# taconite/arah-release

Hardware: AMD Instinct MI355X
Metric: rendered rays/sec (higher is better)
Workload: dtype f32 (operands as hi+lo f16 pairs on the f16 MFMA pipe, fp32 accumulate)

## Files before the change

arah_release_amd/csrc/arah_hip.hip:

```cpp
#include <hip/hip_runtime.h>
#include <stdint.h>
#include <stdlib.h>
#include <string.h>

#include <atomic>
#include <mutex>
#include <type_traits>

#include "../../include/arah_hip.h"
#include "pointwise.hpp"
#include "mlp.hpp"

using namespace arah;

namespace {

constexpr float kRootThresh = 1e-5f;
constexpr int kSphereIters = 50;
constexpr float kSurfaceRange = 0.05f;
constexpr float kClampDist = 0.1f;
constexpr int kBroydenSteps = 50;
constexpr float kDvg = 1.0f;
constexpr int kMaxVerts = 6912;
constexpr int kKnnThreads = 1024;
// ... 187 lines not shown
                            const unsigned* amax, float* fw, float* pw, float* fws) {
    const int i = blockIdx.x * blockDim.x + threadIdx.x;
    if (i >= 6 * 256) return;
    const int k = i >> 8;
    const double c = kFilmScale;
    const double f = freq[i];
    fw[i] = (float)(f * c);
    pw[i] = (float)((f * (double)bias[i] + (double)phase[i]) * c);
    const float inv = k == 0 ? 1.0f : 1.0f / (split_weight_scale(amax[k - 1]) * kActScale);
    fws[i] = (float)(f * c) * inv;
    if ((i & 255) == 0) fws[6 * 256 + k] = inv;
}

struct SkinRaw {
    const float* w[4];
    const float* b[4];
};
__global__ __launch_bounds__(128) void k_skin_probe(SkinRaw net, unsigned* amax) {
    __shared__ float h[2][128];
    const int pt = blockIdx.x, c = threadIdx.x;
    const float x = -1.5f + 3.0f * (float)(pt % 9) / 8.0f, y = -1.5f + 3.0f * (float)((pt / 9) % 9) / 8.0f,
                z = -1.5f + 3.0f * (float)(pt / 81) / 8.0f;
    float v = softplus100(net.w[0][c * 3] * x + net.w[0][c * 3 + 1] * y + net.w[0][c * 3 + 2] * z + net.b[0][c]);
    h[0][c] = v;
    float m = v;
#pragma unroll
    for (int o = 32; o > 0; o >>= 1) m = fmaxf(m, __shfl_xor(m, o));
    if ((c & 63) == 0) atomicMax(amax + 0, __float_as_uint(m));
    __syncthreads();
    for (int k = 1; k < 4; ++k) {
        const float* hin = h[(k - 1) & 1];
        float s = net.b[k][c];
        for (int i = 0; i < 128; ++i) s += net.w[k][c * 128 + i] * hin[i];
        v = softplus100(s);
        h[k & 1][c] = v;
        m = v == v ? v : 0.f;
#pragma unroll
        for (int o = 32; o > 0; o >>= 1) m = fmaxf(m, __shfl_xor(m, o));
        if ((c & 63) == 0) atomicMax(amax + k, __float_as_uint(m));
        __syncthreads();
    }
}

__global__ void k_skin_scales(const unsigned* amax, float* scales) {
    const int k = threadIdx.x;
    if (k >= 4) return;
    const float a = __uint_as_float(amax[k]);
    float S = 1.0f;
    if (a > 0.f && a < 3.0e38f) {
        int e;
        frexpf(a, &e);
        S = ldexpf(1.0f, 11 - e);
    }
    scales[k] = S;
    scales[4 + k] = 1.0f / (split_weight_scale(amax[4 + k]) * S);
}

__global__ void k_skin_wave_consts(SkinRaw net, const float* __restrict__ w4, const float* __restrict__ w4b, const unsigned* amax,
                                   float* __restrict__ c) {
    const int i = threadIdx.x;
    auto act_scale = [&](int k) {
        const float a = __uint_as_float(amax[k]) * kZUnit;
        if (!(a > 0.f) || a > 3.0e38f) return 1.0f;
        int e;
        frexpf(a, &e);
        return e > 11 ? ldexpf(1.0f, 11 - e) : 1.0f;
    };
    const double M = (double)kCwShift;
    if (i < 128) {
        unsigned* ct = reinterpret_cast<unsigned*>(c + kCwW0T) + i * 8;
        unsigned short h[3], l[3];
#pragma unroll
        for (int k = 0; k < 3; ++k) {
            const float w = net.w[0][i * 3 + k] * kZUnit;
            const _Float16 hh = (_Float16)w, ll = (_Float16)(w - (float)hh);
            h[k] = __builtin_bit_cast(unsigned short, hh);
            l[k] = __builtin_bit_cast(unsigned short, ll);
        }
        ct[0] = ct[2] = (unsigned)h[0] | ((unsigned)h[1] << 16);
        ct[1] = ct[3] = (unsigned)h[2];
        ct[4] = ct[6] = (unsigned)l[0] | ((unsigned)l[1] << 16);
        ct[5] = ct[7] = (unsigned)l[2];
        c[kCwBinit + i] = (float)((double)net.b[0][i] * (double)kZUnit - M);
#pragma unroll 1
        for (int k = 1; k < 4; ++k) {
            double rs = 0.0;
            for (int col = 0; col < 128; ++col) rs += (double)net.w[k][i * 128 + col];
            c[kCwBinit + k * 128 + i] = (float)(((double)net.b[k][i] * (double)kZUnit + M * rs - M) * (double)act_scale(k - 1));
        }
    }
    if (i < 32) {
        double v = 0.0;
        if (i < 25) {
            double rs = 0.0;
            for (int col = 0; col < 128; ++col) rs += (double)w4[i * 128 + col];
            v = ((double)w4b[i] * (100.0 / 0.6931471805599453) + M * rs) * (double)act_scale(3);
        }
        c[kCwBinit + 512 + i] = (float)v;
    }
    if (i < 4) {
        c[kCwActS + i] = act_scale(i);
        if (i == 0) c[kCwScaled] = (act_scale(0) != 1.0f || act_scale(1) != 1.0f || act_scale(2) != 1.0f || act_scale(3) != 1.0f) ? 1.0f : 0.0f;
        c[kCwInv + i] = i < 3 ? 1.0f / act_scale(i) : 0.2f / act_scale(3);
    }
}

__global__ void k_gather_scalars(float* __restrict__ dst, const float* trans, const float* center, const float* cmin,
                                 const float* cmax, const float* beta) {
    const int i = threadIdx.x;
    if (i < 3) dst[i] = trans[i];
    else if (i < 6) dst[i] = center[i - 3];
    else if (i == 6) dst[i] = cmin[0];
    else if (i == 7) dst[i] = cmax[0];
    else if (i == 8) dst[i] = beta ? beta[0] : 1e-3f;
}

__global__ __launch_bounds__(64) void k_vertex_transforms(const float* __restrict__ weights, const float* __restrict__ bones,
                                                          int n_verts, float* __restrict__ vert_T) {
    __shared__ __attribute__((aligned(16))) float sb[24 * 16];
    for (int i = threadIdx.x; i < 24 * 16; i += 64) sb[i] = bones[i];
    __syncthreads();
    const int v = blockIdx.x * 64 + threadIdx.x;
    if (v >= n_verts) return;
    float T[16];
    blend(weights + (size_t)v * 24, sb, T);
#pragma unroll
    for (int c = 0; c < 4; ++c)
        reinterpret_cast<f32x4*>(vert_T + (size_t)v * 16)[c] = f32x4{T[c * 4], T[c * 4 + 1], T[c * 4 + 2], T[c * 4 + 3]};
}

__global__ void k_pad_rows4(float* __restrict__ dst, const float* __restrict__ src, int rows, int rows_pad, int ncol,
                            float fill) {
    const int r = blockIdx.x * blockDim.x + threadIdx.x;
    if (r >= rows_pad) return;
    f32x4 v = {fill, fill, fill, 0.f};
    if (r < rows) {
        for (int c = 0; c < 4; ++c) v[c] = c < ncol ? src[(size_t)r * ncol + c] : 0.f;
    }
    reinterpret_cast<f32x4*>(dst)[r] = v;
}

__global__ void k_copy(float* __restrict__ dst, const float* __restrict__ src, int n, int n_pad) {
    const int i = blockIdx.x * blockDim.x + threadIdx.x;
    if (i < n_pad) dst[i] = i < n ? src[i] : 0.f;
}

__global__ void k_fold_bias(float* __restrict__ dst, const float* __restrict__ b, const float* __restrict__ W, int ld,
                            int col0, const float* __restrict__ vec, int n_vec, int rows) {
    const int r = blockIdx.x * blockDim.x + threadIdx.x;
    if (r >= rows) return;
    float s = b[r];
    for (int c = 0; c < n_vec; ++c) s += W[(size_t)r * ld + col0 + c] * vec[c];
    dst[r] = s;
}

enum { SRC_POINTS = 0, SRC_RAYS = 1, SRC_SAMPLES = 2 };

constexpr int kClusterSize = 28;
constexpr int kClusterLds = 29;
constexpr int kMaxClusters = 256;
constexpr int kMaxCells = 65536;
constexpr int kCellBytes = 64;
constexpr float kGridMargin = 0.08f;

struct GridInfo {
    float origin[3];
    float h, inv_h;
    int dims[3];
    int n_cells;
    int n_clusters;
    int pad[2];
};

struct RaySet {
    const float* cam_loc;
    const float* dirs;
    int rays_per_cam;
};

__device__ __forceinline__ V3 ray_point(const RaySet& rs, int ray, float t) {
    const int cam = ray / rs.rays_per_cam;
    V3 p;
    p.x = rs.dirs[ray * 3 + 0] * t + rs.cam_loc[cam * 3 + 0];
    p.y = rs.dirs[ray * 3 + 1] * t + rs.cam_loc[cam * 3 + 1];
    p.z = rs.dirs[ray * 3 + 2] * t + rs.cam_loc[cam * 3 + 2];
    return p;
}

__device__ __forceinline__ void bitonic_cas(unsigned* keys, unsigned short* idxs, int i, int j, int k) {
    const int l = i | j;
    const bool up = (i & k) == 0;
    const unsigned ka = keys[i], kb = keys[l];
    const unsigned short ia = idxs[i], ib = idxs[l];
    const bool gt = ka > kb || (ka == kb && ia > ib);
    if (gt == up) {
        keys[i] = kb;
        keys[l] = ka;
        idxs[i] = ib;
        idxs[l] = ia;
    }
}
__device__ __forceinline__ void bitonic_sort_8192(unsigned* keys, unsigned short* idxs, int tid) {
    const int wave = tid >> 6, lane = tid & 63;
    for (int k = 2; k <= 8192; k <<= 1) {
        int j = k >> 1;
        for (; j >= 512; j >>= 1) {
            for (int t = tid; t < 4096; t += 1024) bitonic_cas(keys, idxs, ((t & ~(j - 1)) << 1) | (t & (j - 1)), j, k);
            __syncthreads();
        }
        for (; j > 0; j >>= 1) {
#pragma unroll
            for (int u = 0; u < 4; ++u) {
                const int t = lane + 64 * u;
                bitonic_cas(keys, idxs, wave * 512 + (((t & ~(j - 1)) << 1) | (t & (j - 1))), j, k);
            }
            __builtin_amdgcn_fence(__ATOMIC_RELEASE, "wavefront");
            __builtin_amdgcn_wave_barrier();
            __builtin_amdgcn_fence(__ATOMIC_ACQUIRE, "wavefront");
        }
        __syncthreads();
    }
}

__device__ __forceinline__ void wave_lds_handover() {
    __builtin_amdgcn_fence(__ATOMIC_RELEASE, "wavefront");
    __builtin_amdgcn_wave_barrier();
    __builtin_amdgcn_fence(__ATOMIC_ACQUIRE, "wavefront");
}

__device__ __forceinline__ int float_ordered(float f) {
    const int b = __float_as_int(f);
    return b >= 0 ? b : b ^ 0x7fffffff;
}
__device__ __forceinline__ float ordered_float(int o) { return __int_as_float(o >= 0 ? o : o ^ 0x7fffffff); }

__global__ __launch_bounds__(1024) void k_sort_verts(const float* __restrict__ verts, int n, float* __restrict__ sorted4,
                                                      GridInfo* __restrict__ grid) {
    __shared__ unsigned keys[8192];
    __shared__ unsigned short idxs[8192];
    __shared__ unsigned char segid[8192];
    int (*sbox)[6] = reinterpret_cast<int(*)[6]>(keys);
    __shared__ int sstart[2][257];
    __shared__ unsigned char saxis[256];
    __shared__ float bb[6];
    const int tid = threadIdx.x;
    for (int i = tid; i < 8192; i += 1024) {
        idxs[i] = (unsigned short)i;
        segid[i] = 0;
    }
    if (tid == 0) {
        sstart[0][0] = 0;
        sstart[0][1] = n;
    }
    __syncthreads();
    int cur = 0;
    for (int level = 0; level < 8; ++level) {
        const int nseg = 1 << level;
        for (int i = tid; i < nseg * 6; i += 1024) sbox[i / 6][i % 6] = (i % 6) < 3 ? 0x7fffffff : (int)0x80000000;
        __syncthreads();
        for (int i = tid; i < n; i += 1024) {
            const int o = idxs[i], sg = segid[i];
            for (int c = 0; c < 3; ++c) {
                const int v = float_ordered(verts[o * 3 + c]);
                atomicMin(&sbox[sg][c], v);
                atomicMax(&sbox[sg][3 + c], v);
            }
        }
        __syncthreads();
        if (level == 0 && tid < 6) bb[tid] = ordered_float(sbox[0][tid]);
        if (tid < nseg) {
            float e[3];
            for (int c = 0; c < 3; ++c) e[c] = ordered_float(sbox[tid][3 + c]) - ordered_float(sbox[tid][c]);
            saxis[tid] = (unsigned char)(e[0] >= e[1] ? (e[0] >= e[2] ? 0 : 2) : (e[1] >= e[2] ? 1 : 2));
        }
        __syncthreads();
        for (int i = tid; i < 8192; i += 1024) {
            unsigned key = 0xffffffffu;
            if (i < n) {
                const int o = idxs[i], sg = segid[i], a = saxis[sg];
                const float lo = bb[a], ext = fmaxf(bb[3 + a] - bb[a], 1e-9f);
                const unsigned q = (unsigned)fminf(fmaxf((verts[o * 3 + a] - lo) / ext * 65535.0f, 0.f), 65535.f);
                key = ((unsigned)sg << 16) | q;
            }
            keys[i] = key;
        }
        __syncthreads();
        bitonic_sort_8192(keys, idxs, tid);
        if (tid < nseg) {
            const int a = sstart[cur][tid], b = sstart[cur][tid + 1];
            sstart[cur ^ 1][2 * tid] = a;
            sstart[cur ^ 1][2 * tid + 1] = a + (b - a + 1) / 2;
            if (tid == nseg - 1) sstart[cur ^ 1][2 * nseg] = b;
        }
        __syncthreads();
        for (int i = tid; i < n; i += 1024) {
            const int sg = segid[i];
            segid[i] = (unsigned char)(2 * sg + (i >= sstart[cur ^ 1][2 * sg + 1] ? 1 : 0));
        }
        cur ^= 1;
        __syncthreads();
    }
    if (tid == 0) {
        GridInfo g;
        float ext[3];
        for (int c = 0; c < 3; ++c) {
            g.origin[c] = bb[c] - kGridMargin;
// ... 2712 lines not shown
    unsigned char* cells = nullptr;
};
constexpr size_t kBodyOffSpheres = (size_t)kMaxClusters * kClusterSize * 16;
constexpr size_t kBodyOffGrid = kBodyOffSpheres + (size_t)kMaxClusters * 16;
constexpr size_t kBodyOffCells = kBodyOffGrid + ((sizeof(GridInfo) + 255) / 256) * 256;
constexpr size_t kBodyBytes = kBodyOffCells + (size_t)kMaxCells * kCellBytes;
static_assert(kBodyOffSpheres == ARAH_BODY_OFF_SPHERES && kBodyOffGrid == ARAH_BODY_OFF_GRID && kBodyOffCells == ARAH_BODY_OFF_CELLS,
              "the body buffer's layout is part of the test ABI (arah_cell_clusters_debug)");

BodyTables body_tables(void* buf) {
    char* b = reinterpret_cast<char*>(buf);
    BodyTables t;
    t.verts4 = reinterpret_cast<float*>(b);
    t.spheres = reinterpret_cast<float*>(b + kBodyOffSpheres);
    t.grid = reinterpret_cast<GridInfo*>(b + kBodyOffGrid);
    t.cells = reinterpret_cast<unsigned char*>(b + kBodyOffCells);
    return t;
}

void launch_cell_clusters(int variant, const GridInfo* grid, const float* spheres, unsigned char* cells, hipStream_t s) {
    if (variant == 0)
        hipLaunchKernelGGL(k_cell_clusters, dim3(kMaxCells / kCellThreads), dim3(kCellThreads), 0, s, grid, spheres, cells);
    else
        hipLaunchKernelGGL(k_cell_clusters_wave, dim3(2048), dim3(kCellWaves * 64), 0, s, grid, spheres, cells);
}

void launch_body_tables(const float* verts, int n_verts, const BodyTables& t, hipStream_t s) {
    hipLaunchKernelGGL(k_sort_verts, dim3(1), dim3(1024), 0, s, verts, n_verts, t.verts4, t.grid);
    hipLaunchKernelGGL(k_cluster_spheres, dim3(1), dim3(256), 0, s, (const float*)t.verts4, t.spheres);
    launch_cell_clusters(1, t.grid, t.spheres, t.cells, s);
}

}

static B3Nets b3_of(const ArahFrame& f) {
    B3Nets b;
    for (int i = 0; i < 5; ++i) {
        b.sdf_wp[i] = reinterpret_cast<const bf16x8*>(f.b3[i]);
        b.sdf_wpT[i] = reinterpret_cast<const bf16x8*>(f.b3[5 + i]);
    }
    for (int i = 0; i < 6; ++i) {
        b.col[i] = reinterpret_cast<const bf16x8*>(f.b3[10 + i]);
        b.colT[i] = reinterpret_cast<const bf16x8*>(f.b3[16 + i]);
    }
    return b;
}

static bool shade_b3(int32_t shade_engine) { return shade_engine != ARAH_SHADE_ENGINE_FP32; }

extern "C" {

size_t arah_body_bytes(void) { return kBodyBytes; }

int arah_prepare_body(const float* verts, int32_t n_verts, void* body_buf, size_t body_bytes, void* stream) {
    if (!verts || !body_buf || (reinterpret_cast<uintptr_t>(body_buf) & 255) != 0) return ARAH_E_BADARG;
    if (n_verts <= 0 || n_verts > kMaxVerts) return ARAH_E_SHAPE;
    if (body_bytes < kBodyBytes) return ARAH_E_WORKSPACE;
    if (int arc = setup_attributes()) return arc;
    launch_body_tables(verts, n_verts, body_tables(body_buf), reinterpret_cast<hipStream_t>(stream));
    return check_launch();
}

int arah_cell_clusters_debug(int32_t variant, const void* grid, const float* spheres, uint8_t* cells, void* stream) {
    if ((variant != 0 && variant != 1) || !grid || !spheres || !cells) return ARAH_E_BADARG;
    launch_cell_clusters(variant, reinterpret_cast<const GridInfo*>(grid), spheres, cells, reinterpret_cast<hipStream_t>(stream));
    return check_launch();
}

const char* arah_dominant_kernel(void) { return "k_canon_wave"; }

size_t arah_frame_bytes(const ArahNets* h_nets, const ArahBody* h_body) {
    if (!h_nets || !h_body) return 0;
    return frame_layout(h_nets->col_mode).bytes;
}

int arah_prepare_frame(const ArahNets* nets, const ArahBody* body, void* frame_buf, size_t frame_bytes,
                       ArahFrame* out, void* stream) {
    if (!nets || !body || !frame_buf || !out) return ARAH_E_BADARG;
    if (nets->col_mode != ARAH_COLOR_IDR && nets->col_mode != ARAH_COLOR_NO_VIEW_DIR) return ARAH_E_SHAPE;
    if (body->n_verts <= 0 || body->n_verts > kMaxVerts || nets->n_pose < 0) return ARAH_E_SHAPE;
    if (nets->precision != ARAH_PRECISION_SPLIT_F16 && nets->precision != ARAH_PRECISION_FP32) return ARAH_E_BADARG;
    const FrameLayout L = frame_layout(nets->col_mode);
    if (frame_bytes < L.bytes) return ARAH_E_WORKSPACE;
    if (int arc = setup_attributes()) return arc;
    hipStream_t s = reinterpret_cast<hipStream_t>(stream);
    char* base = reinterpret_cast<char*>(frame_buf);
    auto P = [&](size_t off) { return reinterpret_cast<float*>(base + off); };
    const bool idr = nets->col_mode == ARAH_COLOR_IDR;
    const int kin_pad = idr ? ColDims<true>::kInPad : ColDims<false>::kInPad;
    const int kc0 = kin_pad / 16;
    const int n_view = idr ? 27 : 0;
    const int in_dim = 3 + n_view + 3 + 256 + nets->n_pose;
    PrepJobs jobs;
    unsigned* amax_sdf = reinterpret_cast<unsigned*>(base + L.sdf_amax);
    unsigned* amax_skin = reinterpret_cast<unsigned*>(base + L.skin_amax);
    hipLaunchKernelGGL(k_zero_words, dim3(1), dim3(64), 0, s, amax_sdf, 64, amax_skin, 64);
    jobs.add_rows4(P(L.sdf_w0), nets->sdf_w[0], 256, 256, 3);
    for (int i = 0; i < 5; ++i) {
        jobs.add_pack(P(L.sdf_wp[i]), nets->sdf_w[i + 1], 256, 256, 16, 16, one_seg(256), 0);
        jobs.add_pack(P(L.sdf_wpT[i]), nets->sdf_w[i + 1], 256, 256, 16, 16, one_seg(256), 1);
    }
    jobs.add_copy(P(L.sdf_w6), nets->sdf_w[6], 256, 256);
    for (int i = 0; i < 6; ++i) jobs.add_copy(P(L.sdf_bias) + i * 256, nets->sdf_b[i], 256, 256);
    jobs.add_copy(P(L.sdf_freq), nets->film_freq, 6 * 256, 6 * 256);
    jobs.add_copy(P(L.sdf_phase), nets->film_phase, 6 * 256, 6 * 256);
    jobs.add_copy(P(L.sdf_b6), nets->sdf_b[6], 1, 64);
    for (int i = 0; i < 5; ++i) {
        jobs.add_absmax(nets->sdf_w[i + 1], 256 * 256, amax_sdf + i, 16);
        jobs.add_split(reinterpret_cast<f16x8*>(base + L.sdf_wps[i]), nets->sdf_w[i + 1], 256, 256, 16, 8, amax_sdf + i, 0);
    }
    jobs.add_rows4(P(L.skin_w0), nets->skin_w[0], 128, 128, 3);
    for (int i = 0; i < 3; ++i) jobs.add_pack(P(L.skin_wp[i]), nets->skin_w[i + 1], 128, 128, 8, 8, one_seg(128), 0);
    jobs.add_pack(P(L.skin_w4p), nets->skin_w[4], 25, 128, 2, 8, one_seg(128), 0);
    for (int i = 0; i < 4; ++i) jobs.add_copy(P(L.skin_bias) + i * 128, nets->skin_b[i], 128, 128);
    jobs.add_copy(P(L.skin_bias) + 512, nets->skin_b[4], 25, 32);
    SkinRaw raw;
    for (int i = 0; i < 4; ++i) {
        raw.w[i] = nets->skin_w[i];
        raw.b[i] = nets->skin_b[i];
    }
    hipLaunchKernelGGL(k_skin_probe, dim3(9 * 9 * 9), dim3(128), 0, s, raw, amax_skin);
    for (int i = 0; i < 4; ++i) {
        const int M = i < 3 ? 128 : 25, mt = i < 3 ? 8 : 2;
        jobs.add_absmax(nets->skin_w[i + 1], M * 128, amax_skin + 4 + i, 8);
        jobs.add_split(reinterpret_cast<f16x8*>(base + L.skin_wps[i]), nets->skin_w[i + 1], M, 128, mt, 4, amax_skin + 4 + i, 0);
        jobs.add_split(reinterpret_cast<f16x8*>(base + L.skin_wpr + (size_t)i * kCwLayerBytes), nets->skin_w[i + 1], M, 128, mt, 4,
                       amax_skin + 4 + i, 1);
    }
    {
        ColSegs sg;
        memset(&sg, 0, sizeof(sg));
        const int feat0 = 3 + n_view + 3;
        sg.n = idr ? 4 : 3;
        sg.dst0[0] = 0; sg.src0[0] = feat0; sg.len[0] = 256;
        sg.dst0[1] = 256; sg.src0[1] = 0; sg.len[1] = 3;
        sg.dst0[2] = 259; sg.src0[2] = 3 + n_view; sg.len[2] = 3;
        if (idr) { sg.dst0[3] = 262; sg.src0[3] = 3; sg.len[3] = 27; }
        jobs.add_pack(P(L.col_w0p), nets->col_w[0], 256, in_dim, 16, kc0, sg, 0);
        jobs.add_pack(P(L.col_w3ap), nets->col_w[3], 256, in_dim + 128, 16, kc0, sg, 0);
        ColSegs sb = one_seg(128);
        sb.src0[0] = in_dim;
        jobs.add_pack(P(L.col_w3bp), nets->col_w[3], 256, in_dim + 128, 16, 8, sb, 0);
        jobs.add_pack(P(L.col_w1p), nets->col_w[1], 256, 256, 16, 16, one_seg(256), 0);
        jobs.add_pack(P(L.col_w2p), nets->col_w[2], 128, 256, 8, 16, one_seg(256), 0);
        jobs.add_pack(P(L.col_w4p), nets->col_w[4], 256, 256, 16, 16, one_seg(256), 0);
        jobs.add_pack(P(L.col_w0pT), nets->col_w[0], kin_pad, in_dim, kc0, 16, sg, 2, 256);
        jobs.add_pack(P(L.col_w3apT), nets->col_w[3], kin_pad, in_dim + 128, kc0, 16, sg, 2, 256);
        jobs.add_pack(P(L.col_w3bpT), nets->col_w[3], 128, in_dim + 128, 8, 16, sb, 2, 256);
        jobs.add_pack(P(L.col_w1pT), nets->col_w[1], 256, 256, 16, 16, one_seg(256), 1);
        jobs.add_pack(P(L.col_w2pT), nets->col_w[2], 256, 256, 16, 8, one_seg(128), 1);
        jobs.add_pack(P(L.col_w4pT), nets->col_w[4], 256, 256, 16, 16, one_seg(256), 1);
        jobs.add_copy(P(L.col_w5), nets->col_w[5], 3 * 256, 3 * 256);
        float* cb = P(L.col_bias);
        hipLaunchKernelGGL(k_fold_bias, dim3(1), dim3(256), 0, s, cb, nets->col_b[0], nets->col_w[0], in_dim,
                           feat0 + 256, nets->pose_vec, nets->pose_vec ? nets->n_pose : 0, 256);
        jobs.add_copy(cb + 256, nets->col_b[1], 256, 256);
        jobs.add_copy(cb + 512, nets->col_b[2], 128, 128);
        hipLaunchKernelGGL(k_fold_bias, dim3(1), dim3(256), 0, s, cb + 640, nets->col_b[3], nets->col_w[3],
                           in_dim + 128, feat0 + 256, nets->pose_vec, nets->pose_vec ? nets->n_pose : 0, 256);
        jobs.add_copy(cb + 896, nets->col_b[4], 256, 256);
        jobs.add_copy(cb + 1152, nets->col_b[5], 3, 4);
    }
    if (nets->precision == ARAH_PRECISION_SPLIT_F16) {
        const size_t src[kB3Count] = {L.sdf_wp[0], L.sdf_wp[1], L.sdf_wp[2], L.sdf_wp[3], L.sdf_wp[4],
                                      L.sdf_wpT[0], L.sdf_wpT[1], L.sdf_wpT[2], L.sdf_wpT[3], L.sdf_wpT[4],
                                      L.col_w0p, L.col_w1p, L.col_w2p, L.col_w3ap, L.col_w3bp, L.col_w4p,
                                      L.col_w0pT, L.col_w1pT, L.col_w2pT, L.col_w3apT, L.col_w3bpT, L.col_w4pT};
        for (int i = 5; i < 16; ++i) {
            const B3Src e = b3_source(i, kc0);
            jobs.add_b3(reinterpret_cast<bf16x8*>(base + L.b3[i]), (const float*)P(src[i]), e.m_tiles, e.kc16);
        }
    }
    if (!jobs.ok) return ARAH_E_LAUNCH;
    jobs.flush_a(s);
    jobs.flush_b(s);
    hipLaunchKernelGGL(k_fold_film, dim3(6), dim3(256), 0, s, (const float*)P(L.sdf_freq), (const float*)P(L.sdf_phase),
                       (const float*)P(L.sdf_bias), (const unsigned*)amax_sdf, P(L.sdf_fw), P(L.sdf_pw), P(L.sdf_fws));
    hipLaunchKernelGGL(k_skin_scales, dim3(1), dim3(64), 0, s, (const unsigned*)amax_skin, P(L.skin_scales));
    hipLaunchKernelGGL(k_skin_wave_consts, dim3(1), dim3(128), 0, s, raw, nets->skin_w[4], nets->skin_b[4],
                       (const unsigned*)amax_skin, P(L.skin_wconsts));
    if (!body->trans || !body->center || !body->coord_min || !body->coord_max || !body->verts || !body->vert_weights ||
        !body->bones)
        return ARAH_E_BADARG;
    hipLaunchKernelGGL(k_gather_scalars, dim3(1), dim3(64), 0, s, P(L.scalars), body->trans, body->center, body->coord_min,
                       body->coord_max, nets->beta);
    BodyTables bt;
    if (body->prepared) {
        bt = body_tables(const_cast<void*>(body->prepared));
    } else {
        bt.verts4 = P(L.verts4);
        bt.spheres = P(L.knn_spheres);
        bt.grid = reinterpret_cast<GridInfo*>(base + L.knn_grid);
        bt.cells = reinterpret_cast<unsigned char*>(base + L.knn_cells);
        launch_body_tables(body->verts, body->n_verts, bt, s);
    }
    hipLaunchKernelGGL(k_vertex_transforms, dim3((body->n_verts + 63) / 64), dim3(64), 0, s, body->vert_weights, body->bones,
                       body->n_verts, P(L.vert_T));
    memset(out, 0, sizeof(*out));
    out->sdf_w0 = P(L.sdf_w0);
    for (int i = 0; i < 5; ++i) {
        out->sdf_wp[i] = P(L.sdf_wp[i]);
        out->sdf_wpT[i] = P(L.sdf_wpT[i]);
    }
    out->sdf_w6 = P(L.sdf_w6);
    out->sdf_bias = P(L.sdf_bias);
    out->sdf_freq = P(L.sdf_freq);
    out->sdf_phase = P(L.sdf_phase);
    for (int i = 0; i < 5; ++i) out->sdf_wps[i] = base + L.sdf_wps[i];
    out->sdf_fw = P(L.sdf_fw);
    out->sdf_pw = P(L.sdf_pw);
    out->sdf_fws = P(L.sdf_fws);
    out->precision = nets->precision;
    out->skin_w0 = P(L.skin_w0);
    for (int i = 0; i < 3; ++i) out->skin_wp[i] = P(L.skin_wp[i]);
    out->skin_w4p = P(L.skin_w4p);
    out->skin_bias = P(L.skin_bias);
    for (int i = 0; i < 4; ++i) out->skin_wps[i] = base + L.skin_wps[i];
    out->skin_scales = P(L.skin_scales);
    out->skin_wpr = base + L.skin_wpr;
    out->skin_wconsts = P(L.skin_wconsts);
    out->col_w0p = P(L.col_w0p);
    out->col_w1p = P(L.col_w1p);
    out->col_w2p = P(L.col_w2p);
    out->col_w3ap = P(L.col_w3ap);
    out->col_w3bp = P(L.col_w3bp);
    out->col_w4p = P(L.col_w4p);
    out->col_w5 = P(L.col_w5);
    out->col_bias = P(L.col_bias);
    out->col_w0pT = P(L.col_w0pT);
    out->col_w1pT = P(L.col_w1pT);
    out->col_w2pT = P(L.col_w2pT);
    out->col_w3apT = P(L.col_w3apT);
    out->col_w3bpT = P(L.col_w3bpT);
    out->col_w4pT = P(L.col_w4pT);
    for (int i = 0; i < kB3Count; ++i) out->b3[i] = base + L.b3[i];
    out->verts4 = bt.verts4;
    out->knn_spheres = bt.spheres;
    out->knn_grid = bt.grid;
    out->knn_cells = bt.cells;
    out->verts = body->verts;
    out->vert_T = P(L.vert_T);
    out->bones = body->bones;
    out->sdf_b6 = P(L.sdf_b6);
    out->scalars = P(L.scalars);
    out->n_verts = body->n_verts;
    out->col_mode = nets->col_mode;
    return check_launch();
}

size_t arah_workspace_bytes(int32_t n_rays, int32_t n_steps) {
    if (n_rays < 0 || n_steps < 0) return 0;
    return carve(nullptr, n_rays, n_steps).bytes;
}

int arah_counters_reset(void* workspace, void* stream) {
    if (!workspace) return ARAH_E_BADARG;
    Workspace w = carve(workspace, 1, 1);
    return hipMemsetAsync(w.ctr, 0, sizeof(Counters), reinterpret_cast<hipStream_t>(stream)) == hipSuccess ? ARAH_OK
                                                                                                           : ARAH_E_LAUNCH;
}

#ifdef ARAH_CLOCKS
int arah_debug_clocks(const void* workspace, unsigned long long* h_out, void* stream) {
    if (!workspace || !h_out) return ARAH_E_BADARG;
    Workspace w = carve(const_cast<void*>(workspace), 1, 1);
    hipStream_t s = reinterpret_cast<hipStream_t>(stream);
    if (hipMemcpyAsync(h_out, w.ctr->clk, sizeof(w.ctr->clk) + sizeof(w.ctr->clk_shade), hipMemcpyDeviceToHost, s) != hipSuccess) return ARAH_E_LAUNCH;
    return hipStreamSynchronize(s) == hipSuccess ? ARAH_OK : ARAH_E_LAUNCH;
}
#endif

int arah_counters_read(const void* workspace, ArahCounters* h_out, void* stream) {
    if (!workspace || !h_out) return ARAH_E_BADARG;
    Workspace w = carve(const_cast<void*>(workspace), 1, 1);
    hipStream_t s = reinterpret_cast<hipStream_t>(stream);
    if (hipMemcpyAsync(h_out, w.ctr, sizeof(ArahCounters), hipMemcpyDeviceToHost, s) != hipSuccess) return ARAH_E_LAUNCH;
    return hipStreamSynchronize(s) == hipSuccess ? ARAH_OK : ARAH_E_LAUNCH;
}

int arah_sdf_eval(const ArahFrame* f, const float* x_norm, int32_t n, float* sdf, float* feat, float* grad,
                  void* workspace, size_t wbytes, void* stream) {
    if (!f || n < 0 || !workspace) return ARAH_E_BADARG;
    if (n == 0) return ARAH_OK;
    if (!x_norm || !sdf) return ARAH_E_BADARG;
    Workspace w = carve(workspace, 1, 1);
    if (wbytes < w.bytes) return ARAH_E_WORKSPACE;
    if (int arc = setup_attributes()) return arc;
    hipStream_t s = reinterpret_cast<hipStream_t>(stream);
    const FrameDev fd = to_dev(*f);
    const int g = grid_for(n, kTile);
    if (grad)
        LAUNCH_ENGINE(fd.split, (k_sdf_eval<true, true>), (k_sdf_eval<true, false>), dim3(g), dim3(kThreads), kLdsSdfGrad,
                      s, fd, x_norm, (const int*)nullptr, (const int*)nullptr, n, sdf, feat, grad, w.spill,
                      &w.ctr->n_sdf_fwd, &w.ctr->n_sdf_grad, 0);
    else
        LAUNCH_ENGINE(fd.split, (k_sdf_eval<false, true>), (k_sdf_eval<false, false>), dim3(g), dim3(kThreads),
                      kLdsSdfFwd, s, fd, x_norm, (const int*)nullptr, (const int*)nullptr, n, sdf, feat, (float*)nullptr,
                      (f32x4*)nullptr, &w.ctr->n_sdf_fwd, (unsigned long long*)nullptr, 0);
    return check_launch();
}

int arah_sdf_grid(const ArahFrame* f, int32_t n_side, float* sdf, void* workspace, size_t wbytes, void* stream) {
    if (!f || !sdf || !workspace || n_side < 2 || n_side > 1024) return ARAH_E_BADARG;
    Workspace w = carve(workspace, 1, 1);
    if (wbytes < w.bytes) return ARAH_E_WORKSPACE;
    if (int arc = setup_attributes()) return arc;
    hipStream_t s = reinterpret_cast<hipStream_t>(stream);
    const FrameDev fd = to_dev(*f);
    const long long n = (long long)n_side * n_side * n_side;
    if (n > 0x7fffffffLL) return ARAH_E_BADARG;
    if (fd.split && n >= 128ll * 1024)
        hipLaunchKernelGGL(k_sdf_lattice, dim3(min(num_cus(), grid_for(n, 128))), dim3(kThreads), kLdsDensityWide, s, fd, (int)n_side,
// ... 783 lines not shown
    const int64_t n_pix = (int64_t)H * W;
    unsigned long long* k = reinterpret_cast<unsigned long long*>(keys);
    int* med_list = pix_to_face;
    int* huge_list = reinterpret_cast<int*>(depth);
    unsigned* counters = reinterpret_cast<unsigned*>(bary);
    hipLaunchKernelGGL(k_mr_init, dim3(mesh_grid(n_pix, kMrMaxGrid)), dim3(kImeshThreads), 0, s, k, (long long)n_pix, counters);
    if (F > 0 && V > 0) {
        hipLaunchKernelGGL(k_mr_scatter, dim3(mesh_grid(F, kMrMaxGrid)), dim3(kImeshThreads), 0, s, verts, V, (const int*)faces, F, (int)H, (int)W, z_near,
                           (int)cull, (int)small_area, (int)wave_area, (int)huge_area, k, med_list, huge_list, (unsigned)n_pix, counters);
        hipLaunchKernelGGL(k_mr_lists, dim3(kMrListGrid), dim3(kImeshThreads), 0, s, verts, V, (const int*)faces, F, (int)H, (int)W, z_near,
                           (int)cull, k, (const int*)med_list, (const int*)huge_list, (unsigned)n_pix, (const unsigned*)counters);
    }
    hipLaunchKernelGGL(k_mr_resolve, dim3(mesh_grid(n_pix, kMrMaxGrid)), dim3(kImeshThreads), 0, s, verts, V, (const int*)faces, F, (int)H, (int)W,
                       (const unsigned long long*)k, (int*)pix_to_face, depth, bary);
    return check_launch();
}

int arah_mesh_rasterize(const float* verts, int64_t n_verts, const int32_t* faces, int64_t n_faces, int32_t H, int32_t W, float z_near,
                        int32_t cull, uint64_t* keys, int32_t* pix_to_face, float* depth, float* bary, void* stream) {
    return mr_rasterize(verts, n_verts, faces, n_faces, H, W, z_near, cull, kMrSmallArea, kMrWaveArea, kMrHugeArea, keys, pix_to_face,
                        depth, bary, stream);
}

int arah_mesh_rasterize_debug(const float* verts, int64_t n_verts, const int32_t* faces, int64_t n_faces, int32_t H, int32_t W,
                              float z_near, int32_t cull, int32_t small_area, int32_t wave_area, int32_t huge_area, uint64_t* keys,
                              int32_t* pix_to_face, float* depth, float* bary, void* stream) {
    return mr_rasterize(verts, n_verts, faces, n_faces, H, W, z_near, cull, small_area, wave_area, huge_area, keys, pix_to_face, depth,
                        bary, stream);
}

int arah_mesh_interpolate(const int32_t* pix_to_face, const float* bary, int32_t H, int32_t W, const int32_t* faces, int64_t n_faces,
                          const float* attr, int64_t n_verts, int32_t n_channels, float background, float* out, void* stream) {
    if (n_verts < 0 || n_faces < 0 || n_verts > (int64_t)INT32_MAX || n_faces > (int64_t)INT32_MAX) return ARAH_E_BADARG;
    if (H <= 0 || W <= 0 || (int64_t)H * W > (int64_t)INT32_MAX || n_channels < 1 || n_channels > 32) return ARAH_E_BADARG;
    if (!pix_to_face || !bary || !out || (n_verts > 0 && !attr) || (n_faces > 0 && !faces)) return ARAH_E_BADARG;
    const int64_t n_pix = (int64_t)H * W;
    hipLaunchKernelGGL(k_mr_interpolate, dim3(mesh_grid(n_pix * n_channels, kMrMaxGrid)), dim3(kImeshThreads), 0, reinterpret_cast<hipStream_t>(stream),
                       (const int*)pix_to_face, bary, (long long)n_pix, (const int*)faces, (int)n_faces, attr, (int)n_verts,
                       (int)n_channels, background, out);
    return check_launch();
}

int arah_skin_jacobian(const ArahFrame* f, const float* x_hat, int32_t n, float* jac, void* workspace, size_t wbytes,
                       void* stream) {
    if (!f || n < 0 || !workspace) return ARAH_E_BADARG;
    if (n == 0) return ARAH_OK;
    if (!x_hat || !jac) return ARAH_E_BADARG;
    Workspace w = carve(workspace, 1, 1);
    if (wbytes < w.bytes) return ARAH_E_WORKSPACE;
    if (int arc = setup_attributes()) return arc;
    hipLaunchKernelGGL(k_skin_jac, dim3(grid_for(n, 16)), dim3(kThreads), kLdsSkin,
                       reinterpret_cast<hipStream_t>(stream), to_dev(*f), x_hat, (const int*)nullptr,
                       (const int*)nullptr, n, jac, &w.ctr->n_skin_jac);
    return check_launch();
}

int arah_color_eval(const ArahFrame* f, const float* x_norm, const float* normal, const float* view,
                    const float* feat, int32_t n, float* rgb, void* workspace, size_t wbytes, void* stream) {
    if (!f || n < 0 || !workspace) return ARAH_E_BADARG;
    if (n == 0) return ARAH_OK;
    if (!x_norm || !normal || !feat || !rgb) return ARAH_E_BADARG;
    if (f->col_mode == ARAH_COLOR_IDR && !view) return ARAH_E_BADARG;
    Workspace w = carve(workspace, 1, 1);
    if (wbytes < w.bytes) return ARAH_E_WORKSPACE;
    if (int arc = setup_attributes()) return arc;
    hipStream_t s = reinterpret_cast<hipStream_t>(stream);
    const FrameDev fd = to_dev(*f);
    if (f->col_mode == ARAH_COLOR_IDR)
        hipLaunchKernelGGL(k_color_eval<true>, dim3(grid_for(n, kTile)), dim3(kThreads), lds_color<true>(), s, fd,
                           x_norm, normal, view, feat, n, rgb, &w.ctr->n_col);
    else
        hipLaunchKernelGGL(k_color_eval<false>, dim3(grid_for(n, kTile)), dim3(kThreads), lds_color<false>(), s, fd,
                           x_norm, normal, view, feat, n, rgb, &w.ctr->n_col);
    return check_launch();
}

int arah_nearest_inverse_lbs(const ArahFrame* f, const float* pts, int32_t n, int32_t* idx, float* x_hat0, float* T0,
                             void* workspace, size_t wbytes, void* stream) {
    if (!f || !pts || !x_hat0 || !T0 || n < 0 || !workspace) return ARAH_E_BADARG;
    if (n == 0) return ARAH_OK;
    Workspace w = carve(workspace, 1, 1);
    if (wbytes < w.bytes) return ARAH_E_WORKSPACE;
    if (int arc = setup_attributes()) return arc;
    RaySet rs = make_rays(nullptr, nullptr, 1);
    launch_nearest<SRC_POINTS>(reinterpret_cast<hipStream_t>(stream), to_dev(*f), n, pts, rs, (const float*)nullptr, 1,
                               (const int*)nullptr, (const int*)nullptr, n, idx, x_hat0, T0, 0,
                               &w.ctr->n_knn);
    return check_launch();
}

static int run_broyden3(const FrameDev& fd, Workspace& w, const float* tgt, CanonOut outp, long long max_pts,
                        hipStream_t s, int mode_arg = ARAH_CANON_KERNEL_WAVE, void* const* ev = nullptr,
                        const int* list_arg = nullptr, int* cnt_arg = nullptr) {
    int* cnt = cnt_arg ? cnt_arg : w.counts;
    const int* const list = list_arg ? list_arg : w.listA;
    if (tgt)
        hipLaunchKernelGGL(k_canon_seed, dim3(grid_for(max_pts, 256)), dim3(256), 0, s, list,
                           (const int*)&cnt[0], tgt, outp.T);
    const int mode = mode_arg == ARAH_CANON_KERNEL_TILE ? 0 : (mode_arg == ARAH_CANON_KERNEL_WAVE_L2 ? 2 : 1);
    hipEvent_t ev0 = ev ? reinterpret_cast<hipEvent_t>(ev[0]) : nullptr, ev1 = ev ? reinterpret_cast<hipEvent_t>(ev[1]) : nullptr;
    if (ev0 && ev1) hipEventRecord(ev0, s);
    unsigned long long* const clk_arg = w.ctr->clk;
    if (fd.split && mode != 0) {
        long long gw = (max_pts + kCwWaves * kCwSlots - 1) / (kCwWaves * kCwSlots);
        int cus = num_cus();
        if (list_arg && knobs().canon_tier_wgs > 0) cus = min(cus, knobs().canon_tier_wgs);
        if (gw > cus) gw = cus;
        if (gw < 1) gw = 1;
        if (mode == 1) {
            hipLaunchKernelGGL((k_canon_wave<true, false>), dim3((int)gw), dim3(kCwThreads), kLdsCanonWave, s, fd, list,
                               (const int*)&cnt[0], &cnt[1], outp, &w.ctr->n_skin_fwd, &w.ctr->n_canon,
                               &w.ctr->n_split_nonfinite, clk_arg);
            hipLaunchKernelGGL((k_canon_wave<true, true>), dim3((int)gw), dim3(kCwThreads), kLdsCanonWave, s, fd, list,
                               (const int*)&cnt[0], &cnt[1], outp, &w.ctr->n_skin_fwd, &w.ctr->n_canon,
                               &w.ctr->n_split_nonfinite, clk_arg);
        } else {
            const size_t lds_l2 = kLdsCanonWave - kCwHiBytes;
            hipLaunchKernelGGL((k_canon_wave<false, false>), dim3((int)gw), dim3(kCwThreads), lds_l2, s, fd,
                               list, (const int*)&cnt[0], &cnt[1], outp, &w.ctr->n_skin_fwd,
                               &w.ctr->n_canon, &w.ctr->n_split_nonfinite, clk_arg);
            hipLaunchKernelGGL((k_canon_wave<false, true>), dim3((int)gw), dim3(kCwThreads), lds_l2, s, fd,
                               list, (const int*)&cnt[0], &cnt[1], outp, &w.ctr->n_skin_fwd,
                               &w.ctr->n_canon, &w.ctr->n_split_nonfinite, clk_arg);
        }
    } else {
        LAUNCH_ENGINE(fd.split, k_canon_solve<true>, k_canon_solve<false>, dim3(grid_for(max_pts, kTile)), dim3(kThreads),
                      kLdsCanonSolve, s, fd, list, (const int*)&cnt[0], &cnt[1], outp,
                      &w.ctr->n_skin_fwd, &w.ctr->n_canon, w.ctr->clk);
    }
    if (ev0 && ev1) hipEventRecord(ev1, s);
    return check_launch();
}

int arah_broyden3_lbs(const ArahFrame* f, const float* tgt, const float* x0, const float* T0, int32_t n, float* x,
                      float* T, float* err, uint8_t* conv, int32_t canon_kernel, void* workspace, size_t wbytes, void* stream) {
    if (!f || n < 0 || !workspace) return ARAH_E_BADARG;
    if (n == 0) return ARAH_OK;
    if (!tgt || !x0 || !T0 || !x || !T || !conv) return ARAH_E_BADARG;
    Workspace w = carve(workspace, n, 1);
    if (wbytes < w.bytes) return ARAH_E_WORKSPACE;
    if (int arc = setup_attributes()) return arc;
    hipStream_t s = reinterpret_cast<hipStream_t>(stream);
    const FrameDev fd = to_dev(*f);
    hipMemcpyAsync(x, x0, (size_t)n * 3 * 4, hipMemcpyDeviceToDevice, s);
    hipMemcpyAsync(T, T0, (size_t)n * 16 * 4, hipMemcpyDeviceToDevice, s);
    hipMemsetAsync(w.counts, 0, sizeof(int) * 3 * kNumCounts, s);
    hipLaunchKernelGGL(k_iota, dim3((n + 255) / 256), dim3(256), 0, s, n, w.listA, &w.counts[0]);
    int rc = run_broyden3(fd, w, tgt, CanonOut{x, T, w.q_err}, n, s, canon_kernel);
    if (rc) return rc;
    hipLaunchKernelGGL(k_broyden3_finalize, dim3((n + 255) / 256), dim3(256), 0, s, n, (const float*)w.q_err, err, conv);
    return check_launch();
}

static void joint_impl(const FrameDev& fd, Workspace& w, const RaySet& rs, int n, float* T, hipStream_t s) {
    int* cntB = w.counts + kNumCounts;
    const int gm = grid_for(n, kTile);
    hipLaunchKernelGGL(k_skin_jac, dim3(grid_for(n, 16)), dim3(kThreads), kLdsSkin, s, fd, (const float*)w.x0raw,
                       (const int*)w.listA, (const int*)&cntB[0], 0, w.jac_lbs, &w.ctr->n_skin_jac);
    LAUNCH_ENGINE(fd.split, (k_sdf_eval<true, true>), (k_sdf_eval<true, false>), dim3(gm), dim3(kThreads), kLdsSdfGrad, s,
                  fd, (const float*)w.xcur, (const int*)w.listA, (const int*)&cntB[0], 0, w.u_gx ,
                  (float*)nullptr, w.grad_sdf, w.spill, &w.ctr->n_sdf_fwd, &w.ctr->n_sdf_grad, 0);
    Broyden4State st{w.u_eval, w.u_step, w.u_gx, w.u_Jinv, w.err_best_ray, w.xbest_ray, w.zbest_ray, T};
    hipLaunchKernelGGL(k_joint_init, dim3(grid_for(n, 256)), dim3(256), 0, s, fd, st, rs, (const int*)w.listA,
                       (const int*)&cntB[0], (const float*)w.grad_sdf, (const float*)w.jac_lbs, (const float*)w.xcur,
                       (const float*)w.t, w.x0raw);
    const int bulk = knobs().joint_bulk;
    for (int it = 0; it < bulk; ++it) {
        int* lin = (it & 1) ? w.listB : w.listA;
        int* lout = (it & 1) ? w.listA : w.listB;
        if (it == 0)
            LAUNCH_ENGINE(fd.split, (k_joint_iter<true, true>), (k_joint_iter<true, false>), dim3(gm), dim3(kThreads),
                          kLdsJoint, s, fd, st, rs, (const int*)lin, (const int*)&cntB[it], lout, &cntB[it + 1],
                          &w.ctr->n_skin_fwd, &w.ctr->n_sdf_fwd);
        else
            LAUNCH_ENGINE(fd.split, (k_joint_iter<false, true>), (k_joint_iter<false, false>), dim3(gm), dim3(kThreads),
                          kLdsJoint, s, fd, st, rs, (const int*)lin, (const int*)&cntB[it], lout, &cntB[it + 1],
                          &w.ctr->n_skin_fwd, &w.ctr->n_sdf_fwd);
    }
    if (bulk <= kBroydenSteps) {
        const int* lin = (bulk & 1) ? w.listB : w.listA;
        const int gf = min(4 * num_cus(), max(1, (n + kFinTile - 1) / kFinTile));
        LAUNCH_ENGINE(fd.split, k_joint_finish<true>, k_joint_finish<false>, dim3(gf), dim3(kThreads), kLdsJointFinish, s, fd,
                      st, rs, lin, (const int*)&cntB[bulk], kBroydenSteps + 1 - bulk, &w.ctr->n_skin_fwd, &w.ctr->n_sdf_fwd);
    }
}

static int trace_impl(const ArahFrame* f, Workspace& w, const float* cam_loc, int32_t rays_per_cam,
                      const float* dirs, const float* near_far, int32_t n, int root_find_all, float* points_hat_norm,
                      float* T, uint8_t* conv, float* start, float* end, hipStream_t s, const uint8_t* skip = nullptr) {
    const FrameDev fd = to_dev(*f);
    const RaySet rs = make_rays(cam_loc, dirs, rays_per_cam);
    const int gb = (n + 255) / 256;
    int* cntA = w.counts;
    int* cntB = w.counts + kNumCounts;
    hipMemsetAsync(w.counts, 0, sizeof(int) * 3 * kNumCounts, s);
    hipMemsetAsync(w.nn_idx, 0xff, sizeof(int) * (size_t)n, s);
    hipLaunchKernelGGL(k_trace_begin, dim3(gb), dim3(256), 0, s, near_far, n, w.t, w.far, w.diverged, w.xcur, w.Tcur,
                       w.listA, &cntA[0], skip);
    TraceState ts{w.t, w.far, w.xcur, w.diverged};
    const int gm = grid_for(n, kTile);
    const int bulk = n <= knobs().trace_small ? 0 : knobs().trace_bulk;
    for (int it = 0; it < bulk; ++it) {
        int* lin = (it & 1) ? w.listB : w.listA;
        int* lout = (it & 1) ? w.listA : w.listB;
        launch_nearest<SRC_RAYS>(s, fd, n, (const float*)nullptr, rs, (const float*)w.t, 1, (const int*)lin,
                                 (const int*)&cntA[it], 0, w.nn_idx, w.xcur, w.Tcur, 0, &w.ctr->n_knn);
        LAUNCH_ENGINE(fd.split, k_sdf_march<true>, k_sdf_march<false>, dim3(gm), dim3(kThreads), kLdsSdfFwd, s, fd, ts,
                      (const int*)lin, (const int*)&cntA[it], lout, &cntA[it + 1], &w.ctr->n_sdf_fwd);
    }
    if (bulk < kSphereIters) {
        const int* lin = (bulk & 1) ? w.listB : w.listA;
        const int gf = min(4 * num_cus(), max(1, (n + kFinTile - 1) / kFinTile));
        LAUNCH_ENGINE(fd.split, k_trace_finish<true>, k_trace_finish<false>, dim3(gf), dim3(kThreads), kLdsTraceFinish, s, fd,
                      knn_of(fd), rs, ts, w.Tcur, w.nn_idx, lin, (const int*)&cntA[bulk], kSphereIters - bulk, &w.ctr->n_knn,
                      &w.ctr->n_sdf_fwd);
    }
    hipLaunchKernelGGL(k_joint_select, dim3(gb), dim3(256), 0, s, fd, n, (const float*)w.xcur, (const float*)w.Tcur,
                       (const float*)w.t, (const uint8_t*)w.diverged, root_find_all, w.x0raw, w.xbest_ray, w.zbest_ray, T,
                       w.err_best_ray, w.listA, &cntB[0]);
    joint_impl(fd, w, rs, n, T, s);
    hipLaunchKernelGGL(k_trace_finalize, dim3(gb), dim3(256), 0, s, fd, n, near_far, (const float*)w.xbest_ray,
                       (const float*)w.zbest_ray, (const float*)w.err_best_ray, points_hat_norm, conv, start, end);
    return check_launch();
}

int arah_trace(const ArahFrame* f, const float* cam_loc, int32_t rays_per_cam, const float* dirs,
               const float* near_far, int32_t n, int32_t root_find_all, float* points_hat_norm, float* T,
               uint8_t* conv, float* start, float* end, void* workspace, size_t wbytes, void* stream) {
    if (!f || n < 0 || !workspace) return ARAH_E_BADARG;
    if (n == 0) return ARAH_OK;
    if (!cam_loc || !dirs || !near_far || !points_hat_norm || !T || !conv || !start || !end) return ARAH_E_BADARG;
    Workspace w = carve(workspace, n, 1);
    if (wbytes < w.bytes) return ARAH_E_WORKSPACE;
    if (int arc = setup_attributes()) return arc;
    return trace_impl(f, w, cam_loc, rays_per_cam, dirs, near_far, n, root_find_all, points_hat_norm, T, conv, start,
                      end, reinterpret_cast<hipStream_t>(stream));
}

int arah_joint_root_find(const ArahFrame* f, const float* cam_loc, int32_t rays_per_cam, const float* dirs,
                         const uint8_t* valid, const float* x0, const float* z0, const float* T0, int32_t n, float* x,
                         float* z, float* T, uint8_t* conv, void* workspace, size_t wbytes, void* stream) {
    if (!f || n < 0 || !workspace) return ARAH_E_BADARG;
    if (n == 0) return ARAH_OK;
    if (!cam_loc || !dirs || !valid || !x0 || !z0 || !T0 || !x || !z || !T || !conv) return ARAH_E_BADARG;
    Workspace w = carve(workspace, n, 1);
    if (wbytes < w.bytes) return ARAH_E_WORKSPACE;
    if (int arc = setup_attributes()) return arc;
    hipStream_t s = reinterpret_cast<hipStream_t>(stream);
    const FrameDev fd = to_dev(*f);
    const RaySet rs = make_rays(cam_loc, dirs, rays_per_cam);
    const int gb = (n + 255) / 256;
    hipMemsetAsync(w.counts, 0, sizeof(int) * 3 * kNumCounts, s);
    hipLaunchKernelGGL(k_joint_seed, dim3(gb), dim3(256), 0, s, fd, n, x0, z0, T0, valid, w.x0raw, w.xcur, w.t, w.xbest_ray,
                       w.zbest_ray, T, w.err_best_ray, w.listA, &w.counts[kNumCounts]);
    joint_impl(fd, w, rs, n, T, s);
    hipLaunchKernelGGL(k_joint_seam_out, dim3(gb), dim3(256), 0, s, n, (const float*)w.xbest_ray, (const float*)w.zbest_ray,
                       (const float*)w.err_best_ray, valid, x, z, conv);
    return check_launch();
}

static DepthArgs depth_args(const ArahSampling* cfg, const float* near_far, const float* start, const float* end) {
    return DepthArgs{cfg->n_near, cfg->n_far, near_far, start, end, cfg->lin_steps, cfg->lin_near, cfg->lin_far};
}

static void launch_sample_depths(int variant, int n, const ArahSampling* cfg, const float* near_far, const uint8_t* conv,
                                 const float* start, const float* end, const float* rand_s, const float* rand_near,
                                 const float* rand_far, float* z, uint8_t* mask, hipStream_t s) {
    if (variant == 0)
        hipLaunchKernelGGL(k_sample_depths, dim3((n + 127) / 128), dim3(128), 0, s, n, cfg->n_steps, cfg->n_near, cfg->n_far, near_far,
                           conv, start, end, cfg->lin_steps, cfg->lin_near, cfg->lin_far, rand_s, rand_near, rand_far, z, mask);
    else
        hipLaunchKernelGGL(k_sample_depths_wave, dim3(min(2048, (n + kTierWaves - 1) / kTierWaves)), dim3(kTierWaves * 64), 0, s, n,
                           cfg->n_steps, depth_args(cfg, near_far, start, end), conv, z, mask);
}

static int sample_impl(const ArahFrame* f, const ArahSampling* cfg, Workspace& w, const float* cam_loc,
                       int32_t rays_per_cam, const float* dirs, const float* near_far, const uint8_t* conv,
                       const float* start, const float* end, int32_t n, const float* rand_s, const float* rand_near,
                       const float* rand_far, float* z, float* pts, float* T, uint8_t* mask, hipStream_t s) {
    const int S = cfg->n_steps;
    const FrameDev fd = to_dev(*f);
    const RaySet rs = make_rays(cam_loc, dirs, rays_per_cam);
    const long long Q = (long long)n * S;
    hipMemsetAsync(w.counts, 0, sizeof(int) * 3 * kNumCounts, s);
    launch_sample_depths(rand_s || rand_near || rand_far ? 0 : 1, n, cfg, near_far, conv, start, end, rand_s, rand_near, rand_far, z,
                         w.q_smask, s);
    const int gq = (int)((Q + 255) / 256);
    hipLaunchKernelGGL(k_build_list, dim3((int)((Q + 4095) / 4096)), dim3(1024), 0, s, (const uint8_t*)w.q_smask, (int)Q, w.listA, &w.counts[0]);
    launch_nearest<SRC_SAMPLES>(s, fd, Q, (const float*)nullptr, rs, (const float*)z, S, (const int*)w.listA,
                                (const int*)&w.counts[0], 0, (int*)nullptr, pts, T, 1, &w.ctr->n_knn);
    int rc = run_broyden3(fd, w, nullptr, CanonOut{pts, T, w.q_err}, Q, s, cfg->canon_kernel, cfg->ev_canon);
    if (rc) return rc;
    hipLaunchKernelGGL(k_canon_finalize, dim3(gq), dim3(256), 0, s, fd, (int)Q, (const uint8_t*)w.q_smask,
                       (const float*)w.q_err, pts, T, mask);
    return check_launch();
}

static int check_sampling(const ArahSampling* cfg) {
    const int S = cfg->n_steps;
    if (S <= 0 || S > ARAH_MAX_STEPS || cfg->n_near < 0 || cfg->n_far < 0 || S < cfg->n_near + cfg->n_far + 1)
        return ARAH_E_SAMPLING;
    if (!cfg->lin_steps || !cfg->lin_near || (cfg->n_far > 0 && !cfg->lin_far)) return ARAH_E_BADARG;
    return ARAH_OK;
}

int arah_sample_canonicalize(const ArahFrame* f, const ArahSampling* cfg, const float* cam_loc, int32_t rays_per_cam,
                             const float* dirs, const float* near_far, const uint8_t* conv, const float* start,
                             const float* end, int32_t n, const float* rand_steps, const float* rand_near,
                             const float* rand_far, float* z, float* pts, float* T, uint8_t* mask, void* workspace,
                             size_t wbytes, void* stream) {
    if (!f || !cfg || n < 0 || !workspace) return ARAH_E_BADARG;
    int rc = check_sampling(cfg);
    if (rc) return rc;
    if (n == 0) return ARAH_OK;
    if (!cam_loc || !dirs || !near_far || !conv || !start || !end || !z || !pts || !T || !mask) return ARAH_E_BADARG;
    Workspace w = carve(workspace, n, cfg->n_steps);
    if (wbytes < w.bytes) return ARAH_E_WORKSPACE;
    if (int arc = setup_attributes()) return arc;
    if ((rand_steps || rand_near || rand_far) && (!rand_steps || !rand_near || (cfg->n_far > 0 && !rand_far)))
        return ARAH_E_BADARG;
    return sample_impl(f, cfg, w, cam_loc, rays_per_cam, dirs, near_far, conv, start, end, n, rand_steps, rand_near,
                       rand_far, z, pts, T, mask, reinterpret_cast<hipStream_t>(stream));
}

int arah_sample_depths_debug(int32_t variant, int32_t n, int32_t n_steps, int32_t n_near, int32_t n_far,
                             const float* near_far, const uint8_t* conv, const float* start, const float* end,
                             const float* lin_steps, const float* lin_near, const float* lin_far, float* z, uint8_t* mask,
                             void* stream) {
    if ((variant != 0 && variant != 1) || n < 0) return ARAH_E_BADARG;
    ArahSampling cfg;
    memset(&cfg, 0, sizeof(cfg));
    cfg.n_steps = n_steps;
    cfg.n_near = n_near;
    cfg.n_far = n_far;
    cfg.lin_steps = lin_steps;
    cfg.lin_near = lin_near;
    cfg.lin_far = lin_far;
    if (int rc = check_sampling(&cfg)) return rc;
    if (n == 0) return ARAH_OK;
    if (!near_far || !conv || !start || !end || !z || !mask) return ARAH_E_BADARG;
    launch_sample_depths(variant, n, &cfg, near_far, conv, start, end, nullptr, nullptr, nullptr, z, mask,
                         reinterpret_cast<hipStream_t>(stream));
    return check_launch();
}

static void launch_density(const FrameDev& fd, Workspace& w, const float* pts, long long Q, const int* list, const int* count,
                           int* next_list, int* next_count, hipStream_t s) {
    const int g = grid_for(Q, kTile);
    if (fd.split && Q >= 128ll * 1024)
        hipLaunchKernelGGL((k_density<true, 8>), dim3(min(num_cus(), grid_for(Q, 128))), dim3(kThreads), kLdsDensityWide, s, fd,
                           pts, list, count, w.shaded, next_list, next_count, &w.ctr->n_sdf_fwd, &w.ctr->n_density);
    else
        LAUNCH_ENGINE(fd.split, k_density<true>, k_density<false>, dim3(g), dim3(kThreads), kLdsSdfFwd, s, fd, pts, list, count,
                      w.shaded, next_list, next_count, &w.ctr->n_sdf_fwd, &w.ctr->n_density);
}

struct MapsOut {
    f32x4* nrm;
    float* normal;
    float* depth;
};

static int shade_tail(const ArahFrame* f, const ArahSampling* cfg, Workspace& w, const FrameDev& fd, const float* dirs,
                      const float* z, const float* pts, const float* T, const uint8_t* mask, int32_t n, const int* slist,
                      const int* scount, float* rgb, float* acc, uint8_t* vol_mask, const MapsOut* maps, hipStream_t s);

static int shade_impl(const ArahFrame* f, const ArahSampling* cfg, Workspace& w, const float* dirs, const float* z,
                      const float* pts, const float* T, const uint8_t* mask, int32_t n, float* rgb, float* acc,
                      uint8_t* vol_mask, const MapsOut* maps, hipStream_t s) {
    const int S = cfg->n_steps;
    const FrameDev fd = to_dev(*f);
    const long long Q = (long long)n * S;
    hipMemsetAsync(w.counts, 0, sizeof(int) * 3 * kNumCounts, s);
    hipLaunchKernelGGL(k_build_list, dim3((int)((Q + 4095) / 4096)), dim3(1024), 0, s, mask, (int)Q, w.listA, &w.counts[0]);
    const int g = grid_for(Q, kTile);
    const int* slist = w.listA;
    const int* scount = &w.counts[0];
    if (!cfg->full_shading) {
        if (cfg->ev_density[0] && cfg->ev_density[1]) hipEventRecord(reinterpret_cast<hipEvent_t>(cfg->ev_density[0]), s);
        launch_density(fd, w, pts, Q, (const int*)w.listA, (const int*)&w.counts[0], w.listB, &w.counts[1], s);
        if (cfg->ev_density[0] && cfg->ev_density[1]) hipEventRecord(reinterpret_cast<hipEvent_t>(cfg->ev_density[1]), s);
        slist = w.listB;
        scount = &w.counts[1];
    }
    return shade_tail(f, cfg, w, fd, dirs, z, pts, T, mask, n, slist, scount, rgb, acc, vol_mask, maps, s);
}

extern "C++" template <bool MAPS>
static void launch_shade(const ArahFrame* f, const ArahSampling* cfg, Workspace& w, const FrameDev& fd, const float* dirs,
                         const float* pts, const float* T, const int* slist, const int* scount, int g, f32x4* nrm,
                         hipStream_t s) {
    const int S = cfg->n_steps;
    const B3Nets b3 = b3_of(*f);
    if (fd.split && shade_b3(cfg->shade_engine)) {
        if (f->col_mode == ARAH_COLOR_IDR)
            hipLaunchKernelGGL((k_shade<true, true, true, MAPS>), dim3(g), dim3(kThreads), lds_shade_b3<true>(), s, fd,
                               S, cfg->cano_view_dirs, dirs, pts, T, slist, scount, 0, w.shaded, w.spill, &w.ctr->n_sdf_fwd,
                               &w.ctr->n_sdf_grad, &w.ctr->n_col, b3, nrm);
        else
            hipLaunchKernelGGL((k_shade<false, true, true, MAPS>), dim3(g), dim3(kThreads), lds_shade_b3<false>(), s, fd,
                               S, cfg->cano_view_dirs, dirs, pts, T, slist, scount, 0, w.shaded, w.spill, &w.ctr->n_sdf_fwd,
                               &w.ctr->n_sdf_grad, &w.ctr->n_col, b3, nrm);
    } else if (f->col_mode == ARAH_COLOR_IDR)
        LAUNCH_ENGINE(fd.split, (k_shade<true, true, false, MAPS>), (k_shade<true, false, false, MAPS>), dim3(g), dim3(kThreads),
                      lds_shade<true>(), s, fd, S, cfg->cano_view_dirs, dirs, pts, T, slist, scount, 0, w.shaded, w.spill,
                      &w.ctr->n_sdf_fwd, &w.ctr->n_sdf_grad, &w.ctr->n_col, b3, nrm);
    else
        LAUNCH_ENGINE(fd.split, (k_shade<false, true, false, MAPS>), (k_shade<false, false, false, MAPS>), dim3(g), dim3(kThreads),
                      lds_shade<false>(), s, fd, S, cfg->cano_view_dirs, dirs, pts, T, slist, scount, 0, w.shaded, w.spill,
                      &w.ctr->n_sdf_fwd, &w.ctr->n_sdf_grad, &w.ctr->n_col, b3, nrm);
}

static int shade_tail(const ArahFrame* f, const ArahSampling* cfg, Workspace& w, const FrameDev& fd, const float* dirs,
                      const float* z, const float* pts, const float* T, const uint8_t* mask, int32_t n, const int* slist,
                      const int* scount, float* rgb, float* acc, uint8_t* vol_mask, const MapsOut* maps, hipStream_t s) {
    const int S = cfg->n_steps;
    const long long Q = (long long)n * S;
    const int g = grid_for(Q, kTile);
    if (cfg->ev_shade[0] && cfg->ev_shade[1]) hipEventRecord(reinterpret_cast<hipEvent_t>(cfg->ev_shade[0]), s);
    if (maps) launch_shade<true>(f, cfg, w, fd, dirs, pts, T, slist, scount, g, maps->nrm, s);
    else launch_shade<false>(f, cfg, w, fd, dirs, pts, T, slist, scount, g, nullptr, s);
    if (cfg->ev_shade[0] && cfg->ev_shade[1]) hipEventRecord(reinterpret_cast<hipEvent_t>(cfg->ev_shade[1]), s);
    const bool chunk = S % 8 == 0 && (reinterpret_cast<uintptr_t>(z) & 15) == 0 && (reinterpret_cast<uintptr_t>(mask) & 7) == 0;
    const dim3 gc((n + 127) / 128), bc(128);
    if (maps) {
        if (chunk) hipLaunchKernelGGL(k_composite_maps<true>, gc, bc, 0, s, n, S, cfg->render_last_pt, z, mask, (const f32x4*)w.shaded,
                                      rgb, acc, vol_mask, (const f32x4*)maps->nrm, maps->normal, maps->depth);
        else hipLaunchKernelGGL(k_composite_maps<false>, gc, bc, 0, s, n, S, cfg->render_last_pt, z, mask, (const f32x4*)w.shaded,
                                rgb, acc, vol_mask, (const f32x4*)maps->nrm, maps->normal, maps->depth);
    } else if (chunk) hipLaunchKernelGGL(k_composite<true>, gc, bc, 0, s, n, S, cfg->render_last_pt, z, mask, (const f32x4*)w.shaded,
                                         rgb, acc, vol_mask);
    else hipLaunchKernelGGL(k_composite<false>, gc, bc, 0, s, n, S, cfg->render_last_pt, z, mask, (const f32x4*)w.shaded,
                            rgb, acc, vol_mask);
    return check_launch();
}

int arah_shade_points(const ArahFrame* f, const float* x_norm, const float* T, const float* dirs, int32_t n,
                      int32_t cano_view_dirs, int32_t shade_engine, float* rgbs, float* sdfn, void* workspace, size_t wbytes,
                      void* stream) {
    if (!f || n < 0 || !workspace) return ARAH_E_BADARG;
    if (n == 0) return ARAH_OK;
    if (!x_norm || !T || !dirs || !rgbs || !sdfn) return ARAH_E_BADARG;
    Workspace w = carve(workspace, n, 1);
    if (wbytes < w.bytes) return ARAH_E_WORKSPACE;
    if (int arc = setup_attributes()) return arc;
    hipStream_t s = reinterpret_cast<hipStream_t>(stream);
    const FrameDev fd = to_dev(*f);
    const B3Nets b3 = b3_of(*f);
    const int g = grid_for(n, kTile);
    f32x4* out = reinterpret_cast<f32x4*>(rgbs);
    f32x4* dbg = reinterpret_cast<f32x4*>(sdfn);
    if (fd.split && shade_b3(shade_engine)) {
        if (f->col_mode == ARAH_COLOR_IDR)
            hipLaunchKernelGGL((k_shade<true, true, true>), dim3(g), dim3(kThreads), lds_shade_b3<true>(), s, fd, 1,
                               cano_view_dirs, dirs, x_norm, T, (const int*)nullptr, (const int*)nullptr, n, out, w.spill,
                               &w.ctr->n_sdf_fwd, &w.ctr->n_sdf_grad, &w.ctr->n_col, b3, dbg);
        else
            hipLaunchKernelGGL((k_shade<false, true, true>), dim3(g), dim3(kThreads), lds_shade_b3<false>(), s, fd, 1,
                               cano_view_dirs, dirs, x_norm, T, (const int*)nullptr, (const int*)nullptr, n, out, w.spill,
                               &w.ctr->n_sdf_fwd, &w.ctr->n_sdf_grad, &w.ctr->n_col, b3, dbg);
    } else if (f->col_mode == ARAH_COLOR_IDR)
        LAUNCH_ENGINE(fd.split, (k_shade<true, true>), (k_shade<true, false>), dim3(g), dim3(kThreads), lds_shade<true>(),
                      s, fd, 1, cano_view_dirs, dirs, x_norm, T, (const int*)nullptr, (const int*)nullptr, n, out, w.spill,
                      &w.ctr->n_sdf_fwd, &w.ctr->n_sdf_grad, &w.ctr->n_col, b3, dbg);
    else
        LAUNCH_ENGINE(fd.split, (k_shade<false, true>), (k_shade<false, false>), dim3(g), dim3(kThreads),
                      lds_shade<false>(), s, fd, 1, cano_view_dirs, dirs, x_norm, T, (const int*)nullptr, (const int*)nullptr, n,
                      out, w.spill, &w.ctr->n_sdf_fwd, &w.ctr->n_sdf_grad, &w.ctr->n_col, b3, dbg);
    return check_launch();
}

int arah_shade_composite(const ArahFrame* f, const ArahSampling* cfg, const float* dirs, const float* z,
                         const float* pts, const float* T, const uint8_t* mask, int32_t n, float* rgb, float* acc,
                         uint8_t* vol_mask, void* workspace, size_t wbytes, void* stream) {
    if (!f || !cfg || n < 0 || !workspace) return ARAH_E_BADARG;
    if (cfg->n_steps <= 0 || cfg->n_steps > ARAH_MAX_STEPS) return ARAH_E_SAMPLING;
    if (n == 0) return ARAH_OK;
    if (!dirs || !z || !pts || !T || !mask || !rgb || !vol_mask) return ARAH_E_BADARG;
    Workspace w = carve(workspace, n, cfg->n_steps);
    if (wbytes < w.bytes) return ARAH_E_WORKSPACE;
    if (int arc = setup_attributes()) return arc;
    return shade_impl(f, cfg, w, dirs, z, pts, T, mask, n, rgb, acc, vol_mask, nullptr, reinterpret_cast<hipStream_t>(stream));
}

static ColNetT colT_of(const ArahFrame& f) {
    return ColNetT{f.col_w0pT, f.col_w1pT, f.col_w2pT, f.col_w3apT, f.col_w3bpT, f.col_w4pT};
}

static bool train_b3(const ArahFrame& f) {
    return knobs().train_b3 && f.precision == ARAH_PRECISION_SPLIT_F16;
}

size_t arah_shade_train_slab_bytes(void) { return (size_t)kMaxGrid / 2 * kTrainSlabPerWg * sizeof(f32x4); }

int arah_shade_train_forward(const ArahFrame* f, const ArahTrainIn* in, float* sdf, float* rgb4, void* workspace,
// ... 1704 lines not shown
```

arah_release_amd/csrc/finish.hpp:

```cpp
#pragma once

constexpr int kFinTile = 16;
constexpr size_t kLdsTraceFinish = (kFinTile * 4 * 2 + kFinTile * 16 + kFinTile * 8) * 4 + (size_t)kFinTile * kSdfLd * 4;
constexpr size_t kLdsJointFinish = (kFinTile * 4 * 3 + 24 * 16 + kFinTile * 2 + kFinTile * kLogitLd + 32) * 4 + (size_t)kFinTile * kSdfLd * 4;

template <bool SPLIT>
__global__ __launch_bounds__(kThreads, 4) void k_trace_finish(FrameDev fr, KnnData kd, RaySet rs, TraceState st, float* Tcur,
                                                            int* nn_idx, const int* list, const int* count, int steps_left,
                                                            unsigned long long* ctr_knn, unsigned long long* ctr_fwd) {
    const BodyConst bc = load_bc(fr);
    extern __shared__ __attribute__((aligned(16))) float smem[];
    float* xin = smem;
    float* outv = xin + kFinTile * 4;
    float* Tl = outv + kFinTile * 4;
    int* ids = reinterpret_cast<int*>(Tl + kFinTile * 16);
    float* tl = reinterpret_cast<float*>(ids + kFinTile);
    float* farl = tl + kFinTile;
    int* nnl = reinterpret_cast<int*>(farl + kFinTile);
    int* divl = nnl + kFinTile;
    int* s_live = divl + kFinTile;
    float* actA = reinterpret_cast<float*>(s_live + 3 * kFinTile);
    const int tid = threadIdx.x, wave = __builtin_amdgcn_readfirstlane(tid >> 6), lane = tid & 63;
    const int n = *count;
    const GridInfo g = *kd.grid;
    const float scale = sdf_scale(bc);
    int n_done = 0;
    for (int tile = blockIdx.x; tile * kFinTile < n; tile += gridDim.x) {
        __syncthreads();
        if (tid < kFinTile) {
            const int i = tile * kFinTile + tid;
            const int id = i < n ? list[i] : -1;
            ids[tid] = id;
            tl[tid] = id >= 0 ? st.t[id] : 0.f;
            farl[tid] = id >= 0 ? st.far[id] : 0.f;
            nnl[tid] = id >= 0 ? nn_idx[id] : -1;
            divl[tid] = 0;
        }
        for (int step = 0; step < steps_left; ++step) {
            __syncthreads();
            if (wave == 0) {
                const unsigned long long live = __ballot(lane < kFinTile && ids[lane] >= 0);
                n_done += __popcll(live);
                if (lane == 0) *s_live = live != 0ull;
            }
            __syncthreads();
            if (!*s_live) break;
            if (wave < 4) {
                const int s = wave * 4 + (lane >> 4);
                const int id = ids[s];
                if (id >= 0) {
                    const V3 p = ray_point(rs, id, tl[s]);
                    float best = 3.4e38f;
                    int bi = 0x7fffffff;
                    const int seed = nnl[s];
                    if (seed >= 0) {
                        const float dx = fr.verts_raw[seed * 3] - p.x, dy = fr.verts_raw[seed * 3 + 1] - p.y,
                                    dz = fr.verts_raw[seed * 3 + 2] - p.z;
                        best = dx * dx + dy * dy + dz * dz;
                        bi = seed;
                    }
                    bi = nearest_vertex_group16<kClusterSize>(kd, kd.sorted4, kd.spheres, g, p, best, bi, lane);
                    if ((lane & 15) == 0) {
                        float T[16];
                        vertex_transform(fr, bi, T);
                        const V3 y = V3{p.x - bc.trans[0], p.y - bc.trans[1], p.z - bc.trans[2]};
                        const V3 xh = normalize_pt(bc, inverse_affine_apply(T, y));
                        store_T(Tl + s * 16, T);
                        nnl[s] = bi;
                        reinterpret_cast<f32x4*>(xin)[s] = f32x4{xh.x, xh.y, xh.z, 0.f};
                    }
                } else if ((lane & 15) == 0) {
                    reinterpret_cast<f32x4*>(xin)[s] = f32x4{0.f, 0.f, 0.f, 0.f};
                }
            }
            __syncthreads();
            f32x4 dlast[kSdfMT][1];
            sdf_trunk<false, 1, SPLIT>(fr.sdf, xin, actA, kSdfLd, nullptr, dlast, wave, lane);
            sdf_head<SPLIT>(fr.sdf, actA, kSdfLd, outv, 4, tid, kFinTile);
            __syncthreads();
            if (tid < kFinTile) {
                const int id = ids[tid];
                if (id >= 0) {
                    const float sdf = outv[tid * 4] * scale;
                    const float march = fminf(fmaxf(sdf, -kClampDist), kClampDist);
                    bool div = false;
                    if (fabsf(march) > kRootThresh) {
                        const float t = tl[tid] + march;
                        tl[tid] = t;
                        div = t >= farl[tid];
                        divl[tid] = div ? 1 : 0;
                    }
                    const bool keep = !((fabsf(sdf) <= kRootThresh) || div);
                    if (!keep || step + 1 == steps_left) {
                        st.t[id] = tl[tid];
                        st.diverged[id] = divl[tid] ? 1 : 0;
                        const f32x4 xn = reinterpret_cast<const f32x4*>(xin)[tid];
                        st.xcur[(size_t)id * 3] = xn[0];
                        st.xcur[(size_t)id * 3 + 1] = xn[1];
                        st.xcur[(size_t)id * 3 + 2] = xn[2];
#pragma unroll
                        for (int c = 0; c < 4; ++c)
                            reinterpret_cast<f32x4*>(Tcur + (size_t)id * 16)[c] = reinterpret_cast<const f32x4*>(Tl + tid * 16)[c];
                        nn_idx[id] = nnl[tid];
                        ids[tid] = -1;
                    }
                }
            }
        }
    }
    if (tid == 0) {
        count_add(ctr_knn, n_done);
        count_add(ctr_fwd, n_done);
    }
}

template <bool SPLIT>
__global__ __launch_bounds__(kThreads, 4) void k_joint_finish(FrameDev fr, Broyden4State st, RaySet rs, const int* list,
                                                            const int* count, int iters_left, unsigned long long* ctr_skin,
                                                            unsigned long long* ctr_sdf) {
    const BodyConst bc = load_bc(fr);
    extern __shared__ __attribute__((aligned(16))) float smem[];
    constexpr int TW = kFinTile;
    float* xin = smem;
    float* xraw = xin + TW * 4;
    float* outv = xraw + TW * 4;
    float* sbones = outv + TW * 4;
    int* ids = reinterpret_cast<int*>(sbones + 24 * 16);
    int* s_live = ids + TW;
    float* logits = reinterpret_cast<float*>(s_live + TW);
    float* act = logits + TW * kLogitLd;
    const int tid = threadIdx.x, wave = __builtin_amdgcn_readfirstlane(tid >> 6), lane = tid & 63;
    const int n = *count;
    const float scale = sdf_scale(bc);
    int n_done = 0;
    for (int i = tid; i < 24 * 16; i += kThreads) sbones[i] = fr.bones[i];
    for (int tile = blockIdx.x; tile * TW < n; tile += gridDim.x) {
        __syncthreads();
        if (tid < TW) {
            const int i = tile * TW + tid;
            ids[tid] = i < n ? list[i] : -1;
        }
        for (int it = 0; it < iters_left; ++it) {
            __syncthreads();
            if (wave == 0) {
                const unsigned long long live = __ballot(lane < TW && ids[lane] >= 0);
                n_done += __popcll(live);
                if (lane == 0) *s_live = live != 0ull;
            }
            if (tid < TW) {
                const int id = ids[tid];
                f32x4 u = {0.f, 0.f, 0.f, 0.f};
                if (id >= 0) u = reinterpret_cast<const f32x4*>(st.ueval)[id];
                const V3 q = normalize_pt(bc, V3{u[0], u[1], u[2]});
                reinterpret_cast<f32x4*>(xin)[tid] = f32x4{q.x, q.y, q.z, 0.f};
                reinterpret_cast<f32x4*>(xraw)[tid] = u;
            }
            __syncthreads();
            if (!*s_live) break;
            skin_mlp<1>(fr.skin, xin, act, logits, wave, lane);
            f32x4 dlast[kSdfMT][1];
            sdf_trunk<false, 1, SPLIT>(fr.sdf, xin, act, kSdfLd, nullptr, dlast, wave, lane);
            sdf_head<SPLIT>(fr.sdf, act, kSdfLd, outv, 4, tid, TW);
            __syncthreads();
            if (tid < TW) {
                const int id = ids[tid];
                if (id >= 0) {
                    float T[16];
                    V3 xb;
                    const f32x4 u = reinterpret_cast<const f32x4*>(xraw)[tid];
                    skin_tail(logits + tid * kLogitLd, sbones, V3{u[0], u[1], u[2]}, T, xb);
                    const V3 p = ray_point(rs, id, u[3]);
                    float gnew[4] = {outv[tid * 4] * scale, xb.x - (p.x - bc.trans[0]), xb.y - (p.y - bc.trans[1]),
                                     xb.z - (p.z - bc.trans[2])};
                    float J[16], stp[4], gx[4], dg[4], dx[4];
#pragma unroll
                    for (int e = 0; e < 16; ++e) J[e] = st.Jinv[(size_t)id * 16 + e];
#pragma unroll
                    for (int r = 0; r < 4; ++r) {
                        dx[r] = st.step[(size_t)id * 4 + r];
                        const float gold = st.gx[(size_t)id * 4 + r];
                        dg[r] = gnew[r] - gold;
                        gx[r] = gold + dg[r];
                    }
                    const float err = sqrtf(gx[0] * gx[0] + gx[1] * gx[1] + gx[2] * gx[2] + gx[3] * gx[3]);
                    float eb = st.err_best[id];
                    if (err < eb) {
                        eb = err;
                        st.err_best[id] = err;
                        st.xbest[(size_t)id * 3] = u[0];
                        st.xbest[(size_t)id * 3 + 1] = u[1];
                        st.xbest[(size_t)id * 3 + 2] = u[2];
                        st.zbest[id] = u[3];
                        store_T(st.Tbest + (size_t)id * 16, T);
                    }
                    const bool keep = (eb > kRootThresh) && (err < kDvg);
                    if (keep) {
                        broyden_update<4>(J, dx, dg, gx, stp);
#pragma unroll
                        for (int r = 0; r < 4; ++r) st.gx[(size_t)id * 4 + r] = gx[r];
#pragma unroll
                        for (int e = 0; e < 16; ++e) st.Jinv[(size_t)id * 16 + e] = J[e];
                        reinterpret_cast<f32x4*>(st.step)[id] = f32x4{stp[0], stp[1], stp[2], stp[3]};
                        reinterpret_cast<f32x4*>(st.ueval)[id] = f32x4{u[0] + stp[0], u[1] + stp[1], u[2] + stp[2], u[3] + stp[3]};
                    } else {
                        ids[tid] = -1;
                    }
                }
            }
        }
    }
    if (tid == 0) {
        count_add(ctr_skin, n_done);
        count_add(ctr_sdf, n_done);
    }
}
```

arah_release_amd/csrc/mlp.hpp:

```cpp
#pragma once
#include <hip/hip_runtime.h>

#include "pointwise.hpp"

namespace arah {

typedef float f32x4 __attribute__((ext_vector_type(4)));

constexpr int kThreads = 512;
constexpr int kWaves = 8;
constexpr int kTile = 64;
constexpr int kNT = 4;

__device__ __forceinline__ void zero_acc(f32x4& a) { a = f32x4{0.f, 0.f, 0.f, 0.f}; }

__device__ __forceinline__ void no_pack(f32x4& v) { asm volatile("" : "+v"(v[0]), "+v"(v[1]), "+v"(v[2]), "+v"(v[3])); }

template <typename Tp>
__device__ __forceinline__ Tp ld_frag(const void* __restrict__ base, unsigned lane_off, int const_off) {
    typedef unsigned u32x4_t __attribute__((ext_vector_type(4)));
    static_assert(sizeof(Tp) == 16, "fragments are 16 bytes per lane");
    const __amdgpu_buffer_rsrc_t rsrc = __builtin_amdgcn_make_buffer_rsrc(const_cast<void*>(base), 0, 0x7fffffff, 0x00020000);
    const u32x4_t v = __builtin_amdgcn_raw_buffer_load_b128(rsrc, (int)lane_off + (const_off & 4095), const_off & ~4095, 0);
    return __builtin_bit_cast(Tp, v);
// ... 137 lines not shown
                    bl[x][n] = *reinterpret_cast<const f16x8*>(bptr + n * 16 * ld * 4 + lo_off + (kc + 1) * 64);
                }
            }
#pragma unroll
            for (int m = 0; m < MT; ++m)
#pragma unroll
                for (int n = 0; n < NT; ++n)
                    acc[m][n] = __builtin_amdgcn_mfma_f32_16x16x32_f16(al[c][m], bh[c][n], acc[m][n], 0, 0, 0);
#pragma unroll
            for (int m = 0; m < MT; ++m)
#pragma unroll
                for (int n = 0; n < NT; ++n)
                    acc[m][n] = __builtin_amdgcn_mfma_f32_16x16x32_f16(ah[c][m], bl[c][n], acc[m][n], 0, 0, 0);
#pragma unroll
            for (int m = 0; m < MT; ++m)
#pragma unroll
                for (int n = 0; n < NT; ++n)
                    acc[m][n] = __builtin_amdgcn_mfma_f32_16x16x32_f16(ah[c][m], bh[c][n], acc[m][n], 0, 0, 0);
            __builtin_amdgcn_sched_barrier(0);
        }
    } else {
        f16x8 ah[MT], al[MT], ahn[MT], aln[MT];
#pragma unroll
        for (int m = 0; m < MT; ++m) {
            ah[m] = lda(((m * KC32) * 2 + 0));
            al[m] = lda(((m * KC32) * 2 + 1));
        }
#pragma unroll 1
        for (int kc = 0; kc < KC32; ++kc) {
            const int kn = kc + 1 < KC32 ? kc + 1 : kc;
#pragma unroll
            for (int m = 0; m < MT; ++m) {
                ahn[m] = lda(((m * KC32 + kn) * 2 + 0));
                aln[m] = lda(((m * KC32 + kn) * 2 + 1));
            }
            f16x8 bh[NT], bl[NT];
#pragma unroll
            for (int n = 0; n < NT; ++n) {
                bh[n] = *reinterpret_cast<const f16x8*>(bptr + n * 16 * ld * 4 + kc * 64);
                bl[n] = *reinterpret_cast<const f16x8*>(bptr + n * 16 * ld * 4 + lo_off + kc * 64);
            }
#pragma unroll
            for (int m = 0; m < MT; ++m)
#pragma unroll
                for (int n = 0; n < NT; ++n)
                    acc[m][n] = __builtin_amdgcn_mfma_f32_16x16x32_f16(al[m], bh[n], acc[m][n], 0, 0, 0);
#pragma unroll
            for (int m = 0; m < MT; ++m)
#pragma unroll
                for (int n = 0; n < NT; ++n)
                    acc[m][n] = __builtin_amdgcn_mfma_f32_16x16x32_f16(ah[m], bl[n], acc[m][n], 0, 0, 0);
#pragma unroll
            for (int m = 0; m < MT; ++m)
#pragma unroll
                for (int n = 0; n < NT; ++n)
                    acc[m][n] = __builtin_amdgcn_mfma_f32_16x16x32_f16(ah[m], bh[n], acc[m][n], 0, 0, 0);
#pragma unroll
            for (int m = 0; m < MT; ++m) {
                ah[m] = ahn[m];
                al[m] = aln[m];
            }
        }
    }
}

template <int I>
struct IC {
    static constexpr int value = I;
};
template <int I, int N, typename F>
__device__ __forceinline__ void static_for(F&& f) {
    if constexpr (I < N) {
        f(IC<I>{});
        static_for<I + 1, N>(f);
    }
}

typedef __bf16 bf16x8 __attribute__((ext_vector_type(8)));
__device__ __forceinline__ f32x4 mfma_frag(const f16x8 a, const f16x8 b, const f32x4 c) {
    return __builtin_amdgcn_mfma_f32_16x16x32_f16(a, b, c, 0, 0, 0);
}
__device__ __forceinline__ f32x4 mfma_frag(const bf16x8 a, const bf16x8 b, const f32x4 c) {
    return __builtin_amdgcn_mfma_f32_16x16x32_bf16(a, b, c, 0, 0, 0);
}
template <int KC32, int MT, int NT, int H, typename FR = f16x8>
__device__ __forceinline__ void gemm_acc_split_pipe(const FR* __restrict__ wp, int mt0, const float* act, int ld,
                                                    int lo_off, f32x4 (&acc)[MT][NT], int lane) {
    constexpr int NH = NT / H, S = KC32 * H;
    const int j = lane & 15, g = lane >> 4;
    const char* bptr = reinterpret_cast<const char*>(act) + j * ld * 4 + split_slot(j, g) * 16;
    const unsigned aoff = (unsigned)(mt0 * KC32 * 2 * 64 + lane) * 16u;
    auto lda = [&](int idx) { return ld_frag<FR>(wp, aoff, idx * 1024); };
    FR ah[2][MT], al[2][MT], bh[2][NH], bl[2][NH];
#pragma unroll
    for (int m = 0; m < MT; ++m) {
        ah[0][m] = lda((m * KC32) * 2 + 0);
        al[0][m] = lda((m * KC32) * 2 + 1);
    }
#pragma unroll
    for (int n = 0; n < NH; ++n) {
        bh[0][n] = *reinterpret_cast<const FR*>(bptr + n * 16 * ld * 4);
        bl[0][n] = *reinterpret_cast<const FR*>(bptr + n * 16 * ld * 4 + lo_off);
    }
    __builtin_amdgcn_sched_barrier(0);
    static_for<0, S>([&](auto Sc) {
        constexpr int s = decltype(Sc)::value, kc = s / H, h = s % H, cb = s & 1, ca = kc & 1;
        constexpr bool more_b = s + 1 < S, more_a = h == 0 && kc + 1 < KC32;
        if constexpr (more_a) {
#pragma unroll
            for (int m = 0; m < MT; ++m) {
                ah[ca ^ 1][m] = lda((m * KC32 + kc + 1) * 2 + 0);
                al[ca ^ 1][m] = lda((m * KC32 + kc + 1) * 2 + 1);
            }
        }
        if constexpr (more_b) {
            constexpr int k1 = (s + 1) / H, h1 = (s + 1) % H;
#pragma unroll
            for (int n = 0; n < NH; ++n) {
                bh[cb ^ 1][n] = *reinterpret_cast<const FR*>(bptr + (h1 * NH + n) * 16 * ld * 4 + k1 * 64);
                bl[cb ^ 1][n] = *reinterpret_cast<const FR*>(bptr + (h1 * NH + n) * 16 * ld * 4 + lo_off + k1 * 64);
            }
        }
#pragma unroll
        for (int m = 0; m < MT; ++m)
#pragma unroll
            for (int n = 0; n < NH; ++n)
                acc[m][h * NH + n] = mfma_frag(al[ca][m], bh[cb][n], acc[m][h * NH + n]);
#pragma unroll
        for (int m = 0; m < MT; ++m)
#pragma unroll
            for (int n = 0; n < NH; ++n)
                acc[m][h * NH + n] = mfma_frag(ah[ca][m], bl[cb][n], acc[m][h * NH + n]);
#pragma unroll
        for (int m = 0; m < MT; ++m)
#pragma unroll
            for (int n = 0; n < NH; ++n)
                acc[m][h * NH + n] = mfma_frag(ah[ca][m], bh[cb][n], acc[m][h * NH + n]);
        constexpr int n_vm = more_a ? 2 * MT : 0, n_ds = more_b ? 2 * NH : 0, n_mf = 3 * MT * NH;
        constexpr int per = (n_vm + n_ds) > 0 ? (n_mf - 2) / (n_vm + n_ds) : n_mf;
        constexpr int lead = per >= 2 ? 2 : 1;
        static_for<0, n_vm>([&](auto) {
            __builtin_amdgcn_sched_group_barrier(0x008, lead > per ? per : (per >= 1 ? per : 1), 0);
            __builtin_amdgcn_sched_group_barrier(0x020, 1, 0);
        });
        static_for<0, n_ds>([&](auto) {
            __builtin_amdgcn_sched_group_barrier(0x008, per >= 1 ? per : 1, 0);
            __builtin_amdgcn_sched_group_barrier(0x100, 1, 0);
        });
        __builtin_amdgcn_sched_group_barrier(0x008, n_mf, 0);
        __builtin_amdgcn_sched_barrier(0);
    });
}


struct B3Nets {
    const bf16x8* sdf_wp[5];
    const bf16x8* sdf_wpT[5];
    const bf16x8* col[6];
    const bf16x8* colT[6];
};

__device__ __forceinline__ void bsplit8(const f32x4 a, const f32x4 b, bf16x8& hi, bf16x8& lo) {
    typedef __bf16 bf16x2 __attribute__((ext_vector_type(2)));
    typedef float f32x2 __attribute__((ext_vector_type(2)));
#pragma unroll
    for (int i = 0; i < 4; ++i) {
        const float x0 = i < 2 ? a[2 * i] : b[2 * i - 4], x1 = i < 2 ? a[2 * i + 1] : b[2 * i - 3];
        const bf16x2 h = __builtin_convertvector(f32x2{x0, x1}, bf16x2);
        const bf16x2 l = __builtin_convertvector(f32x2{x0 - (float)h[0], x1 - (float)h[1]}, bf16x2);
        hi[2 * i] = h[0];
        hi[2 * i + 1] = h[1];
        lo[2 * i] = l[0];
        lo[2 * i + 1] = l[1];
    }
}

template <int KC16, int MT, int NT = kNT>
__device__ __forceinline__ void gemm_acc_b3(const bf16x8* __restrict__ wp, int mt0, const float* act, int ld,
                                            f32x4 (&acc)[MT][NT], int lane) {
    constexpr int KC32 = (KC16 + 1) / 2;
    const int j = lane & 15, g = lane >> 4;
    const unsigned aoff = (unsigned)(mt0 * KC32 * 2 * 64 + lane) * 16u;
    auto lda = [&](int idx) { return ld_frag<bf16x8>(wp, aoff, idx * 1024); };
    const bool tail_ok = (KC16 & 1) == 0 || g < 2;
    const float* brow = act + j * ld;
    bf16x8 ah[MT], al[MT], ahn[MT], aln[MT];
#pragma unroll
    for (int m = 0; m < MT; ++m) {
        ah[m] = lda((m * KC32) * 2 + 0);
        al[m] = lda((m * KC32) * 2 + 1);
    }
#pragma unroll 2
    for (int kc = 0; kc < KC32; ++kc) {
        const int kn = kc + 1 < KC32 ? kc + 1 : kc;
#pragma unroll
        for (int m = 0; m < MT; ++m) {
            ahn[m] = lda((m * KC32 + kn) * 2 + 0);
            aln[m] = lda((m * KC32 + kn) * 2 + 1);
        }
        const bool ok = kc + 1 < KC32 || tail_ok;
        const float* bp = brow + (ok ? kc * 32 + 8 * g : 0);
#pragma unroll
        for (int n = 0; n < NT; ++n) {
            f32x4 x0 = *reinterpret_cast<const f32x4*>(bp + n * 16 * ld);
            f32x4 x1 = *reinterpret_cast<const f32x4*>(bp + n * 16 * ld + 4);
            if (!ok) x0 = x1 = f32x4{0.f, 0.f, 0.f, 0.f};
            bf16x8 bh, bl;
            bsplit8(x0, x1, bh, bl);
#pragma unroll
            for (int m = 0; m < MT; ++m) {
                acc[m][n] = __builtin_amdgcn_mfma_f32_16x16x32_bf16(al[m], bh, acc[m][n], 0, 0, 0);
                acc[m][n] = __builtin_amdgcn_mfma_f32_16x16x32_bf16(ah[m], bl, acc[m][n], 0, 0, 0);
                acc[m][n] = __builtin_amdgcn_mfma_f32_16x16x32_bf16(ah[m], bh, acc[m][n], 0, 0, 0);
            }
        }
#pragma unroll
        for (int m = 0; m < MT; ++m) {
            ah[m] = ahn[m];
            al[m] = aln[m];
        }
    }
}

template <bool B3, int KC16, int MT, int NT = kNT>
__device__ __forceinline__ void gemm_any(const float* __restrict__ wp, const bf16x8* __restrict__ wpb, int mt0, const float* act,
                                         int ld, f32x4 (&acc)[MT][NT], int lane) {
    if constexpr (B3) gemm_acc_b3<KC16, MT, NT>(wpb, mt0, act, ld, acc, lane);
    else gemm_acc<KC16, MT, NT>(wp, mt0, act, ld, acc, lane);
}

__device__ __forceinline__ void store_bsplit4(float* act, int ld, int lo_off, int pt, int ch0, const f32x4 v) {
    typedef __bf16 bf16x2 __attribute__((ext_vector_type(2)));
    typedef float f32x2 __attribute__((ext_vector_type(2)));
    typedef unsigned u32x2 __attribute__((ext_vector_type(2)));
    u32x2 hi, lo;
#pragma unroll
    for (int p = 0; p < 2; ++p) {
        const bf16x2 h = __builtin_convertvector(f32x2{v[2 * p], v[2 * p + 1]}, bf16x2);
        const bf16x2 l = __builtin_convertvector(f32x2{v[2 * p] - (float)h[0], v[2 * p + 1] - (float)h[1]}, bf16x2);
        hi[p] = __builtin_bit_cast(unsigned, h);
        lo[p] = __builtin_bit_cast(unsigned, l);
    }
    char* row = reinterpret_cast<char*>(act) + pt * ld * 4 + split_byte(pt, ch0);
    *reinterpret_cast<u32x2*>(row) = hi;
    *reinterpret_cast<u32x2*>(row + lo_off) = lo;
}
__device__ __forceinline__ void store_bsplit1(float* act, int ld, int lo_off, int pt, int ch, float v) {
    const __bf16 h = (__bf16)v;
    char* row = reinterpret_cast<char*>(act) + pt * ld * 4 + split_byte(pt, ch);
    *reinterpret_cast<__bf16*>(row) = h;
    *reinterpret_cast<__bf16*>(row + lo_off) = (__bf16)(v - (float)h);
}
__device__ __forceinline__ float load_bsplit(const float* act, int ld, int lo_off, int pt, int ch) {
    const char* row = reinterpret_cast<const char*>(act) + pt * ld * 4 + split_byte(pt, ch);
    return (float)*reinterpret_cast<const __bf16*>(row) + (float)*reinterpret_cast<const __bf16*>(row + lo_off);
}

template <int KC32, int MT, int NT = kNT>
__device__ __forceinline__ void gemm_acc_bsplit(const bf16x8* __restrict__ wp, int mt0, const float* act, int ld, int lo_off,
                                                f32x4 (&acc)[MT][NT], int lane) {
    gemm_acc_split_pipe<KC32, MT, NT, NT % 2 == 0 ? 2 : 1, bf16x8>(wp, mt0, act, ld, lo_off, acc, lane);
}

__device__ __forceinline__ float opaque_one() {
    float one;
    asm("s_mov_b32 %0, 1.0" : "=s"(one));
    return one;
}
__device__ __forceinline__ unsigned split_residual2(float a, float b, unsigned hi_pk) {
    typedef _Float16 f16x2 __attribute__((ext_vector_type(2)));
    const float one = opaque_one();
    const f16x2 h = __builtin_bit_cast(f16x2, hi_pk);
    f16x2 l;
    l[0] = (_Float16)__builtin_fmaf(a, one, -(float)h[0]);
    l[1] = (_Float16)__builtin_fmaf(b, one, -(float)h[1]);
    return __builtin_bit_cast(unsigned, l);
}
__device__ __forceinline__ void store_split4(float* act, int ld, int lo_off, int pt, int ch0, const f32x4 hs) {
    typedef _Float16 f16x2 __attribute__((ext_vector_type(2)));
    typedef float f32x2 __attribute__((ext_vector_type(2)));
    typedef unsigned u32x2 __attribute__((ext_vector_type(2)));
    u32x2 hi, lo;
#pragma unroll
    for (int p = 0; p < 2; ++p) {
        const f16x2 h2 = __builtin_convertvector(f32x2{hs[2 * p], hs[2 * p + 1]}, f16x2);
        hi[p] = __builtin_bit_cast(unsigned, h2);
        lo[p] = split_residual2(hs[2 * p], hs[2 * p + 1], hi[p]);
    }
    char* row = reinterpret_cast<char*>(act) + pt * ld * 4 + split_byte(pt, ch0);
    *reinterpret_cast<u32x2*>(row) = hi;
    *reinterpret_cast<u32x2*>(row + lo_off) = lo;
}

__device__ __forceinline__ void split4(const float (&v)[4], unsigned& h0, unsigned& h1, unsigned& l0, unsigned& l1) {
    typedef _Float16 f16x2 __attribute__((ext_vector_type(2)));
    typedef float f32x2 __attribute__((ext_vector_type(2)));
    h0 = __builtin_bit_cast(unsigned, __builtin_convertvector(f32x2{v[0], v[1]}, f16x2));
    h1 = __builtin_bit_cast(unsigned, __builtin_convertvector(f32x2{v[2], v[3]}, f16x2));
    l0 = split_residual2(v[0], v[1], h0);
    l1 = split_residual2(v[2], v[3], h1);
}

__device__ __forceinline__ float load_split(const float* act, int ld, int lo_off, int pt, int ch) {
    const char* row = reinterpret_cast<const char*>(act) + pt * ld * 4 + split_byte(pt, ch);
    return ((float)*reinterpret_cast<const _Float16*>(row) + (float)*reinterpret_cast<const _Float16*>(row + lo_off)) * kInvActScale;
}
// ... 287 lines not shown
        const float u = bwd[pt * ld + ch];
        const f32x4 w = *reinterpret_cast<const f32x4*>(net.w0 + ch * 4);
        gx += w[0] * u;
        gy += w[1] * u;
        gz += w[2] * u;
    }
#pragma unroll
    for (int o = 1; o < 8; o <<= 1) {
        gx += __shfl_xor(gx, o);
        gy += __shfl_xor(gy, o);
        gz += __shfl_xor(gz, o);
    }
    if (part == 0) {
        out[pt * ostride + 1] = gx;
        out[pt * ostride + 2] = gy;
        out[pt * ostride + 3] = gz;
    }
}

struct SkinNet {
    const float* w0;
    const float* wp[3];
    const float* w4p;
    const float* bias;
    const f16x8* wps[4];
    const float* scales;
};

constexpr int kSkinLd = 136;
constexpr int kLogitLd = 33;

struct SkinWave {
    const f16x8* wpr;
    const float* consts;
};
constexpr int kCwLayerBytes = 128 * 128 * 4;
constexpr int kCwWeightBytes = 3 * kCwLayerBytes + 32 * 128 * 4;
enum {
    kCwW0T = 0,
    kCwBinit = 1024,
    kCwInv = 1568,
    kCwActS = 1572,
    kCwScaled = 1576,
    kCwSize = 1580
};
constexpr float kZUnit = 144.269504088896341f;
constexpr float kCwShift = 24.0f;

__device__ __forceinline__ float softplus_shift(float zs, float inf) {
    const float e = __builtin_amdgcn_fmed3f(__builtin_amdgcn_exp2f(zs), 0.f, 1.f);
    return __builtin_amdgcn_fmed3f(zs, __builtin_amdgcn_logf(e + 0x1p-24f), inf);
}

__device__ __forceinline__ float softplus100_scaled(float xs, float c1, float c2) {
    const float e = __builtin_amdgcn_exp2f(-fabsf(xs) * c1);
    return fmaf(__builtin_amdgcn_logf(1.0f + e), c2, fmaxf(xs, 0.f));
}
__device__ __forceinline__ float softplus100(float x) {
    return softplus100_scaled(x, 144.269504088896341f, 6.93147180559945e-3f);
}

template <int NT = kNT, bool SPLIT = false, typename CLK = NoClk>
__device__ __forceinline__ void skin_mlp(const SkinNet& net, const float* xin, float* act, float* logits, int wave,
                                         int lane, CLK&& clk = NoClk()) {
    const int j = lane & 15, g = lane >> 4;
    const int ld = kSkinLd;
    constexpr float kSat = 65504.0f;
    {
        const int ch0 = wave * 16 + 4 * g;
        f32x4 w[4];
#pragma unroll
        for (int r = 0; r < 4; ++r) w[r] = *reinterpret_cast<const f32x4*>(net.w0 + (ch0 + r) * 4);
        const f32x4 b = *reinterpret_cast<const f32x4*>(net.bias + ch0);
        const float S = SPLIT ? net.scales[0] : 1.0f;
        const float c1 = 144.269504088896341f / S, c2 = 6.93147180559945e-3f * S;
#pragma unroll
        for (int n = 0; n < NT; ++n) {
            const f32x4 x = *reinterpret_cast<const f32x4*>(xin + (n * 16 + j) * 4);
            f32x4 h;
#pragma unroll
            for (int r = 0; r < 4; ++r)
                h[r] = fmaf(w[r][2], x[2], fmaf(w[r][1], x[1], fmaf(w[r][0], x[0], b[r])));
            no_pack(h);
            if (SPLIT) {
#pragma unroll
                for (int r = 0; r < 4; ++r) h[r] = fminf(softplus100_scaled(h[r] * S, c1, c2), kSat);
                store_split4(act, ld, 256, n * 16 + j, ch0, h);
            } else {
#pragma unroll
                for (int r = 0; r < 4; ++r) h[r] = softplus100(h[r]);
                *reinterpret_cast<f32x4*>(act + (n * 16 + j) * ld + ch0) = h;
            }
        }
    }
    __syncthreads();
    clk.mark(2);
    SplitA<4> a_out;
#pragma unroll 1
    for (int k = 1; k < 4; ++k) {
        f32x4 acc[1][NT];
#pragma unroll
        for (int n = 0; n < NT; ++n) zero_acc(acc[0][n]);
        if (SPLIT) gemm_acc_split<4, 1, NT>(net.wps[k - 1], wave, act, ld, 256, acc, lane);
        else gemm_acc<8, 1, NT>(net.wp[k - 1], wave, act, ld, acc, lane);
        clk.mark(1 + 2 * k);
        const int ch0 = wave * 16 + 4 * g;
        f32x4 b = *reinterpret_cast<const f32x4*>(net.bias + k * 128 + ch0);
        const float S = SPLIT ? net.scales[k] : 1.0f;
        const float inv = SPLIT ? net.scales[4 + k - 1] * S : 1.0f;
        __syncthreads();
        const float c1 = 144.269504088896341f / S, c2 = 6.93147180559945e-3f * S;
        if (SPLIT) b = b * S;
#pragma unroll
        for (int n = 0; n < NT; ++n) {
            f32x4 h;
            if (SPLIT) {
#pragma unroll
                for (int r = 0; r < 4; ++r)
                    h[r] = fminf(softplus100_scaled(fmaf(acc[0][n][r], inv, b[r]), c1, c2), kSat);
                store_split4(act, ld, 256, n * 16 + j, ch0, h);
            } else {
#pragma unroll
                for (int r = 0; r < 4; ++r) h[r] = softplus100(acc[0][n][r] + b[r]);
                *reinterpret_cast<f32x4*>(act + (n * 16 + j) * ld + ch0) = h;
            }
        }
        if (k < 3) {
            __syncthreads();
            clk.mark(2 + 2 * k);
        }
    }
    if (SPLIT && (wave >> 1) < NT) a_out = load_split_a<4>(net.wps[3], wave & 1, lane);
    __syncthreads();
    clk.mark(8);
    {
        const int mt = wave & 1, nt = wave >> 1;
        if (nt < NT) {
            f32x4 acc;
            if (SPLIT) {
                acc = gemm_one_split<4>(a_out, nt, act, ld, 256, lane) * net.scales[7];
            } else {
                acc = gemm_one<8>(net.w4p, mt, nt, act, ld, lane);
            }
            const int ch0 = mt * 16 + 4 * g;
            const f32x4 b = *reinterpret_cast<const f32x4*>(net.bias + 4 * 128 + ch0);
#pragma unroll
            for (int r = 0; r < 4; ++r) logits[(nt * 16 + j) * kLogitLd + ch0 + r] = acc[r] + b[r];
        }
    }
    __syncthreads();
    clk.mark(9);
}

struct ColNet {
    const float* w0p;
    const float* w1p;
    const float* w2p;
    const float* w3ap;
    const float* w3bp;
    const float* w4p;
    const float* w5;
    const float* bias;
};

template <bool IDR>
struct ColDims {
    static constexpr int kExtra = IDR ? 33 : 6;
    static constexpr int kIn = 256 + kExtra;
    static constexpr int kKC0 = (kIn + 15) / 16;
    static constexpr int kInPad = kKC0 * 16;
    static constexpr int kLdA = kInPad + 8;
};

template <int MT>
__device__ __forceinline__ void relu_store(const f32x4 (&acc)[MT][kNT], const float* bias, float* dst, int ld,
                                           int mt0, int lane) {
    const int j = lane & 15, g = lane >> 4;
#pragma unroll
    for (int m = 0; m < MT; ++m) {
        const int ch0 = (mt0 + m) * 16 + 4 * g;
        const f32x4 b = *reinterpret_cast<const f32x4*>(bias + ch0);
#pragma unroll
        for (int n = 0; n < kNT; ++n) {
            f32x4 h;
#pragma unroll
            for (int r = 0; r < 4; ++r) h[r] = fmaxf(acc[m][n][r] + b[r], 0.f);
            *reinterpret_cast<f32x4*>(dst + (n * 16 + j) * ld + ch0) = h;
        }
    }
}

struct ColTap {
    float* cin;
    float* c[5];
    long long row0;
    int rows;
};

__device__ __forceinline__ void resplit_rows_bf16(float* act, int ld, int lo_off, int tid) {
    f32x4 v[8];
#pragma unroll
    for (int i = 0; i < 8; ++i) {
        const int e = tid + i * kThreads, pt = e >> 6, ch0 = (e & 63) * 4;
#pragma unroll
        for (int r = 0; r < 4; ++r) v[i][r] = load_split(act, ld, 512, pt, ch0 + r);
    }
    __syncthreads();
#pragma unroll
    for (int i = 0; i < 8; ++i) {
        const int e = tid + i * kThreads;
        store_bsplit4(act, ld, lo_off, e >> 6, (e & 63) * 4, v[i]);
    }
}

__device__ __forceinline__ f32x4 layer0_dfactor(const SdfNet& net, const float* xin, int mt0, int m, int n, int lane) {
    const int j = lane & 15, g = lane >> 4;
    const int ch0 = (mt0 + m) * 16 + 4 * g;
    const f32x4 x = *reinterpret_cast<const f32x4*>(xin + (n * 16 + j) * 4);
    const f32x4 fw = *reinterpret_cast<const f32x4*>(net.fw + ch0);
    const f32x4 pw = *reinterpret_cast<const f32x4*>(net.pw + ch0);
    const f32x4 f = *reinterpret_cast<const f32x4*>(net.freq + ch0);
    f32x4 v, h, d;
#pragma unroll
    for (int r = 0; r < 4; ++r) {
        const f32x4 w = *reinterpret_cast<const f32x4*>(net.w0 + (ch0 + r) * 4);
        v[r] = fmaf(w[2], x[2], fmaf(w[1], x[1], w[0] * x[0]));
    }
    no_pack(v);
    film_sine<true>(v, fw, pw, f, 1.0f, h, d);
    return d;
}

template <typename CLK = NoClk>
__device__ __forceinline__ void sdf_backward_bp(const SdfNet& net, const B3Nets& b3, float* bwd, int ld, const f32x4* spill,
                                                const f32x4 (&dlast)[kSdfMT][kNT], float* out, int ostride, int wave,
                                                int lane, int tid, CLK* pc = nullptr, const float* xin = nullptr) {
    const int j = lane & 15, g = lane >> 4;
    const int mt0 = wave * kSdfMT;
#pragma unroll
    for (int m = 0; m < kSdfMT; ++m) {
        const int ch0 = (mt0 + m) * 16 + 4 * g;
        const f32x4 w = *reinterpret_cast<const f32x4*>(net.w6 + ch0);
#pragma unroll
        for (int n = 0; n < kNT; ++n) store_bsplit4(bwd, ld, 512, n * 16 + j, ch0, dlast[m][n] * w);
    }
    __syncthreads();
#pragma unroll 1
    for (int k = 4; k >= 0; --k) {
        f32x4 acc[kSdfMT][kNT];
#pragma unroll
        for (int m = 0; m < kSdfMT; ++m)
#pragma unroll
            for (int n = 0; n < kNT; ++n) zero_acc(acc[m][n]);
        f32x4 dk[kSdfMT][kNT];
#pragma unroll
        for (int m = 0; m < kSdfMT; ++m)
#pragma unroll
            for (int n = 0; n < kNT; ++n)
                dk[m][n] = k == 0 && xin ? layer0_dfactor(net, xin, mt0, m, n, lane)
                                         : spill[((k * kWaves + wave) * (kSdfMT * kNT) + m * kNT + n) * 64 + lane];
        gemm_acc_bsplit<8, kSdfMT>(b3.sdf_wpT[k], mt0, bwd, ld, 512, acc, lane);
        ARAH_PC_MARK(10);
        __syncthreads();
        ARAH_PC_MARK(12);
#pragma unroll
        for (int m = 0; m < kSdfMT; ++m) {
            const int ch0 = (mt0 + m) * 16 + 4 * g;
#pragma unroll
            for (int n = 0; n < kNT; ++n) store_bsplit4(bwd, ld, 512, n * 16 + j, ch0, acc[m][n] * dk[m][n]);
        }
        ARAH_PC_MARK(11);
        __syncthreads();
        ARAH_PC_MARK(12);
    }
    const int pt = tid >> 3, part = tid & 7;
    float gx = 0.f, gy = 0.f, gz = 0.f;
#pragma unroll 8
    for (int i = 0; i < 32; ++i) {
        const int ch = part + 8 * i;
        const float u = load_bsplit(bwd, ld, 512, pt, ch);
        const f32x4 w = *reinterpret_cast<const f32x4*>(net.w0 + ch * 4);
        gx += w[0] * u;
        gy += w[1] * u;
        gz += w[2] * u;
    }
#pragma unroll
    for (int o = 1; o < 8; o <<= 1) {
        gx += __shfl_xor(gx, o);
        gy += __shfl_xor(gy, o);
        gz += __shfl_xor(gz, o);
    }
    if (part == 0) {
        out[pt * ostride + 1] = gx;
        out[pt * ostride + 2] = gy;
        out[pt * ostride + 3] = gz;
    }
}

template <bool IDR, bool B3 = false>
__device__ __forceinline__ void color_mlp(const ColNet& net, const float* A, float* B, float* out, int ostride,
                                          int wave, int lane, int tid, const ColTap* tap = nullptr, const B3Nets* b3 = nullptr) {
    typedef ColDims<IDR> D;
    constexpr int ldB = kSdfLd;
    {
        f32x4 acc[2][kNT];
#pragma unroll
// ... 202 lines not shown
```

arah_release_amd/hip.py:

```python
import ctypes as C
import os

import torch

_HERE = os.path.dirname(os.path.abspath(__file__))
LIB_PATH = os.environ.get("ARAH_LIB_PATH") or os.path.join(_HERE, "libarah_hip.so")

ARAH_MAX_STEPS = 128
COLOR_NO_VIEW_DIR = 0
COLOR_IDR = 1
PRECISION_SPLIT_F16 = 0
PRECISION_FP32 = 1


SHADE_ENGINE_DEFAULT, SHADE_ENGINE_FP32 = 0, 1
CANON_KERNEL_WAVE, CANON_KERNEL_TILE, CANON_KERNEL_WAVE_L2 = 0, 1, 2


def default_shade_engine():
    return SHADE_ENGINE_FP32 if os.environ.get("ARAH_SHADE_ENGINE", "b3") == "fp32" else SHADE_ENGINE_DEFAULT


def default_canon_kernel():
    return {"tile": CANON_KERNEL_TILE, "wave_l2": CANON_KERNEL_WAVE_L2}.get(os.environ.get("ARAH_CANON_KERNEL", "wave"), CANON_KERNEL_WAVE)


def default_precision():
    v = os.environ.get("ARAH_PRECISION", "split").lower()
    if v in ("split", "split_f16", "f16x3", "0"):
        return PRECISION_SPLIT_F16
    if v in ("fp32", "f32", "exact", "1"):
        return PRECISION_FP32
    raise ValueError("ARAH_PRECISION must be 'split' or 'fp32', got %r" % v)

_ERRORS = {-1: "ARAH_E_BADARG", -2: "ARAH_E_SHAPE", -3: "ARAH_E_WORKSPACE", -4: "ARAH_E_LAUNCH",
           -5: "ARAH_E_SAMPLING", -6: "ARAH_E_OVERFLOW"}

_fp = C.c_void_p


class ArahNets(C.Structure):
    _fields_ = [("sdf_w", _fp * 7), ("sdf_b", _fp * 7), ("film_freq", _fp), ("film_phase", _fp),
                ("skin_w", _fp * 5), ("skin_b", _fp * 5), ("col_w", _fp * 6), ("col_b", _fp * 6),
                ("pose_vec", _fp), ("col_mode", C.c_int32), ("n_pose", C.c_int32), ("beta", _fp),
                ("precision", C.c_int32)]


class ArahBody(C.Structure):
    _fields_ = [("verts", _fp), ("vert_weights", _fp), ("bones", _fp), ("trans", _fp), ("center", _fp),
                ("coord_min", _fp), ("coord_max", _fp), ("n_verts", C.c_int32), ("prepared", C.c_void_p)]


class ArahSampling(C.Structure):
    _fields_ = [("n_steps", C.c_int32), ("n_near", C.c_int32), ("n_far", C.c_int32),
                ("cano_view_dirs", C.c_int32), ("render_last_pt", C.c_int32), ("full_shading", C.c_int32),
                ("lin_steps", _fp), ("lin_near", _fp), ("lin_far", _fp),
                ("shade_engine", C.c_int32), ("canon_kernel", C.c_int32),
                ("ev_canon", C.c_void_p * 2), ("ev_density", C.c_void_p * 2), ("ev_shade", C.c_void_p * 2),
                ("occupancy", C.c_void_p), ("ev_canon2", C.c_void_p * 2), ("ev_density2", C.c_void_p * 2)]


class ArahFrame(C.Structure):
    _fields_ = [("sdf_w0", _fp), ("sdf_wp", _fp * 5), ("sdf_wpT", _fp * 5), ("sdf_w6", _fp), ("sdf_b6", _fp),
                ("sdf_bias", _fp), ("sdf_freq", _fp), ("sdf_phase", _fp),
                ("sdf_wps", _fp * 5), ("sdf_fw", _fp), ("sdf_pw", _fp), ("sdf_fws", _fp),
                ("skin_w0", _fp), ("skin_wp", _fp * 3), ("skin_w4p", _fp), ("skin_bias", _fp),
                ("skin_wps", _fp * 4), ("skin_scales", _fp), ("skin_wpr", _fp), ("skin_wconsts", _fp),
                ("col_w0p", _fp), ("col_w1p", _fp), ("col_w2p", _fp), ("col_w3ap", _fp), ("col_w3bp", _fp),
                ("col_w4p", _fp), ("col_w5", _fp), ("col_bias", _fp),
                ("col_w0pT", _fp), ("col_w1pT", _fp), ("col_w2pT", _fp), ("col_w3apT", _fp), ("col_w3bpT", _fp),
                ("col_w4pT", _fp), ("b3", C.c_void_p * 22),
                ("verts4", _fp), ("knn_spheres", _fp), ("knn_grid", _fp), ("knn_cells", _fp),
                ("verts", _fp), ("vert_T", _fp), ("bones", _fp),
                ("scalars", _fp), ("n_verts", C.c_int32),
                ("col_mode", C.c_int32), ("precision", C.c_int32)]


class ArahTrainIn(C.Structure):
    _fields_ = [("n", C.c_int32), ("rotate_normal", C.c_int32), ("ray_augm", C.c_int32), ("geom_only", C.c_int32),
                ("x", _fp), ("T", _fp), ("view", _fp), ("view_orig", _fp), ("g_s", _fp), ("g_rgb", _fp),
                ("tap_cin", _fp), ("tap_c", _fp * 5), ("fwd_rgb4", _fp)]


class ArahTrainGrads(C.Structure):
    _fields_ = [("sdf", _fp), ("rgb4", _fp), ("gx4", _fp), ("film_freq", _fp), ("film_phase", _fp),
                ("h", _fp * 6), ("hd", _fp * 7), ("av", _fp * 6), ("avd", _fp * 6), ("cin", _fp), ("c", _fp * 5),
                ("d", _fp * 6)]


class ArahCounters(C.Structure):
    _fields_ = [("n_sdf_fwd", C.c_uint64), ("n_sdf_grad", C.c_uint64), ("n_skin_fwd", C.c_uint64),
                ("n_skin_jac", C.c_uint64), ("n_col", C.c_uint64), ("n_knn", C.c_uint64),
                ("n_density", C.c_uint64), ("n_canon", C.c_uint64), ("n_split_nonfinite", C.c_uint64),
                ("n_tier_rays", C.c_uint64), ("n_tier_rays_surface", C.c_uint64), ("n_tier_rays_promoted", C.c_uint64),
                ("n_tier_rays_skipped", C.c_uint64), ("n_tier_samples_p1", C.c_uint64), ("n_tier_samples_p2", C.c_uint64),
                ("n_tier_samples_skipped", C.c_uint64), ("n_tier_witnesses", C.c_uint64),
                ("n_tier_rays_untraced", C.c_uint64),
                ("n_canon_p2", C.c_uint64), ("n_density_p2", C.c_uint64)]


COUNTER_BYTES = C.sizeof(ArahCounters)


class ArahTierAudit(C.Structure):
    _fields_ = [("a_examined", C.c_uint64), ("a_violations", C.c_uint64), ("b_examined", C.c_uint64),
                ("b_converged", C.c_uint64), ("b_violations", C.c_uint64), ("c_examined", C.c_uint64),
                ("c_violations", C.c_uint64), ("n_first", C.c_uint64), ("first_index", C.c_int64 * 8),
                ("first_class", C.c_int32 * 8), ("min_ratio", C.c_float), ("rate_log2", C.c_int32), ("seed", C.c_uint32),
                ("reserved", C.c_int32)]


AUDIT_BYTES = C.sizeof(ArahTierAudit)

EXPORTS = ["arah_frame_bytes", "arah_prepare_frame", "arah_body_bytes", "arah_prepare_body", "arah_workspace_bytes", "arah_counters_reset",
           "arah_counters_read", "arah_sdf_eval", "arah_sdf_grid", "arah_rasterize", "arah_skin_lbs", "arah_skin_jacobian", "arah_color_eval",
           "arah_nearest_inverse_lbs", "arah_broyden3_lbs", "arah_joint_root_find", "arah_trace", "arah_sample_canonicalize",
           "arah_shade_composite", "arah_shade_points", "arah_render", "arah_shade_train_slab_bytes", "arah_shade_train_forward",
           "arah_shade_train_backward", "arah_composite_train_forward", "arah_composite_train_backward", "arah_gram_skinny_blocks", "arah_gram_skinny", "arah_colsum_blocks", "arah_colsum", "arah_inverse3x3", "arah_hsoftmax_train_forward", "arah_hsoftmax_train_backward", "arah_pose_tree_forward", "arah_pose_tree_backward", "arah_gemv_rows", "arah_mesh_query_scratch_bytes", "arah_mesh_query", "arah_dominant_kernel",
           "arah_skin_lbs_counted", "arah_marching_cubes_scratch_bytes", "arah_marching_cubes",
           "arah_marching_cubes_indexed_scratch_bytes", "arah_marching_cubes_indexed",
           "arah_occupancy_bytes", "arah_prepare_occupancy", "arah_occupancy_info", "arah_tier_debug", "arah_debug_samples",
           "arah_sample_depths_debug", "arah_cell_clusters_debug",
           "arah_sdf_grid_band_scratch_bytes", "arah_sdf_grid_band", "arah_tier_audit_bytes", "arah_tier_audit",
           "arah_tier_audit_debug", "arah_occupancy_clear_box", "arah_render_maps_bytes", "arah_render_maps",
           "arah_query_posed_bytes", "arah_query_posed", "arah_sdf_grid_posed_bytes", "arah_sdf_grid_posed",
           "arah_image_metrics_bytes", "arah_image_metrics",
           "arah_mesh_index_bytes", "arah_mesh_index_build", "arah_mesh_closest", "arah_surface_metrics_bytes", "arah_surface_metrics", "arah_face_area_cumsum",
           "arah_mesh_components_scratch_bytes", "arah_mesh_components", "arah_mesh_select_scratch_bytes", "arah_mesh_select",
           "arah_mesh_simplify_scratch_bytes", "arah_mesh_simplify",
           "arah_mesh_quadric_place_scratch_bytes", "arah_mesh_quadric_place",
           "arah_mesh_adjacency_scratch_bytes", "arah_mesh_adjacency", "arah_mesh_vertex_normals", "arah_mesh_smooth",
           "arah_mesh_orient_scratch_bytes", "arah_mesh_orient", "arah_mesh_boundary_loops_scratch_bytes",
           "arah_mesh_boundary_loops", "arah_mesh_fill_holes_scratch_bytes", "arah_mesh_fill_holes",
           "arah_mesh_rasterize", "arah_mesh_rasterize_debug", "arah_mesh_interpolate", "arah_mesh_raycast", "arah_mesh_raycast_debug",
           "arah_point_index_bytes", "arah_point_index_build", "arah_point_nearest", "arah_sample_scores_bytes", "arah_sample_scores",
           "arah_contains_index_bytes", "arah_contains_index_count", "arah_contains_index_fill", "arah_mesh_contains",
           "arah_mesh_contains_grid", "arah_mesh_sdf_grid_bytes", "arah_mesh_sdf_grid",
           "arah_winding_index_bytes", "arah_winding_index_count", "arah_winding_index_fill", "arah_mesh_winding",
           "arah_mesh_winding_grid", "arah_mesh_intersections_scratch_bytes", "arah_mesh_intersections"]

_lib = None


def load_library():
    global _lib
    if _lib is not None:
        return _lib
    if not os.path.exists(LIB_PATH):
        raise RuntimeError("libarah_hip.so is not built (%s): run `python -c 'import __graft_entry__ as g; "
                           "g.build()'` -- there is no CPU fallback for the hot path" % LIB_PATH)
    lib = C.CDLL(LIB_PATH)
    lib.arah_frame_bytes.restype = C.c_size_t
    lib.arah_body_bytes.restype = C.c_size_t
    lib.arah_workspace_bytes.restype = C.c_size_t
    lib.arah_workspace_bytes.argtypes = [C.c_int32, C.c_int32]
    lib.arah_dominant_kernel.restype = C.c_char_p
    lib.arah_shade_train_slab_bytes.restype = C.c_size_t
    lib.arah_mesh_query_scratch_bytes.restype = C.c_size_t
    lib.arah_marching_cubes_scratch_bytes.restype = C.c_size_t
    lib.arah_marching_cubes_scratch_bytes.argtypes = [C.c_int32]
    lib.arah_marching_cubes_indexed_scratch_bytes.restype = C.c_size_t
    lib.arah_marching_cubes_indexed_scratch_bytes.argtypes = [C.c_int32]
    lib.arah_occupancy_bytes.restype = C.c_size_t
    lib.arah_sdf_grid_band_scratch_bytes.restype = C.c_size_t
    lib.arah_colsum_blocks.argtypes = [C.c_int64]
    lib.arah_tier_audit_bytes.restype = C.c_size_t
    lib.arah_tier_audit_bytes.argtypes = [C.c_int32, C.c_int32]
    lib.arah_render_maps_bytes.restype = C.c_size_t
    lib.arah_render_maps_bytes.argtypes = [C.c_int32, C.c_int32]
    lib.arah_query_posed_bytes.restype = C.c_size_t
    lib.arah_query_posed_bytes.argtypes = [C.c_int32]
    lib.arah_sdf_grid_posed_bytes.restype = C.c_size_t
    lib.arah_sdf_grid_posed_bytes.argtypes = [C.c_int32]
    lib.arah_image_metrics_bytes.restype = C.c_size_t
    lib.arah_image_metrics_bytes.argtypes = [C.c_int32, C.c_int32]
    lib.arah_mesh_index_bytes.restype = C.c_size_t
    lib.arah_mesh_index_bytes.argtypes = [C.c_int32]
    lib.arah_surface_metrics_bytes.restype = C.c_size_t
    lib.arah_surface_metrics_bytes.argtypes = [C.c_int32, C.c_int32]
    for name in ("arah_point_index_bytes", "arah_sample_scores_bytes"):
        getattr(lib, name).restype = C.c_size_t
        getattr(lib, name).argtypes = [C.c_int32]
    for name in ("arah_mesh_components_scratch_bytes", "arah_mesh_select_scratch_bytes", "arah_mesh_adjacency_scratch_bytes",
                 "arah_mesh_quadric_place_scratch_bytes",
                 "arah_mesh_orient_scratch_bytes", "arah_mesh_boundary_loops_scratch_bytes", "arah_mesh_fill_holes_scratch_bytes"):
        getattr(lib, name).restype = C.c_size_t
        getattr(lib, name).argtypes = [C.c_int64, C.c_int64]
    lib.arah_mesh_simplify_scratch_bytes.restype = C.c_size_t
    lib.arah_mesh_simplify_scratch_bytes.argtypes = [C.c_int64, C.c_int64, C.c_int64]
    lib.arah_contains_index_bytes.restype = C.c_size_t
    lib.arah_contains_index_bytes.argtypes = [C.c_int32, C.c_int32]
    lib.arah_mesh_sdf_grid_bytes.restype = C.c_size_t
    lib.arah_mesh_sdf_grid_bytes.argtypes = [C.c_int64, C.c_int64, C.c_int64, C.c_int64]
    lib.arah_winding_index_bytes.restype = C.c_size_t
    lib.arah_winding_index_bytes.argtypes = [C.c_int32, C.c_int32]
    lib.arah_mesh_intersections_scratch_bytes.restype = C.c_size_t
    lib.arah_mesh_intersections_scratch_bytes.argtypes = [C.c_int64, C.c_int64, C.c_int64]
    for name in EXPORTS:
        getattr(lib, name)
    _lib = lib
    return lib


def _check(rc, what):
    if rc != 0:
        raise RuntimeError("%s failed: %s (%d)" % (what, _ERRORS.get(rc, "?"), rc))


def _ptr(t):
    if t is None:
        return None
    assert t.is_cuda and t.is_contiguous(), "device-resident contiguous tensor required"
    return C.c_void_p(t.data_ptr())


def _f32(t):
    return t.detach().to(dtype=torch.float32).contiguous()


_call_device = [None]


def _stream(device=None):
    device = device if device is not None else _call_device[0]
    return C.c_void_p(torch.cuda.current_stream(device).cuda_stream)


class _on_device:

    def __init__(self, device):
        self.device = torch.device(device)
        self.guard = torch.cuda.device(self.device)

    def __enter__(self):
        self.guard.__enter__()
        self.prev = _call_device[0]
        _call_device[0] = self.device

    def __exit__(self, *exc):
        _call_device[0] = self.prev
        return self.guard.__exit__(*exc)


def _guarded(fn):
    import functools

    @functools.wraps(fn)
    def wrapper(frame, ws, *args, **kwargs):
        dev = frame.device
        if ws.device != dev:
            raise ValueError("workspace lives on %s, frame on %s" % (ws.device, dev))

        def check(v):
            if isinstance(v, torch.Tensor):
                if v.device != dev:
                    raise ValueError("argument on %s, frame on %s" % (v.device, dev))
            elif isinstance(v, (tuple, list)):
                for u in v:
                    check(u)
        for v in list(args) + list(kwargs.values()):
            check(v)
        with _on_device(dev):
            return fn(frame, ws, *args, **kwargs)
    return wrapper


def _same_device(*tensors):
    dev = None
    for t in tensors:
        if t is None:
            continue
        if not t.is_cuda:
            raise ValueError("device-resident tensor required")
        if dev is None:
            dev = t.device
# ... 929 lines not shown

@_guarded
def skin_lbs_counted(frame, ws, x_hat, n_items, per_item=1):
    lib = load_library()
    x = _f32(x_hat)
    buf = ws.ensure(1, 1)
    xb = torch.zeros(x.shape[0], 3, device=x.device)
    _check(lib.arah_skin_lbs_counted(C.byref(frame.handle), _ptr(x), C.c_int32(int(x.shape[0])), _ptr(n_items),
                                     C.c_int32(int(per_item)), _ptr(xb), _ptr(buf), C.c_size_t(buf.numel()), _stream()),
           "arah_skin_lbs_counted")
    return xb


def gemv_rows(weight, x, b0=None, b1=None):
    require_gpu()
    lib = load_library()
    w, xv = weight.detach(), _f32(x).reshape(-1)
    if not (w.dtype == torch.float32 and w.is_contiguous() and w.dim() == 2 and w.shape[1] == xv.numel() and w.shape[1] % 4 == 0):
        raise ValueError("gemv_rows: weight (R, C) fp32 contiguous with C % 4 == 0 and x of C elements")
    with _on_device(w.device):
        y = torch.empty(w.shape[0], device=w.device)
        _check(lib.arah_gemv_rows(_ptr(w), C.c_int32(w.shape[0]), C.c_int32(w.shape[1]), _ptr(xv),
                                  _ptr(None if b0 is None else _f32(b0).reshape(-1)),
                                  _ptr(None if b1 is None else _f32(b1).reshape(-1)), _ptr(y), _stream()), "arah_gemv_rows")
    return y


def rasterize(tri_uvz, height, width, z_near=1e-4):
    require_gpu()
    lib = load_library()
    tri = _f32(tri_uvz)
    dev = tri.device
    with _on_device(dev):
        zbuf = torch.full((height * width,), -1, dtype=torch.int64, device=dev)
        _check(lib.arah_rasterize(_ptr(tri), C.c_int32(int(tri.shape[0])), C.c_int32(int(height)), C.c_int32(int(width)),
                                  C.c_float(float(z_near)), _ptr(zbuf), _stream()), "arah_rasterize")
    face = (zbuf & 0xffffffff).reshape(height, width)
    return torch.where(zbuf.reshape(height, width) == -1, torch.full_like(face, -1), face)


@_guarded
def skin_lbs(frame, ws, x_hat):
    lib = load_library()
    x = _f32(x_hat)
    n = x.shape[0]
    buf = ws.ensure(1, 1)
    w = torch.empty(n, 24, device=x.device)
    xb = torch.empty(n, 3, device=x.device)
    T = torch.empty(n, 4, 4, device=x.device)
    _check(lib.arah_skin_lbs(C.byref(frame.handle), _ptr(x), C.c_int32(n), _ptr(w), _ptr(xb), _ptr(T), _ptr(buf),
                             C.c_size_t(buf.numel()), _stream()), "arah_skin_lbs")
    return w, xb, T


@_guarded
def skin_jacobian(frame, ws, x_hat):
    lib = load_library()
    x = _f32(x_hat)
    n = x.shape[0]
    buf = ws.ensure(1, 1)
    jac = torch.empty(n, 3, 3, device=x.device)
    _check(lib.arah_skin_jacobian(C.byref(frame.handle), _ptr(x), C.c_int32(n), _ptr(jac), _ptr(buf),
                                  C.c_size_t(buf.numel()), _stream()), "arah_skin_jacobian")
    return jac


@_guarded
def color_eval(frame, ws, x_norm, normal, view, feat):
    lib = load_library()
    x, nr, ft = _f32(x_norm), _f32(normal), _f32(feat)
    vw = _f32(view) if view is not None else None
    n = x.shape[0]
    buf = ws.ensure(1, 1)
    rgb = torch.empty(n, 3, device=x.device)
    _check(lib.arah_color_eval(C.byref(frame.handle), _ptr(x), _ptr(nr), _ptr(vw), _ptr(ft), C.c_int32(n), _ptr(rgb),
                               _ptr(buf), C.c_size_t(buf.numel()), _stream()), "arah_color_eval")
    return rgb


@_guarded
def shade_points(frame, ws, x_norm, T, dirs, cano_view_dirs=True, shade_engine=None):
    lib = load_library()
    x, Tm, d = _f32(x_norm), _f32(T), _f32(dirs)
    n = x.shape[0]
    buf = ws.ensure(n, 1)
    rgbs = torch.empty(n, 4, device=x.device)
    sdfn = torch.empty(n, 4, device=x.device)
    eng = default_shade_engine() if shade_engine is None else int(shade_engine)
    _check(lib.arah_shade_points(C.byref(frame.handle), _ptr(x), _ptr(Tm), _ptr(d), C.c_int32(n), C.c_int32(int(bool(cano_view_dirs))),
                                 C.c_int32(eng), _ptr(rgbs), _ptr(sdfn), _ptr(buf), C.c_size_t(buf.numel()), _stream()), "arah_shade_points")
    return rgbs[:, :3], rgbs[:, 3], sdfn[:, 0], sdfn[:, 1:]


def sample_depths_debug(variant, sampling, near_far, conv, start, end):
    dev = near_far.device
    nf, st, en = _f32(near_far), _f32(start), _f32(end)
    cv = conv.to(torch.uint8).contiguous()
    n, S = int(st.shape[0]), int(sampling.n_steps)
    z = torch.empty(n, S, device=dev)
    mask = torch.empty(n, S, dtype=torch.uint8, device=dev)
    with _on_device(dev):
        _check(load_library().arah_sample_depths_debug(
            C.c_int32(int(variant)), C.c_int32(n), C.c_int32(S), C.c_int32(int(sampling.n_near)), C.c_int32(int(sampling.n_far)),
            _ptr(nf), _ptr(cv), _ptr(st), _ptr(en), _ptr(sampling.lin_steps), _ptr(sampling.lin_near), _ptr(sampling.lin_far),
            _ptr(z), _ptr(mask), _stream(dev)), "arah_sample_depths_debug")
    return z, mask


BODY_OFF_SPHERES, BODY_OFF_GRID, BODY_OFF_CELLS, BODY_CELL_BYTES = 114688, 118784, 119040, 64


def cell_clusters_debug(variant, body_buf):
    dev = body_buf.device
    n_cells = int(body_buf[BODY_OFF_GRID:BODY_OFF_GRID + 48].view(torch.int32)[8].item())
    cells = torch.zeros(n_cells, BODY_CELL_BYTES, dtype=torch.uint8, device=dev)
    with _on_device(dev):
        _check(load_library().arah_cell_clusters_debug(C.c_int32(int(variant)), _ptr(body_buf[BODY_OFF_GRID:]),
                                                       _ptr(body_buf[BODY_OFF_SPHERES:]), _ptr(cells), _stream(dev)),
               "arah_cell_clusters_debug")
    return cells


@_guarded
def nearest_inverse_lbs(frame, ws, pts):
    lib = load_library()
    p = _f32(pts)
    n = p.shape[0]
    buf = ws.ensure(1, 1)
    idx = torch.empty(n, dtype=torch.int32, device=p.device)
    x0 = torch.empty(n, 3, device=p.device)
    T0 = torch.empty(n, 4, 4, device=p.device)
    _check(lib.arah_nearest_inverse_lbs(C.byref(frame.handle), _ptr(p), C.c_int32(n), _ptr(idx), _ptr(x0), _ptr(T0),
                                        _ptr(buf), C.c_size_t(buf.numel()), _stream()), "arah_nearest_inverse_lbs")
    return idx, x0, T0


@_guarded
def broyden3_lbs(frame, ws, tgt, x0, T0, canon_kernel=None):
    lib = load_library()
    kern = default_canon_kernel() if canon_kernel is None else int(canon_kernel)
    tgt, x0, T0 = _f32(tgt), _f32(x0), _f32(T0)
    n = tgt.shape[0]
    buf = ws.ensure(n, 1)
    x = torch.empty(n, 3, device=tgt.device)
    T = torch.empty(n, 4, 4, device=tgt.device)
    err = torch.empty(n, device=tgt.device)
    conv = torch.empty(n, dtype=torch.uint8, device=tgt.device)
    _check(lib.arah_broyden3_lbs(C.byref(frame.handle), _ptr(tgt), _ptr(x0), _ptr(T0), C.c_int32(n), _ptr(x), _ptr(T),
                                 _ptr(err), _ptr(conv), C.c_int32(kern), _ptr(buf), C.c_size_t(buf.numel()), _stream()),
           "arah_broyden3_lbs")
    return x, T, err, conv.bool()


@_guarded
def joint_root_find(frame, ws, cam_loc, dirs, valid, x0, z0, T0):
    lib = load_library()
    cam, d, x0, z0, T0 = _f32(cam_loc), _f32(dirs), _f32(x0), _f32(z0), _f32(T0)
    v = valid.to(torch.uint8).contiguous()
    n = d.shape[0]
    buf = ws.ensure(n, 1)
    dev = d.device
    x = torch.empty(n, 3, device=dev)
    z = torch.empty(n, device=dev)
    T = torch.empty(n, 4, 4, device=dev)
    conv = torch.empty(n, dtype=torch.uint8, device=dev)
    _check(lib.arah_joint_root_find(C.byref(frame.handle), _ptr(cam), C.c_int32(n // cam.shape[0]), _ptr(d), _ptr(v),
                                    _ptr(x0), _ptr(z0), _ptr(T0), C.c_int32(n), _ptr(x), _ptr(z), _ptr(T), _ptr(conv),
                                    _ptr(buf), C.c_size_t(buf.numel()), _stream()), "arah_joint_root_find")
    return x, z, T, conv.bool()


@_guarded
def trace(frame, ws, cam_loc, dirs, near_far, root_find_all=False):
    lib = load_library()
    cam, d, nf = _f32(cam_loc), _f32(dirs), _f32(near_far)
    n = d.shape[0]
    buf = ws.ensure(n, 1)
    dev = d.device
    xn = torch.empty(n, 3, device=dev)
    T = torch.empty(n, 4, 4, device=dev)
    conv = torch.empty(n, dtype=torch.uint8, device=dev)
    start = torch.empty(n, device=dev)
    end = torch.empty(n, device=dev)
    _check(lib.arah_trace(C.byref(frame.handle), _ptr(cam), C.c_int32(n // cam.shape[0]), _ptr(d), _ptr(nf),
                          C.c_int32(n), C.c_int32(int(bool(root_find_all))), _ptr(xn), _ptr(T), _ptr(conv), _ptr(start),
                          _ptr(end), _ptr(buf), C.c_size_t(buf.numel()), _stream()), "arah_trace")
    return xn, T, conv, start, end


@_guarded
def sample_canonicalize(frame, ws, sampling, cam_loc, dirs, near_far, conv, start, end, rand=None):
    lib = load_library()
    r_s = r_n = r_f = None
    if rand is not None:
        r_s, r_n, r_f = [_f32(t) for t in rand]
    cam, d, nf = _f32(cam_loc), _f32(dirs), _f32(near_far)
    n, S = d.shape[0], sampling.n_steps
    buf = ws.ensure(n, S)
    dev = d.device
    z = torch.empty(n, S, device=dev)
    pts = torch.empty(n, S, 3, device=dev)
    T = torch.empty(n, S, 4, 4, device=dev)
    mask = torch.empty(n, S, dtype=torch.uint8, device=dev)
    _check(lib.arah_sample_canonicalize(C.byref(frame.handle), C.byref(sampling.handle), _ptr(cam),
                                        C.c_int32(n // cam.shape[0]), _ptr(d), _ptr(nf), _ptr(conv.contiguous()),
                                        _ptr(_f32(start)), _ptr(_f32(end)), C.c_int32(n), _ptr(r_s), _ptr(r_n), _ptr(r_f),
                                        _ptr(z), _ptr(pts), _ptr(T), _ptr(mask), _ptr(buf), C.c_size_t(buf.numel()),
                                        _stream()),
           "arah_sample_canonicalize")
    return z, pts, T, mask


@_guarded
def shade_composite(frame, ws, sampling, dirs, z, pts, T, mask):
    lib = load_library()
    d = _f32(dirs)
    n, S = d.shape[0], sampling.n_steps
    buf = ws.ensure(n, S)
    dev = d.device
    rgb = torch.empty(n, 3, device=dev)
    acc = torch.empty(n, device=dev)
    vol = torch.empty(n, dtype=torch.uint8, device=dev)
    _check(lib.arah_shade_composite(C.byref(frame.handle), C.byref(sampling.handle), _ptr(d), _ptr(_f32(z)),
                                    _ptr(_f32(pts)), _ptr(_f32(T)), _ptr(mask.contiguous()), C.c_int32(n), _ptr(rgb),
                                    _ptr(acc), _ptr(vol), _ptr(buf), C.c_size_t(buf.numel()), _stream()),
           "arah_shade_composite")
    return rgb, acc, vol


KIN_PAD = {COLOR_NO_VIEW_DIR: 272, COLOR_IDR: 304}


def _grouped(groups, n, width, device, inner=None):
    n_pad = (n + 8191) // 8192 * 8192 if n >= 65536 else ((n + 2047) // 2048 * 2048 if n >= 16384 else (n + 63) // 64 * 64)
    shape = (groups, n_pad, width) if inner is None else (groups, inner, n_pad, width)
    buf = torch.empty(*shape, device=device)
    if n_pad > n:
        buf[..., n:, :].zero_()
    return buf


def _train_in(x, T, view, view_orig, rotate_normal, ray_augm, g_s=None, g_rgb=None):
    t = ArahTrainIn()
    t.n, t.rotate_normal, t.ray_augm = int(x.shape[0]), int(bool(rotate_normal)), int(bool(ray_augm))
    t.x, t.T, t.view, t.view_orig = _ptr(x), _ptr(T), _ptr(view), _ptr(view_orig)
    t.g_s, t.g_rgb = _ptr(g_s), _ptr(g_rgb)
    return t


@_guarded
def shade_train_forward(frame, ws, x, T, view, view_orig, rotate_normal, ray_augm, keep=False):
    lib = load_library()
    x, view = _f32(x), _f32(view)
    T = _f32(T) if (T is not None and rotate_normal) else None
    vo = _f32(view_orig) if (view_orig is not None and ray_augm) else None
    n = x.shape[0]
    buf = ws.ensure(1, 1)
    sdf = torch.empty(n, device=x.device)
    rgb4 = torch.empty(n, 4, device=x.device)
    tin = _train_in(x, T, view, vo, rotate_normal, ray_augm)
    kept = None
    if keep:
        cc = _grouped(4, n, 256, x.device)
        cinp, c2p = _grouped(1, n, KIN_PAD[frame.color_mode], x.device)[0], _grouped(1, n, 128, x.device)[0]
        kept = {"cin": cinp[:n], "c": [cc[0, :n], cc[2, :n], c2p[:n], cc[1, :n], cc[3, :n]], "rgb4": rgb4, "cc": cc,
                "cin_pad": cinp, "c2_pad": c2p}
        tin.tap_cin = _ptr(kept["cin"])
        for i, t in enumerate(kept["c"]):
            tin.tap_c[i] = _ptr(t).value
    _check(lib.arah_shade_train_forward(C.byref(frame.handle), C.byref(tin), _ptr(sdf), _ptr(rgb4), _ptr(buf),
                                        C.c_size_t(buf.numel()), _stream()), "arah_shade_train_forward")
    return (sdf, rgb4[:, :3], kept) if keep else (sdf, rgb4[:, :3])


def _sdf_streams(n, dev):
    avv, hh, h0 = _grouped(6, n, 256, dev, inner=2), _grouped(5, n, 256, dev, inner=2), _grouped(2, n, 4, dev)
    return {"h": [h0[0, :n]] + [hh[k, 0, :n] for k in range(5)],
            "hd": [h0[1, :n]] + [hh[k, 1, :n] for k in range(5)] + [torch.empty(n, 256, device=dev)],
            "av": [avv[k, 0, :n] for k in range(6)], "avd": [avv[k, 1, :n] for k in range(6)], "avv": avv, "hh": hh, "h0": h0}


@_guarded
def sdf_normal_forward(frame, ws, x):
    lib = load_library()
    x = _f32(x)
    n = x.shape[0]
    buf = ws.ensure(1, 1)
    sdf = torch.empty(n, device=x.device)
    n4 = torch.empty(n, 4, device=x.device)
    tin = _train_in(x, None, None, None, False, False)
    tin.geom_only = 1
    _check(lib.arah_shade_train_forward(C.byref(frame.handle), C.byref(tin), _ptr(sdf), _ptr(n4), _ptr(buf),
                                        C.c_size_t(buf.numel()), _stream()), "arah_shade_train_forward")
    return sdf, n4[:, :3]


@_guarded
def sdf_normal_backward(frame, ws, x, g_s, g_n):
    lib = load_library()
    x, g_s, g_n = _f32(x), _f32(g_s), _f32(g_n)
    n, dev = x.shape[0], x.device
    buf = ws.ensure(1, 1)
    E = lambda *shape: torch.empty(*shape, device=dev)
    st = {"gx4": E(n, 4), "film_freq": E(6, 256), "film_phase": E(6, 256), "feat": E(n, 256)}
    st.update(_sdf_streams(n, dev))
    g = ArahTrainGrads()
    for k in ("gx4", "film_freq", "film_phase"):
        setattr(g, k, _ptr(st[k]))
    for k in ("h", "hd", "av", "avd"):
        arr = getattr(g, k)
        for i, t in enumerate(st[k]):
            arr[i] = _ptr(t).value
    g.c[0] = _ptr(st["feat"]).value
    nslab = lib.arah_shade_train_slab_bytes()
    if getattr(ws, "train_slab", None) is None or ws.train_slab.numel() < nslab:
        ws.train_slab = torch.empty(nslab, dtype=torch.uint8, device=dev)
    tin = _train_in(x, None, None, None, False, False, g_s, g_n)
    tin.geom_only = 1
    _check(lib.arah_shade_train_backward(C.byref(frame.handle), C.byref(tin), C.byref(g), _ptr(ws.train_slab),
                                         C.c_size_t(ws.train_slab.numel()), _ptr(buf), C.c_size_t(buf.numel()),
                                         _stream()), "arah_shade_train_backward")
    return st


@_guarded
def shade_train_backward(frame, ws, x, T, view, view_orig, rotate_normal, ray_augm, g_s, g_rgb, kept=None):
    lib = load_library()
    x, view, g_s, g_rgb = _f32(x), _f32(view), _f32(g_s), _f32(g_rgb)
    T = _f32(T) if (T is not None and rotate_normal) else None
    vo = _f32(view_orig) if (view_orig is not None and ray_augm) else None
    n, dev = x.shape[0], x.device
    buf = ws.ensure(1, 1)
    kin = KIN_PAD[frame.color_mode]
    E = lambda *shape: torch.empty(*shape, device=dev)
    if kept:
        cc, cinp, c2p = kept["cc"], kept["cin_pad"], kept["c2_pad"]
    else:
        cc, cinp, c2p = _grouped(4, n, 256, dev), _grouped(1, n, kin, dev)[0], _grouped(1, n, 128, dev)[0]
    dd = _grouped(4, n, 256, dev)
# ... 748 lines not shown
```

include/arah_hip.h:

```cpp
#ifndef ARAH_HIP_H
#define ARAH_HIP_H

#include <stddef.h>
#include <stdint.h>

#ifdef __cplusplus
extern "C" {
#endif

#define ARAH_OK 0
#define ARAH_E_BADARG (-1)
#define ARAH_E_SHAPE (-2)
#define ARAH_E_WORKSPACE (-3)
#define ARAH_E_LAUNCH (-4)
#define ARAH_E_SAMPLING (-5)
#define ARAH_E_OVERFLOW (-6)

#define ARAH_MAX_STEPS 128
#define ARAH_N_JOINTS 24
#define ARAH_COLOR_NO_VIEW_DIR 0
#define ARAH_COLOR_IDR 1

#define ARAH_PRECISION_SPLIT_F16 0
#define ARAH_PRECISION_FP32 1
// ... 230 lines not shown
    float* avd[6];
    float* cin;
    float* c[5];
    float* d[6];
} ArahTrainGrads;

size_t arah_shade_train_slab_bytes(void);
int arah_shade_train_forward(const ArahFrame* h_frame, const ArahTrainIn* h_in, float* sdf, float* rgb4,
                             void* workspace, size_t workspace_bytes, void* stream);
int arah_shade_train_backward(const ArahFrame* h_frame, const ArahTrainIn* h_in, const ArahTrainGrads* h_out,
                              void* slab, size_t slab_bytes, void* workspace, size_t workspace_bytes, void* stream);

int arah_composite_train_forward(int32_t n_rays, int32_t n_steps, int32_t render_last_pt, const int32_t* len,
                                 const int64_t* off, const float* sdf, const float* rgb, const float* z, const float* inv_beta,
                                 float* out_rgb, float* out_acc, void* stream);
int arah_composite_train_backward(int32_t n_rays, int32_t n_steps, int32_t render_last_pt, const int32_t* len,
                                  const int64_t* off, const float* sdf, const float* rgb, const float* z, const float* inv_beta,
                                  const float* g_rgb_map, const float* g_acc, float* g_sdf, float* g_rgb, float* g_inv_beta,
                                  void* stream);

int32_t arah_gram_skinny_blocks(int32_t n_rows);

int arah_gemv_rows(const float* W, int32_t n_rows, int32_t n_cols, const float* x, const float* b0, const float* b1,
                   float* y, void* stream);
int arah_gram_skinny(const float* a, int32_t lda, int32_t m, const float* b, int32_t ldb, int32_t n, int32_t n_rows,
                     float* partial, void* stream);

int32_t arah_colsum_blocks(int64_t n_rows);
int arah_colsum(const float* a, int64_t lda, int32_t n_cols, int64_t n_rows, const float* scale, float* partial, float* y,
                void* stream);

int arah_hsoftmax_train_forward(const float* logits, int32_t n, float scale, float* weights, void* stream);
int arah_hsoftmax_train_backward(const float* logits, int32_t n, float scale, const float* g_weights, float* g_logits, void* stream);

int arah_pose_tree_forward(const float* own, const float* glob, const float* W1, const float* b1, const float* W2,
                           const float* b2, const int32_t* parents_host, int32_t n_joints, float* feats, float* hidden,
                           void* stream);
int arah_pose_tree_backward(const float* own, const float* glob, const float* W1, const float* W2, const int32_t* parents_host,
                            int32_t n_joints, const float* feats, const float* hidden, const float* g_feats, float* gW1,
                            float* gb1, float* gW2, float* gb2, float* g_glob, void* stream);

int arah_inverse3x3(const float* m, int32_t n, float scale, float* inv, void* stream);

size_t arah_mesh_query_scratch_bytes(void);
int arah_mesh_query(const float* verts, int32_t n_verts, const int32_t* faces, int32_t n_faces, const void* pts,
                    int32_t pts_are_f64, int32_t n_pts, double* d2, int32_t* face, double* closest, double* bary,
                    uint8_t* inside, void* scratch, void* stream);

size_t arah_image_metrics_bytes(int32_t height, int32_t width);
int arah_image_metrics(const float* pred, const float* gt, const uint8_t* box_mask, int32_t height, int32_t width,
                       double data_range, double* out, int32_t* rect, void* scratch, size_t scratch_bytes, void* stream);

size_t arah_mesh_index_bytes(int32_t n_faces);
int arah_face_area_cumsum(const float* tris, int32_t n_faces, double* cum, void* stream);
int arah_mesh_index_build(const float* tris, int32_t n_faces, void* index, size_t index_bytes, void* stream);
int arah_mesh_closest(const void* index, size_t index_bytes, const float* tris, int32_t n_faces, const float* pts,
                      int32_t n_pts, double* d2, int32_t* face, double* closest, int32_t* tested, void* stream);
size_t arah_surface_metrics_bytes(int32_t n_a, int32_t n_b);
int arah_surface_metrics(const float* tris_a, int32_t n_faces_a, const int32_t* sample_face_a, const double* d2_ab,
                         const int32_t* face_ab, int32_t n_a, const float* tris_b, int32_t n_faces_b,
                         const int32_t* sample_face_b, const double* d2_ba, const int32_t* face_ba, int32_t n_b, double* out,
                         void* scratch, size_t scratch_bytes, void* stream);

size_t arah_mesh_intersections_scratch_bytes(int64_t n_verts, int64_t n_faces, int64_t max_pairs);
int arah_mesh_intersections(const float* verts, int64_t n_verts, const int32_t* faces, int64_t n_faces, const uint8_t* group,
                            int32_t between, const float h_origin[3], double scale, int64_t max_pairs, int32_t* hits, uint8_t* vert_hit,
                            int32_t* pair_start, int32_t* pairs, int32_t* counts, int64_t* tested, void* scratch, size_t scratch_bytes,
                            void* stream);

int arah_mesh_raycast(const void* index, size_t index_bytes, const float* tris, int32_t n_faces, const float* origins,
                      const float* dirs, int32_t n_rays, double t_min, double t_max, int32_t cull, int32_t mode, double* t,
                      int32_t* face, double* bary, uint8_t* hit, int32_t* tested, void* stream);
int arah_mesh_raycast_debug(const void* index, size_t index_bytes, const float* tris, int32_t n_faces, const float* origins,
                            const float* dirs, int32_t n_rays, double t_min, double t_max, int32_t cull, int32_t mode,
                            int32_t workgroup, double* t, int32_t* face, double* bary, uint8_t* hit, int32_t* tested, void* stream);

size_t arah_point_index_bytes(int32_t n_points);
int arah_point_index_build(const float* points, int32_t n_points, void* index, size_t index_bytes, void* stream);
int arah_point_nearest(const void* index, size_t index_bytes, const float* cloud, int32_t n_cloud, const float* queries,
                       int32_t n_queries, double* d2, int32_t* nearest, int32_t* tested, void* stream);
size_t arah_sample_scores_bytes(int32_t n);
int arah_sample_scores(const double* d2, int32_t n, const double* sample_normals, const double* other_normals, int32_t n_other,
                       const int32_t* idx, const double* thr2, int32_t n_thresholds, double* sums, int64_t* within, void* scratch,
                       size_t scratch_bytes, void* stream);

int arah_trace(const ArahFrame* h_frame, const float* cam_loc, int32_t rays_per_cam, const float* dirs,
               const float* near_far, int32_t n_rays, int32_t root_find_all, float* points_hat_norm, float* T,
               uint8_t* conv, float* start, float* end, void* workspace, size_t workspace_bytes, void* stream);
int arah_sample_canonicalize(const ArahFrame* h_frame, const ArahSampling* h_cfg, const float* cam_loc,
                             int32_t rays_per_cam, const float* dirs, const float* near_far,
                             const uint8_t* conv, const float* start, const float* end, int32_t n_rays,
                             const float* rand_steps, const float* rand_near, const float* rand_far,
                             float* z, float* pts, float* T, uint8_t* mask, void* workspace,
                             size_t workspace_bytes, void* stream);
int arah_shade_composite(const ArahFrame* h_frame, const ArahSampling* h_cfg, const float* dirs,
                         const float* z, const float* pts, const float* T, const uint8_t* mask,
                         int32_t n_rays, float* rgb, float* acc, uint8_t* vol_mask, void* workspace,
                         size_t workspace_bytes, void* stream);
int arah_shade_points(const ArahFrame* h_frame, const float* x_norm, const float* T, const float* dirs, int32_t n_pts,
                      int32_t cano_view_dirs, int32_t shade_engine, float* rgbs, float* sdfn, void* workspace,
                      size_t workspace_bytes, void* stream);
int arah_render(const ArahFrame* h_frame, const ArahSampling* h_cfg, const float* cam_loc,
                int32_t rays_per_cam, const float* dirs, const float* near_far, const float* pose34,
                int32_t n_rays, float* rgb, float* points_cam, uint8_t* vol_mask, float* acc,
                float* dists, uint8_t* surface_conv, void* workspace, size_t workspace_bytes,
                void* stream);

size_t arah_render_maps_bytes(int32_t n_rays, int32_t n_steps);
int arah_render_maps(const ArahFrame* h_frame, const ArahSampling* h_cfg, const float* cam_loc,
                     int32_t rays_per_cam, const float* dirs, const float* near_far, const float* pose34,
                     int32_t n_rays, float* rgb, float* points_cam, uint8_t* vol_mask, float* acc,
                     float* dists, uint8_t* surface_conv, float* normal_world, float* depth, void* workspace,
                     size_t workspace_bytes, void* maps_buf, size_t maps_buf_bytes, void* stream);

size_t arah_occupancy_bytes(void);
int arah_prepare_occupancy(const ArahFrame* h_frame, void* occ_buf, size_t occ_bytes, void* workspace,
                           size_t workspace_bytes, void* stream);
int arah_occupancy_info(const void* occ_buf, int32_t* h_out16, void* stream);
int arah_tier_debug(void* workspace, size_t workspace_bytes, int32_t n_rays, int32_t n_steps, uint8_t* ray_tier,
                    uint8_t* ray_sigma_pos, void* stream);

typedef struct ArahTierAudit {
    uint64_t a_examined, a_violations;
    uint64_t b_examined, b_converged, b_violations;
    uint64_t c_examined, c_violations;
    uint64_t n_first;
    int64_t first_index[8];
    int32_t first_class[8];
    float min_ratio;
    int32_t rate_log2;
    uint32_t seed;
    int32_t reserved;
} ArahTierAudit;
size_t arah_tier_audit_bytes(int32_t n_rays, int32_t n_steps);
int arah_tier_audit(const ArahFrame* h_frame, const ArahSampling* h_cfg, const float* cam_loc, int32_t rays_per_cam,
                    const float* dirs, const float* near_far, int32_t n_rays, int32_t rate_log2, uint32_t seed, void* audit_buf,
                    size_t audit_bytes, void* workspace, size_t workspace_bytes, void* stream);
int arah_tier_audit_debug(const void* audit_buf, size_t audit_bytes, int32_t n_rays, int32_t n_steps, uint8_t* sample_tag,
                          uint8_t* ray_tag, void* stream);
int arah_occupancy_clear_box(void* occ_buf, const float* h_lo, const float* h_hi, void* stream);

int arah_debug_samples(void* workspace, size_t workspace_bytes, int32_t n_rays, int32_t n_steps, float* z, float* pts,
                       float* T, uint8_t* mask, float* shaded, uint8_t* state, void* stream);

#define ARAH_BODY_OFF_SPHERES 114688u
#define ARAH_BODY_OFF_GRID 118784u
#define ARAH_BODY_OFF_CELLS 119040u
int arah_sample_depths_debug(int32_t variant, int32_t n_rays, int32_t n_steps, int32_t n_near, int32_t n_far,
                             const float* near_far, const uint8_t* conv, const float* start, const float* end,
                             const float* lin_steps, const float* lin_near, const float* lin_far, float* z, uint8_t* mask,
                             void* stream);
int arah_cell_clusters_debug(int32_t variant, const void* grid, const float* spheres, uint8_t* cells, void* stream);

#define ARAH_POSED_FILL 1.0f
size_t arah_query_posed_bytes(int32_t n_pts);
int arah_query_posed(const ArahFrame* h_frame, const void* occ_buf, const float* pts, int32_t n_pts, float* sdf, float* x_hat_norm,
                     float* T, float* normal, float* weights, uint8_t* state, void* buf, size_t buf_bytes, void* stream);
size_t arah_sdf_grid_posed_bytes(int32_t n_side);
int arah_sdf_grid_posed(const ArahFrame* h_frame, const void* occ_buf, const float* box, int32_t n_side, int32_t band, float* sdf,
                        float* box_out, int32_t* counts, void* buf, size_t buf_bytes, void* stream);

size_t arah_contains_index_bytes(int32_t n_faces, int32_t resolution);
int arah_contains_index_count(const float* verts, int32_t n_verts, const int32_t* faces, int32_t n_faces, int32_t resolution,
                              void* index, size_t index_bytes, void* stream);
int arah_contains_index_fill(void* index, size_t index_bytes, int32_t n_faces, int32_t resolution, int32_t* refs, int64_t n_refs,
                             void* stream);
int arah_mesh_contains(const void* index, size_t index_bytes, int32_t n_faces, int32_t resolution, const int32_t* refs, int64_t n_refs,
                       const void* pts, int32_t pts_are_f64, int32_t n_pts, uint8_t* inside, uint8_t* ambiguous, int32_t* tested,
                       void* stream);
int arah_mesh_contains_grid(const void* index, size_t index_bytes, int32_t n_faces, int32_t resolution, const int32_t* refs,
                            int64_t n_refs, const float* xs, int32_t nx, const float* ys, int32_t ny, const float* zs, int32_t nz,
                            uint8_t* occupancy, uint64_t* ambiguous, void* stream);

size_t arah_mesh_sdf_grid_bytes(int64_t n_faces, int64_t nx, int64_t ny, int64_t nz);
int arah_mesh_sdf_grid(const float* tris, int32_t n_faces, const float* xs, int32_t nx, const float* ys, int32_t ny, const float* zs,
                       int32_t nz, float trunc, const uint8_t* occupancy, double* d2, int32_t* face, float* sdf, int32_t* info,
                       void* scratch, size_t scratch_bytes, void* stream);

size_t arah_winding_index_bytes(int32_t n_faces, int32_t depth);
int arah_winding_index_count(const float* verts, int32_t n_verts, const int32_t* faces, int32_t n_faces, int32_t depth, void* index,
                             size_t index_bytes, int32_t* order, float* tris, void* stream);
int arah_winding_index_fill(const void* index, size_t index_bytes, int32_t n_faces, int32_t depth, const float* tris, int32_t* node_i,
                            double* node_f, int64_t n_nodes, void* stream);
int arah_mesh_winding(const void* index, size_t index_bytes, int32_t n_faces, int32_t depth, const float* tris, const int32_t* node_i,
                      const double* node_f, int64_t n_nodes, const float* pts, int32_t n_pts, double accuracy, double* w,
                      uint8_t* inside, int32_t* n_exact, int32_t* n_far, void* stream);
int arah_mesh_winding_grid(const void* index, size_t index_bytes, int32_t n_faces, int32_t depth, const float* tris,
                           const int32_t* node_i, const double* node_f, int64_t n_nodes, const float* xs, int32_t nx, const float* ys,
                           int32_t ny, const float* zs, int32_t nz, double accuracy, double* w, uint8_t* inside, int32_t* n_exact,
                           int32_t* n_far, void* stream);

const char* arah_dominant_kernel(void);
#ifdef __cplusplus
}
#endif
#endif
```

Baseline: 11.73 million.

## Fuse skinning and SDF MLP in joint finisher, stage fold-bias, add debug entry points

The joint Broyden finisher is restructured so that per-ray state (Jacobian inverse, step, gradient, best error) is staged in LDS, and a new fused skin+SDF tile routine runs both networks in one pass with split-f16 lookahead. This replaces separate skin and SDF evaluations in the per-iteration loop and removes repeated global loads. The bias-folding setup is merged into one LDS-staged kernel launch covering both layers. Debug entry points that override the bulk/handover iteration counts are added. The LDS budget grows but is asserted to still allow four workgroups per CU.

Measured after the change: 11.69 million. About the same (-0.4%).

```diff
diff --git a/arah_release_amd/csrc/arah_hip.hip b/arah_release_amd/csrc/arah_hip.hip
--- a/arah_release_amd/csrc/arah_hip.hip
+++ b/arah_release_amd/csrc/arah_hip.hip
@@ -363,6 +363,36 @@
     float s = b[r];
     for (int c = 0; c < n_vec; ++c) s += W[(size_t)r * ld + col0 + c] * vec[c];
     dst[r] = s;
+}
+
+constexpr int kFoldCols = 32;
+struct FoldJob {
+    float* dst;
+    const float* b;
+    const float* W;
+    int ld;
+};
+__global__ __launch_bounds__(256) void k_fold_bias_staged(FoldJob j0, FoldJob j1, int col0, const float* __restrict__ vec,
+                                                         int n_vec, int rows) {
+    __shared__ float tile[256][kFoldCols + 1];
+    __shared__ float svec[kFoldCols];
+    const FoldJob j = blockIdx.y == 0 ? j0 : j1;
+    const int r0 = blockIdx.x * 256, r = r0 + threadIdx.x;
+    const int nr = min(256, rows - r0);
+    float s = r < rows ? j.b[r] : 0.f;
+    for (int c0 = 0; c0 < n_vec; c0 += kFoldCols) {
+        const int cw = min(kFoldCols, n_vec - c0);
+        __syncthreads();
+        for (int e = threadIdx.x; e < nr * cw; e += 256) {
+            const int rr = e / cw, cc = e - rr * cw;
+            tile[rr][cc] = j.W[(size_t)(r0 + rr) * j.ld + col0 + c0 + cc];
+        }
+        if ((int)threadIdx.x < cw) svec[threadIdx.x] = vec[c0 + threadIdx.x];
+        __syncthreads();
+        if (r < rows)
+            for (int c = 0; c < cw; ++c) s += tile[threadIdx.x][c] * svec[c];
+    }
+    if (r < rows) j.dst[r] = s;
 }
 
 enum { SRC_POINTS = 0, SRC_RAYS = 1, SRC_SAMPLES = 2 };
@@ -3381,12 +3411,11 @@
         jobs.add_pack(P(L.col_w4pT), nets->col_w[4], 256, 256, 16, 16, one_seg(256), 1);
         jobs.add_copy(P(L.col_w5), nets->col_w[5], 3 * 256, 3 * 256);
         float* cb = P(L.col_bias);
-        hipLaunchKernelGGL(k_fold_bias, dim3(1), dim3(256), 0, s, cb, nets->col_b[0], nets->col_w[0], in_dim,
-                           feat0 + 256, nets->pose_vec, nets->pose_vec ? nets->n_pose : 0, 256);
+        hipLaunchKernelGGL(k_fold_bias_staged, dim3(1, 2), dim3(256), 0, s, FoldJob{cb, nets->col_b[0], nets->col_w[0], in_dim},
+                           FoldJob{cb + 640, nets->col_b[3], nets->col_w[3], in_dim + 128}, feat0 + 256, nets->pose_vec,
+                           nets->pose_vec ? nets->n_pose : 0, 256);
         jobs.add_copy(cb + 256, nets->col_b[1], 256, 256);
         jobs.add_copy(cb + 512, nets->col_b[2], 128, 128);
-        hipLaunchKernelGGL(k_fold_bias, dim3(1), dim3(256), 0, s, cb + 640, nets->col_b[3], nets->col_w[3],
-                           in_dim + 128, feat0 + 256, nets->pose_vec, nets->pose_vec ? nets->n_pose : 0, 256);
         jobs.add_copy(cb + 896, nets->col_b[4], 256, 256);
         jobs.add_copy(cb + 1152, nets->col_b[5], 3, 4);
     }
@@ -4476,7 +4505,7 @@
     return check_launch();
 }
 
-static void joint_impl(const FrameDev& fd, Workspace& w, const RaySet& rs, int n, float* T, hipStream_t s) {
+static void joint_impl(const FrameDev& fd, Workspace& w, const RaySet& rs, int n, float* T, hipStream_t s, int bulk_arg = -1) {
     int* cntB = w.counts + kNumCounts;
     const int gm = grid_for(n, kTile);
     hipLaunchKernelGGL(k_skin_jac, dim3(grid_for(n, 16)), dim3(kThreads), kLdsSkin, s, fd, (const float*)w.x0raw,
@@ -4488,7 +4517,7 @@
     hipLaunchKernelGGL(k_joint_init, dim3(grid_for(n, 256)), dim3(256), 0, s, fd, st, rs, (const int*)w.listA,
                        (const int*)&cntB[0], (const float*)w.grad_sdf, (const float*)w.jac_lbs, (const float*)w.xcur,
                        (const float*)w.t, w.x0raw);
-    const int bulk = knobs().joint_bulk;
+    const int bulk = bulk_arg < 0 ? knobs().joint_bulk : max(1, min(kBroydenSteps + 1, bulk_arg));
     for (int it = 0; it < bulk; ++it) {
         int* lin = (it & 1) ? w.listB : w.listA;
         int* lout = (it & 1) ? w.listA : w.listB;
@@ -4511,7 +4540,8 @@
 
 static int trace_impl(const ArahFrame* f, Workspace& w, const float* cam_loc, int32_t rays_per_cam,
                       const float* dirs, const float* near_far, int32_t n, int root_find_all, float* points_hat_norm,
-                      float* T, uint8_t* conv, float* start, float* end, hipStream_t s, const uint8_t* skip = nullptr) {
+                      float* T, uint8_t* conv, float* start, float* end, hipStream_t s, const uint8_t* skip = nullptr,
+                      int bulk_steps = -1, int small_below = -1, int joint_bulk = -1) {
     const FrameDev fd = to_dev(*f);
     const RaySet rs = make_rays(cam_loc, dirs, rays_per_cam);
     const int gb = (n + 255) / 256;
@@ -4523,7 +4553,9 @@
                        w.listA, &cntA[0], skip);
     TraceState ts{w.t, w.far, w.xcur, w.diverged};
     const int gm = grid_for(n, kTile);
-    const int bulk = n <= knobs().trace_small ? 0 : knobs().trace_bulk;
+    const int trace_small = small_below < 0 ? knobs().trace_small : small_below;
+    const int trace_bulk = bulk_steps < 0 ? knobs().trace_bulk : min(kSphereIters, bulk_steps);
+    const int bulk = n <= trace_small ? 0 : trace_bulk;
     for (int it = 0; it < bulk; ++it) {
         int* lin = (it & 1) ? w.listB : w.listA;
         int* lout = (it & 1) ? w.listA : w.listB;
@@ -4542,15 +4574,16 @@
     hipLaunchKernelGGL(k_joint_select, dim3(gb), dim3(256), 0, s, fd, n, (const float*)w.xcur, (const float*)w.Tcur,
                        (const float*)w.t, (const uint8_t*)w.diverged, root_find_all, w.x0raw, w.xbest_ray, w.zbest_ray, T,
                        w.err_best_ray, w.listA, &cntB[0]);
-    joint_impl(fd, w, rs, n, T, s);
+    joint_impl(fd, w, rs, n, T, s, joint_bulk);
     hipLaunchKernelGGL(k_trace_finalize, dim3(gb), dim3(256), 0, s, fd, n, near_far, (const float*)w.xbest_ray,
                        (const float*)w.zbest_ray, (const float*)w.err_best_ray, points_hat_norm, conv, start, end);
     return check_launch();
 }
 
-int arah_trace(const ArahFrame* f, const float* cam_loc, int32_t rays_per_cam, const float* dirs,
-               const float* near_far, int32_t n, int32_t root_find_all, float* points_hat_norm, float* T,
-               uint8_t* conv, float* start, float* end, void* workspace, size_t wbytes, void* stream) {
+static int trace_entry(const ArahFrame* f, const float* cam_loc, int32_t rays_per_cam, const float* dirs,
+                       const float* near_far, int32_t n, int32_t root_find_all, float* points_hat_norm, float* T,
+                       uint8_t* conv, float* start, float* end, void* workspace, size_t wbytes, void* stream,
+                       int bulk_steps, int small_below) {
     if (!f || n < 0 || !workspace) return ARAH_E_BADARG;
     if (n == 0) return ARAH_OK;
     if (!cam_loc || !dirs || !near_far || !points_hat_norm || !T || !conv || !start || !end) return ARAH_E_BADARG;
@@ -4558,12 +4591,28 @@
     if (wbytes < w.bytes) return ARAH_E_WORKSPACE;
     if (int arc = setup_attributes()) return arc;
     return trace_impl(f, w, cam_loc, rays_per_cam, dirs, near_far, n, root_find_all, points_hat_norm, T, conv, start,
-                      end, reinterpret_cast<hipStream_t>(stream));
-}
-
-int arah_joint_root_find(const ArahFrame* f, const float* cam_loc, int32_t rays_per_cam, const float* dirs,
-                         const uint8_t* valid, const float* x0, const float* z0, const float* T0, int32_t n, float* x,
-                         float* z, float* T, uint8_t* conv, void* workspace, size_t wbytes, void* stream) {
+                      end, reinterpret_cast<hipStream_t>(stream), nullptr, bulk_steps, small_below);
+}
+
+int arah_trace(const ArahFrame* f, const float* cam_loc, int32_t rays_per_cam, const float* dirs,
+               const float* near_far, int32_t n, int32_t root_find_all, float* points_hat_norm, float* T,
+               uint8_t* conv, float* start, float* end, void* workspace, size_t wbytes, void* stream) {
+    return trace_entry(f, cam_loc, rays_per_cam, dirs, near_far, n, root_find_all, points_hat_norm, T, conv, start, end,
+                       workspace, wbytes, stream, -1, -1);
+}
+
+int arah_trace_debug(const ArahFrame* f, const float* cam_loc, int32_t rays_per_cam, const float* dirs,
+                     const float* near_far, int32_t n, int32_t root_find_all, float* points_hat_norm, float* T,
+                     uint8_t* conv, float* start, float* end, void* workspace, size_t wbytes, void* stream,
+                     int32_t bulk_steps, int32_t small_below) {
+    if (bulk_steps < 0 || bulk_steps > kSphereIters || small_below < 0) return ARAH_E_BADARG;
+    return trace_entry(f, cam_loc, rays_per_cam, dirs, near_far, n, root_find_all, points_hat_norm, T, conv, start, end,
+                       workspace, wbytes, stream, bulk_steps, small_below);
+}
+
+static int joint_entry(const ArahFrame* f, const float* cam_loc, int32_t rays_per_cam, const float* dirs,
+                       const uint8_t* valid, const float* x0, const float* z0, const float* T0, int32_t n, float* x,
+                       float* z, float* T, uint8_t* conv, void* workspace, size_t wbytes, void* stream, int bulk_iters) {
     if (!f || n < 0 || !workspace) return ARAH_E_BADARG;
     if (n == 0) return ARAH_OK;
     if (!cam_loc || !dirs || !valid || !x0 || !z0 || !T0 || !x || !z || !T || !conv) return ARAH_E_BADARG;
@@ -4577,10 +4626,25 @@
     hipMemsetAsync(w.counts, 0, sizeof(int) * 3 * kNumCounts, s);
     hipLaunchKernelGGL(k_joint_seed, dim3(gb), dim3(256), 0, s, fd, n, x0, z0, T0, valid, w.x0raw, w.xcur, w.t, w.xbest_ray,
                        w.zbest_ray, T, w.err_best_ray, w.listA, &w.counts[kNumCounts]);
-    joint_impl(fd, w, rs, n, T, s);
+    joint_impl(fd, w, rs, n, T, s, bulk_iters);
     hipLaunchKernelGGL(k_joint_seam_out, dim3(gb), dim3(256), 0, s, n, (const float*)w.xbest_ray, (const float*)w.zbest_ray,
                        (const float*)w.err_best_ray, valid, x, z, conv);
     return check_launch();
+}
+
+int arah_joint_root_find(const ArahFrame* f, const float* cam_loc, int32_t rays_per_cam, const float* dirs,
+                         const uint8_t* valid, const float* x0, const float* z0, const float* T0, int32_t n, float* x,
+                         float* z, float* T, uint8_t* conv, void* workspace, size_t wbytes, void* stream) {
+    return joint_entry(f, cam_loc, rays_per_cam, dirs, valid, x0, z0, T0, n, x, z, T, conv, workspace, wbytes, stream, -1);
+}
+
+int arah_joint_root_find_debug(const ArahFrame* f, const float* cam_loc, int32_t rays_per_cam, const float* dirs,
+                               const uint8_t* valid, const float* x0, const float* z0, const float* T0, int32_t n,
+                               float* x, float* z, float* T, uint8_t* conv, void* workspace, size_t wbytes, void* stream,
+                               int32_t bulk_iters) {
+    if (bulk_iters < 1 || bulk_iters > kBroydenSteps + 1) return ARAH_E_BADARG;
+    return joint_entry(f, cam_loc, rays_per_cam, dirs, valid, x0, z0, T0, n, x, z, T, conv, workspace, wbytes, stream,
+                       bulk_iters);
 }
 
 static DepthArgs depth_args(const ArahSampling* cfg, const float* near_far, const float* start, const float* end) {
@@ -4665,6 +4729,19 @@
     if (!near_far || !conv || !start || !end || !z || !mask) return ARAH_E_BADARG;
     launch_sample_depths(variant, n, &cfg, near_far, conv, start, end, nullptr, nullptr, nullptr, z, mask,
                          reinterpret_cast<hipStream_t>(stream));
+    return check_launch();
+}
+
+int arah_fold_bias_debug(int32_t variant, float* dst, const float* b, const float* W, int32_t ld, int32_t col0,
+                         const float* vec, int32_t n_vec, int32_t rows, void* stream) {
+    if ((variant != 0 && variant != 1) || rows < 0 || n_vec < 0 || col0 < 0 || ld < col0 + n_vec) return ARAH_E_BADARG;
+    if (rows == 0) return ARAH_OK;
+    if (!dst || !b || (n_vec > 0 && (!W || !vec))) return ARAH_E_BADARG;
+    hipStream_t s = reinterpret_cast<hipStream_t>(stream);
+    const int gb = (rows + 255) / 256;
+    if (variant == 0) hipLaunchKernelGGL(k_fold_bias, dim3(gb), dim3(256), 0, s, dst, b, W, ld, col0, vec, n_vec, rows);
+    else hipLaunchKernelGGL(k_fold_bias_staged, dim3(gb, 1), dim3(256), 0, s, FoldJob{dst, b, W, ld}, FoldJob{dst, b, W, ld}, col0,
+                            vec, n_vec, rows);
     return check_launch();
 }
 
diff --git a/arah_release_amd/csrc/finish.hpp b/arah_release_amd/csrc/finish.hpp
--- a/arah_release_amd/csrc/finish.hpp
+++ b/arah_release_amd/csrc/finish.hpp
@@ -1,8 +1,12 @@
 #pragma once
 
 constexpr int kFinTile = 16;
+constexpr int kFinAheadJoint = 2;
 constexpr size_t kLdsTraceFinish = (kFinTile * 4 * 2 + kFinTile * 16 + kFinTile * 8) * 4 + (size_t)kFinTile * kSdfLd * 4;
-constexpr size_t kLdsJointFinish = (kFinTile * 4 * 3 + 24 * 16 + kFinTile * 2 + kFinTile * kLogitLd + 32) * 4 + (size_t)kFinTile * kSdfLd * 4;
+constexpr size_t kLdsJointFinish = (kFinTile * 4 * 3 + 24 * 16 + kFinTile * 2 + kFinTile * kLogitLd + kFinTile * 16 * 2 +
+                                    kFinTile * 4 * 3 + kFinTile * 2) * 4 +
+                                   (size_t)kFinTile * kSkinLd * 4 + (size_t)kFinTile * kSdfLd * 4;
+static_assert(kLdsJointFinish <= 40 * 1024 && kLdsTraceFinish <= 40 * 1024, "four finisher workgroups fit a CU's LDS");
 
 template <bool SPLIT>
 __global__ __launch_bounds__(kThreads, 4) void k_trace_finish(FrameDev fr, KnnData kd, RaySet rs, TraceState st, float* Tcur,
@@ -128,7 +132,15 @@
     int* ids = reinterpret_cast<int*>(sbones + 24 * 16);
     int* s_live = ids + TW;
     float* logits = reinterpret_cast<float*>(s_live + TW);
-    float* act = logits + TW * kLogitLd;
+    float* Jl = logits + TW * kLogitLd;
+    float* Tb = Jl + 16 * TW;
+    float* stepl = Tb + 16 * TW;
+    float* gxl = stepl + TW * 4;
+    float* bestl = gxl + TW * 4;
+    float* ebl = bestl + TW * 4;
+    int* dirty = reinterpret_cast<int*>(ebl + TW);
+    float* sact = reinterpret_cast<float*>(dirty + TW);
+    float* act = sact + TW * kSkinLd;
     const int tid = threadIdx.x, wave = __builtin_amdgcn_readfirstlane(tid >> 6), lane = tid & 63;
     const int n = *count;
     const float scale = sdf_scale(bc);
@@ -136,76 +148,107 @@
     for (int i = tid; i < 24 * 16; i += kThreads) sbones[i] = fr.bones[i];
     for (int tile = blockIdx.x; tile * TW < n; tile += gridDim.x) {
         __syncthreads();
-        if (tid < TW) {
-            const int i = tile * TW + tid;
-            ids[tid] = i < n ? list[i] : -1;
+        if (wave == 0) {
+            int id = -1;
+            if (lane < TW) {
+                const int i = tile * TW + lane;
+                id = i < n ? list[i] : -1;
+                ids[lane] = id;
+                f32x4 u = {0.f, 0.f, 0.f, 0.f};
+                if (id >= 0) {
+                    u = reinterpret_cast<const f32x4*>(st.ueval)[id];
+                    reinterpret_cast<f32x4*>(stepl)[lane] = reinterpret_cast<const f32x4*>(st.step)[id];
+                    reinterpret_cast<f32x4*>(gxl)[lane] = reinterpret_cast<const f32x4*>(st.gx)[id];
+#pragma unroll
+                    for (int c = 0; c < 4; ++c) {
+                        const f32x4 jr = reinterpret_cast<const f32x4*>(st.Jinv + (size_t)id * 16)[c];
+#pragma unroll
+                        for (int r = 0; r < 4; ++r) Jl[(c * 4 + r) * TW + lane] = jr[r];
+                    }
+                    ebl[lane] = st.err_best[id];
+                }
+                dirty[lane] = 0;
+                const V3 q = normalize_pt(bc, V3{u[0], u[1], u[2]});
+                reinterpret_cast<f32x4*>(xin)[lane] = f32x4{q.x, q.y, q.z, 0.f};
+                reinterpret_cast<f32x4*>(xraw)[lane] = u;
+            }
+            const unsigned long long live = __ballot(id >= 0);
+            if (iters_left > 0) n_done += __popcll(live);
+            if (lane == 0) *s_live = live != 0ull;
         }
         for (int it = 0; it < iters_left; ++it) {
             __syncthreads();
+            if (!*s_live) break;
+            skin_sdf_tile16<SPLIT, kFinAheadJoint>(fr.skin, fr.sdf, xin, sact, logits, act, kSdfLd, wave, lane);
+            sdf_head<SPLIT>(fr.sdf, act, kSdfLd, outv, 4, tid, TW);
+            __syncthreads();
             if (wave == 0) {
-                const unsigned long long live = __ballot(lane < TW && ids[lane] >= 0);
-                n_done += __popcll(live);
+                bool keep = false;
+                if (lane < TW) {
+                    const int id = ids[lane];
+                    if (id >= 0) {
+                        float T[16];
+                        V3 xb;
+                        const f32x4 u = reinterpret_cast<const f32x4*>(xraw)[lane];
+                        skin_tail(logits + lane * kLogitLd, sbones, V3{u[0], u[1], u[2]}, T, xb);
+                        const V3 p = ray_point(rs, id, u[3]);
+                        float gnew[4] = {outv[lane * 4] * scale, xb.x - (p.x - bc.trans[0]), xb.y - (p.y - bc.trans[1]),
+                                         xb.z - (p.z - bc.trans[2])};
+                        float J[16], stp[4], gx[4], dg[4], dx[4];
+#pragma unroll
+                        for (int e = 0; e < 16; ++e) J[e] = Jl[e * TW + lane];
+#pragma unroll
+                        for (int r = 0; r < 4; ++r) {
+                            dx[r] = stepl[lane * 4 + r];
+                            const float gold = gxl[lane * 4 + r];
+                            dg[r] = gnew[r] - gold;
+                            gx[r] = gold + dg[r];
+                        }
+                        const float err = sqrtf(gx[0] * gx[0] + gx[1] * gx[1] + gx[2] * gx[2] + gx[3] * gx[3]);
+                        float eb = ebl[lane];
+                        if (err < eb) {
+                            eb = err;
+                            ebl[lane] = err;
+                            reinterpret_cast<f32x4*>(bestl)[lane] = u;
+#pragma unroll
+                            for (int e = 0; e < 16; ++e) Tb[e * TW + lane] = T[e];
+                            dirty[lane] = 1;
+                        }
+                        keep = (eb > kRootThresh) && (err < kDvg);
+                        f32x4 un = {0.f, 0.f, 0.f, 0.f};
+                        if (keep) {
+                            broyden_update<4>(J, dx, dg, gx, stp);
+#pragma unroll
+                            for (int r = 0; r < 4; ++r) gxl[lane * 4 + r] = gx[r];
+#pragma unroll
+                            for (int e = 0; e < 16; ++e) Jl[e * TW + lane] = J[e];
+                            reinterpret_cast<f32x4*>(stepl)[lane] = f32x4{stp[0], stp[1], stp[2], stp[3]};
+                            un = f32x4{u[0] + stp[0], u[1] + stp[1], u[2] + stp[2], u[3] + stp[3]};
+                        }
+                        if (!keep || it + 1 == iters_left) {
+                            if (dirty[lane]) {
+                                const f32x4 b = reinterpret_cast<const f32x4*>(bestl)[lane];
+                                st.err_best[id] = eb;
+                                st.xbest[(size_t)id * 3] = b[0];
+                                st.xbest[(size_t)id * 3 + 1] = b[1];
+                                st.xbest[(size_t)id * 3 + 2] = b[2];
+                                st.zbest[id] = b[3];
+#pragma unroll
+                                for (int c = 0; c < 4; ++c)
+                                    reinterpret_cast<f32x4*>(st.Tbest + (size_t)id * 16)[c] =
+                                        f32x4{Tb[(c * 4) * TW + lane], Tb[(c * 4 + 1) * TW + lane], Tb[(c * 4 + 2) * TW + lane],
+                                              Tb[(c * 4 + 3) * TW + lane]};
+                            }
+                            ids[lane] = -1;
+                        }
+                        const V3 q = normalize_pt(bc, V3{un[0], un[1], un[2]});
+                        reinterpret_cast<f32x4*>(xin)[lane] = f32x4{q.x, q.y, q.z, 0.f};
+                        reinterpret_cast<f32x4*>(xraw)[lane] = un;
+                    }
+                }
+                const unsigned long long live = __ballot(keep);
+                if (it + 1 < iters_left) n_done += __popcll(live);
                 if (lane == 0) *s_live = live != 0ull;
-            }
-            if (tid < TW) {
-                const int id = ids[tid];
-                f32x4 u = {0.f, 0.f, 0.f, 0.f};
-                if (id >= 0) u = reinterpret_cast<const f32x4*>(st.ueval)[id];
-                const V3 q = normalize_pt(bc, V3{u[0], u[1], u[2]});
-                reinterpret_cast<f32x4*>(xin)[tid] = f32x4{q.x, q.y, q.z, 0.f};
-                reinterpret_cast<f32x4*>(xraw)[tid] = u;
-            }
-            __syncthreads();
-            if (!*s_live) break;
-            skin_mlp<1>(fr.skin, xin, act, logits, wave, lane);
-            f32x4 dlast[kSdfMT][1];
-            sdf_trunk<false, 1, SPLIT>(fr.sdf, xin, act, kSdfLd, nullptr, dlast, wave, lane);
-            sdf_head<SPLIT>(fr.sdf, act, kSdfLd, outv, 4, tid, TW);
-            __syncthreads();
-            if (tid < TW) {
-                const int id = ids[tid];
-                if (id >= 0) {
-                    float T[16];
-                    V3 xb;
-                    const f32x4 u = reinterpret_cast<const f32x4*>(xraw)[tid];
-                    skin_tail(logits + tid * kLogitLd, sbones, V3{u[0], u[1], u[2]}, T, xb);
-                    const V3 p = ray_point(rs, id, u[3]);
-                    float gnew[4] = {outv[tid * 4] * scale, xb.x - (p.x - bc.trans[0]), xb.y - (p.y - bc.trans[1]),
-                                     xb.z - (p.z - bc.trans[2])};
-                    float J[16], stp[4], gx[4], dg[4], dx[4];
-#pragma unroll
-                    for (int e = 0; e < 16; ++e) J[e] = st.Jinv[(size_t)id * 16 + e];
-#pragma unroll
-                    for (int r = 0; r < 4; ++r) {
-                        dx[r] = st.step[(size_t)id * 4 + r];
-                        const float gold = st.gx[(size_t)id * 4 + r];
-                        dg[r] = gnew[r] - gold;
-                        gx[r] = gold + dg[r];
-                    }
-                    const float err = sqrtf(gx[0] * gx[0] + gx[1] * gx[1] + gx[2] * gx[2] + gx[3] * gx[3]);
-                    float eb = st.err_best[id];
-                    if (err < eb) {
-                        eb = err;
-                        st.err_best[id] = err;
-                        st.xbest[(size_t)id * 3] = u[0];
-                        st.xbest[(size_t)id * 3 + 1] = u[1];
-                        st.xbest[(size_t)id * 3 + 2] = u[2];
-                        st.zbest[id] = u[3];
-                        store_T(st.Tbest + (size_t)id * 16, T);
-                    }
-                    const bool keep = (eb > kRootThresh) && (err < kDvg);
-                    if (keep) {
-                        broyden_update<4>(J, dx, dg, gx, stp);
-#pragma unroll
-                        for (int r = 0; r < 4; ++r) st.gx[(size_t)id * 4 + r] = gx[r];
-#pragma unroll
-                        for (int e = 0; e < 16; ++e) st.Jinv[(size_t)id * 16 + e] = J[e];
-                        reinterpret_cast<f32x4*>(st.step)[id] = f32x4{stp[0], stp[1], stp[2], stp[3]};
-                        reinterpret_cast<f32x4*>(st.ueval)[id] = f32x4{u[0] + stp[0], u[1] + stp[1], u[2] + stp[2], u[3] + stp[3]};
-                    } else {
-                        ids[tid] = -1;
-                    }
-                }
             }
         }
     }
diff --git a/arah_release_amd/csrc/mlp.hpp b/arah_release_amd/csrc/mlp.hpp
--- a/arah_release_amd/csrc/mlp.hpp
+++ b/arah_release_amd/csrc/mlp.hpp
@@ -313,6 +313,51 @@
     });
 }
 
+template <int KC32, int MT, int LA>
+__device__ __forceinline__ void gemm_acc_split_ahead(const f16x8* __restrict__ wp, int mt0, const float* act, int ld,
+                                                     int lo_off, f32x4 (&acc)[MT][1], int lane) {
+    static_assert(LA >= 1 && LA <= KC32, "lookahead in chunks");
+    constexpr int R = LA + 1;
+    const int j = lane & 15, g = lane >> 4;
+    const char* bptr = reinterpret_cast<const char*>(act) + j * ld * 4 + split_slot(j, g) * 16;
+    const unsigned aoff = (unsigned)(mt0 * KC32 * 2 * 64 + lane) * 16u;
+    auto lda = [&](int idx) { return ld_frag<f16x8>(wp, aoff, idx * 1024); };
+    f16x8 ah[R][MT], al[R][MT], bh[2], bl[2];
+    static_for<0, LA>([&](auto Kc) {
+        constexpr int kc = decltype(Kc)::value;
+#pragma unroll
+        for (int m = 0; m < MT; ++m) {
+            ah[kc][m] = lda((m * KC32 + kc) * 2 + 0);
+            al[kc][m] = lda((m * KC32 + kc) * 2 + 1);
+        }
+    });
+    bh[0] = *reinterpret_cast<const f16x8*>(bptr);
+    bl[0] = *reinterpret_cast<const f16x8*>(bptr + lo_off);
+    __builtin_amdgcn_sched_barrier(0);
+    static_for<0, KC32>([&](auto Kc) {
+        constexpr int kc = decltype(Kc)::value, ca = kc % R, cb = kc & 1;
+        if constexpr (kc + LA < KC32) {
+            constexpr int sn = (kc + LA) % R;
+#pragma unroll
+            for (int m = 0; m < MT; ++m) {
+                ah[sn][m] = lda((m * KC32 + kc + LA) * 2 + 0);
+                al[sn][m] = lda((m * KC32 + kc + LA) * 2 + 1);
+            }
+        }
+        if constexpr (kc + 1 < KC32) {
+            bh[cb ^ 1] = *reinterpret_cast<const f16x8*>(bptr + (kc + 1) * 64);
+            bl[cb ^ 1] = *reinterpret_cast<const f16x8*>(bptr + lo_off + (kc + 1) * 64);
+        }
+#pragma unroll
+        for (int m = 0; m < MT; ++m) acc[m][0] = __builtin_amdgcn_mfma_f32_16x16x32_f16(al[ca][m], bh[cb], acc[m][0], 0, 0, 0);
+#pragma unroll
+        for (int m = 0; m < MT; ++m) acc[m][0] = __builtin_amdgcn_mfma_f32_16x16x32_f16(ah[ca][m], bl[cb], acc[m][0], 0, 0, 0);
+#pragma unroll
+        for (int m = 0; m < MT; ++m) acc[m][0] = __builtin_amdgcn_mfma_f32_16x16x32_f16(ah[ca][m], bh[cb], acc[m][0], 0, 0, 0);
+        __builtin_amdgcn_sched_barrier(0);
+    });
+}
+
 
 struct B3Nets {
     const bf16x8* sdf_wp[5];
@@ -906,6 +951,95 @@
     clk.mark(9);
 }
 
+template <bool SPLIT, int AHEAD>
+__device__ __forceinline__ void skin_sdf_tile16(const SkinNet& skin, const SdfNet& net, const float* xin, float* sact,
+                                                float* logits, float* act, int ld, int wave, int lane) {
+    const int j = lane & 15, g = lane >> 4;
+    const int mt0 = wave * kSdfMT;
+    constexpr float amp = SPLIT ? kActScale : 1.0f;
+    const f32x4 zero4 = {0.f, 0.f, 0.f, 0.f};
+    const int sch0 = wave * 16 + 4 * g;
+    {
+        const f32x4 x = *reinterpret_cast<const f32x4*>(xin + j * 4);
+        {
+            f32x4 w[4];
+#pragma unroll
+            for (int r = 0; r < 4; ++r) w[r] = *reinterpret_cast<const f32x4*>(skin.w0 + (sch0 + r) * 4);
+            const f32x4 b = *reinterpret_cast<const f32x4*>(skin.bias + sch0);
+            f32x4 h;
+#pragma unroll
+            for (int r = 0; r < 4; ++r) h[r] = fmaf(w[r][2], x[2], fmaf(w[r][1], x[1], fmaf(w[r][0], x[0], b[r])));
+            no_pack(h);
+#pragma unroll
+            for (int r = 0; r < 4; ++r) h[r] = softplus100(h[r]);
+            *reinterpret_cast<f32x4*>(sact + j * kSkinLd + sch0) = h;
+        }
+#pragma unroll
+        for (int m = 0; m < kSdfMT; ++m) {
+            const int ch0 = (mt0 + m) * 16 + 4 * g;
+            f32x4 w[4];
+#pragma unroll
+            for (int r = 0; r < 4; ++r) w[r] = *reinterpret_cast<const f32x4*>(net.w0 + (ch0 + r) * 4);
+            const f32x4 fw = *reinterpret_cast<const f32x4*>(net.fw + ch0);
+            const f32x4 pw = *reinterpret_cast<const f32x4*>(net.pw + ch0);
+            f32x4 v, h, d;
+#pragma unroll
+            for (int r = 0; r < 4; ++r) v[r] = fmaf(w[r][2], x[2], fmaf(w[r][1], x[1], w[r][0] * x[0]));
+            no_pack(v);
+            film_sine<false>(v, fw, pw, zero4, amp, h, d);
+            if (SPLIT) store_split4(act, ld, 512, j, ch0, h);
+            else *reinterpret_cast<f32x4*>(act + j * ld + ch0) = h;
+        }
+    }
+    __syncthreads();
+#pragma unroll 1
+    for (int k = 1; k < 6; ++k) {
+        f32x4 sacc[1][1];
+        f32x4 sb = zero4;
+        zero_acc(sacc[0][0]);
+        if (k < 4) {
+            gemm_acc<8, 1, 1>(skin.wp[k - 1], wave, sact, kSkinLd, sacc, lane);
+            sb = *reinterpret_cast<const f32x4*>(skin.bias + k * 128 + sch0);
+        } else if (k == 4 && wave < 2) {
+            sacc[0][0] = gemm_one<8>(skin.w4p, wave, 0, sact, kSkinLd, lane);
+            sb = *reinterpret_cast<const f32x4*>(skin.bias + 4 * 128 + wave * 16 + 4 * g);
+        }
+        f32x4 acc[kSdfMT][1];
+#pragma unroll
+        for (int m = 0; m < kSdfMT; ++m) zero_acc(acc[m][0]);
+        if constexpr (SPLIT && AHEAD > 0) gemm_acc_split_ahead<8, kSdfMT, AHEAD>(net.wps[k - 1], mt0, act, ld, 512, acc, lane);
+        else if (SPLIT) gemm_acc_split<8, kSdfMT, 1, false>(net.wps[k - 1], mt0, act, ld, 512, acc, lane);
+        else gemm_acc<16, kSdfMT, 1>(net.wp[k - 1], mt0, act, ld, acc, lane);
+        f32x4 fwm[kSdfMT], pwm[kSdfMT];
+#pragma unroll
+        for (int m = 0; m < kSdfMT; ++m) {
+            const int ch0 = (mt0 + m) * 16 + 4 * g;
+            fwm[m] = *reinterpret_cast<const f32x4*>((SPLIT ? net.fws : net.fw) + k * 256 + ch0);
+            pwm[m] = *reinterpret_cast<const f32x4*>(net.pw + k * 256 + ch0);
+        }
+        __syncthreads();
+        if (k < 4) {
+            f32x4 h;
+#pragma unroll
+            for (int r = 0; r < 4; ++r) h[r] = softplus100(sacc[0][0][r] + sb[r]);
+            *reinterpret_cast<f32x4*>(sact + j * kSkinLd + sch0) = h;
+        } else if (k == 4 && wave < 2) {
+            const int ch0 = wave * 16 + 4 * g;
+#pragma unroll
+            for (int r = 0; r < 4; ++r) logits[j * kLogitLd + ch0 + r] = sacc[0][0][r] + sb[r];
+        }
+#pragma unroll
+        for (int m = 0; m < kSdfMT; ++m) {
+            const int ch0 = (mt0 + m) * 16 + 4 * g;
+            f32x4 h, d;
+            film_sine<false>(acc[m][0], fwm[m], pwm[m], zero4, amp, h, d);
+            if (SPLIT) store_split4(act, ld, 512, j, ch0, h);
+            else *reinterpret_cast<f32x4*>(act + j * ld + ch0) = h;
+        }
+        __syncthreads();
+    }
+}
+
 struct ColNet {
     const float* w0p;
     const float* w1p;
diff --git a/arah_release_amd/hip.py b/arah_release_amd/hip.py
--- a/arah_release_amd/hip.py
+++ b/arah_release_amd/hip.py
@@ -121,6 +121,7 @@
            "arah_marching_cubes_indexed_scratch_bytes", "arah_marching_cubes_indexed",
            "arah_occupancy_bytes", "arah_prepare_occupancy", "arah_occupancy_info", "arah_tier_debug", "arah_debug_samples",
            "arah_sample_depths_debug", "arah_cell_clusters_debug",
+           "arah_trace_debug", "arah_joint_root_find_debug", "arah_fold_bias_debug",
            "arah_sdf_grid_band_scratch_bytes", "arah_sdf_grid_band", "arah_tier_audit_bytes", "arah_tier_audit",
            "arah_tier_audit_debug", "arah_occupancy_clear_box", "arah_render_maps_bytes", "arah_render_maps",
            "arah_query_posed_bytes", "arah_query_posed", "arah_sdf_grid_posed_bytes", "arah_sdf_grid_posed",
@@ -1356,8 +1357,20 @@
     return x, T, err, conv.bool()
 
 
+def fold_bias_debug(variant, b, W, col0, vec):
+    dev = W.device
+    b, W, vec = _f32(b), _f32(W), _f32(vec)
+    rows, ld, n_vec = int(W.shape[0]), int(W.shape[1]), int(vec.shape[0])
+    dst = torch.full((rows,), float("nan"), device=dev)
+    with _on_device(dev):
+        _check(load_library().arah_fold_bias_debug(C.c_int32(int(variant)), _ptr(dst), _ptr(b), _ptr(W), C.c_int32(ld),
+                                                   C.c_int32(int(col0)), _ptr(vec) if n_vec else None, C.c_int32(n_vec),
+                                                   C.c_int32(rows), _stream(dev)), "arah_fold_bias_debug")
+    return dst
+
+
 @_guarded
-def joint_root_find(frame, ws, cam_loc, dirs, valid, x0, z0, T0):
+def joint_root_find(frame, ws, cam_loc, dirs, valid, x0, z0, T0, bulk_iters=None):
     lib = load_library()
     cam, d, x0, z0, T0 = _f32(cam_loc), _f32(dirs), _f32(x0), _f32(z0), _f32(T0)
     v = valid.to(torch.uint8).contiguous()
@@ -1368,14 +1381,17 @@
     z = torch.empty(n, device=dev)
     T = torch.empty(n, 4, 4, device=dev)
     conv = torch.empty(n, dtype=torch.uint8, device=dev)
-    _check(lib.arah_joint_root_find(C.byref(frame.handle), _ptr(cam), C.c_int32(n // cam.shape[0]), _ptr(d), _ptr(v),
-                                    _ptr(x0), _ptr(z0), _ptr(T0), C.c_int32(n), _ptr(x), _ptr(z), _ptr(T), _ptr(conv),
-                                    _ptr(buf), C.c_size_t(buf.numel()), _stream()), "arah_joint_root_find")
+    args = (C.byref(frame.handle), _ptr(cam), C.c_int32(n // cam.shape[0]), _ptr(d), _ptr(v), _ptr(x0), _ptr(z0), _ptr(T0),
+            C.c_int32(n), _ptr(x), _ptr(z), _ptr(T), _ptr(conv), _ptr(buf), C.c_size_t(buf.numel()), _stream())
+    if bulk_iters is None:
+        _check(lib.arah_joint_root_find(*args), "arah_joint_root_find")
+    else:
+        _check(lib.arah_joint_root_find_debug(*args, C.c_int32(int(bulk_iters))), "arah_joint_root_find_debug")
     return x, z, T, conv.bool()
 
 
 @_guarded
-def trace(frame, ws, cam_loc, dirs, near_far, root_find_all=False):
+def trace(frame, ws, cam_loc, dirs, near_far, root_find_all=False, handover=None):
     lib = load_library()
     cam, d, nf = _f32(cam_loc), _f32(dirs), _f32(near_far)
     n = d.shape[0]
@@ -1386,9 +1402,13 @@
     conv = torch.empty(n, dtype=torch.uint8, device=dev)
     start = torch.empty(n, device=dev)
     end = torch.empty(n, device=dev)
-    _check(lib.arah_trace(C.byref(frame.handle), _ptr(cam), C.c_int32(n // cam.shape[0]), _ptr(d), _ptr(nf),
-                          C.c_int32(n), C.c_int32(int(bool(root_find_all))), _ptr(xn), _ptr(T), _ptr(conv), _ptr(start),
-                          _ptr(end), _ptr(buf), C.c_size_t(buf.numel()), _stream()), "arah_trace")
+    args = (C.byref(frame.handle), _ptr(cam), C.c_int32(n // cam.shape[0]), _ptr(d), _ptr(nf), C.c_int32(n),
+            C.c_int32(int(bool(root_find_all))), _ptr(xn), _ptr(T), _ptr(conv), _ptr(start), _ptr(end), _ptr(buf),
+            C.c_size_t(buf.numel()), _stream())
+    if handover is None:
+        _check(lib.arah_trace(*args), "arah_trace")
+    else:
+        _check(lib.arah_trace_debug(*args, C.c_int32(int(handover[0])), C.c_int32(int(handover[1]))), "arah_trace_debug")
     return xn, T, conv, start, end
 
 
diff --git a/include/arah_hip.h b/include/arah_hip.h
--- a/include/arah_hip.h
+++ b/include/arah_hip.h
@@ -406,6 +406,17 @@
                              void* stream);
 int arah_cell_clusters_debug(int32_t variant, const void* grid, const float* spheres, uint8_t* cells, void* stream);
 
+int arah_trace_debug(const ArahFrame* frame, const float* cam_loc, int32_t rays_per_cam, const float* dirs,
+                     const float* near_far, int32_t n_rays, int32_t root_find_all, float* points_hat_norm, float* T,
+                     uint8_t* conv, float* start, float* end, void* workspace, size_t workspace_bytes, void* stream,
+                     int32_t bulk_steps, int32_t small_below);
+int arah_joint_root_find_debug(const ArahFrame* frame, const float* cam_loc, int32_t rays_per_cam, const float* dirs,
+                               const uint8_t* valid, const float* x0, const float* z0, const float* T0, int32_t n_rays,
+                               float* x, float* z, float* T, uint8_t* conv, void* workspace, size_t workspace_bytes,
+                               void* stream, int32_t bulk_iters);
+int arah_fold_bias_debug(int32_t variant, float* dst, const float* b, const float* W, int32_t ld, int32_t col0,
+                         const float* vec, int32_t n_vec, int32_t rows, void* stream);
+
 #define ARAH_POSED_FILL 1.0f
 size_t arah_query_posed_bytes(int32_t n_pts);
 int arah_query_posed(const ArahFrame* h_frame, const void* occ_buf, const float* pts, int32_t n_pts, float* sdf, float* x_hat_norm,
```
